# jacobkaufmann/kateth

Hardware: AMD Instinct MI355X
Metric: blobs/sec for blob_to_kzg_commitment and verify_blob_kzg_proof_batch (n=4096) (higher is better)
Workload: dtype u32 limbs (381-bit Fp / 255-bit Fr Montgomery integer arithmetic; signed 30-bit limbs on v_mad_i64_i32 in the fixed-base MSM, 28/29-bit radix in the other hot loops); 1 GPU; blob_to_kzg_commitment batch=4096 blobs per GPU (BASELINE configs[1]); blobs_per_gpu=4096, calls_in_flight=1, window_bits=22, parallelism=blob-sharded x1, RCCL all-gather of 48-B results, plane_groups=8

## Files before the change

include/kateth_amd.h:

```cpp
#ifndef KATETH_AMD_H
#define KATETH_AMD_H

#include <stddef.h>
#include <stdint.h>

#ifdef __cplusplus
extern "C" {
#endif

#define KZG_FIELD_ELEMENTS_PER_BLOB 4096
#define KZG_BYTES_PER_FIELD_ELEMENT 32
#define KZG_BYTES_PER_BLOB 131072
#define KZG_BYTES_PER_G1 48
#define KZG_BYTES_PER_G2 96
#define KZG_SETUP_G1_POINTS 4096
#define KZG_SETUP_G2_POINTS 65
#define KZG_CELLS_PER_EXT_BLOB 128
#define KZG_FIELD_ELEMENTS_PER_CELL 64
#define KZG_BYTES_PER_CELL 2048
#define KZG_G1_MONOMIAL_POINTS 64

#define KZG_OK 0
#define KZG_ERR_BLOB_INVALID_LEN 1
#define KZG_ERR_BLOB_INVALID_FIELD_ELEMENT 2
#define KZG_ERR_EC_INVALID_ENCODING 3
#define KZG_ERR_EC_NOT_ON_CURVE 4
#define KZG_ERR_EC_NOT_IN_GROUP 5
#define KZG_ERR_FF_INVALID_ENCODING 6
#define KZG_ERR_FF_NOT_IN_FIELD 7
#define KZG_ERR_CELLS_NOT_ENOUGH 8
#define KZG_ERR_CELLS_INCONSISTENT 9
#define KZG_ERR_CELL_INDEX 10
#define KZG_ERR_COMMITMENT_INDEX 11

#define KZG_FAIL_ARGUMENT (-1)
#define KZG_FAIL_HIP (-2)
#define KZG_FAIL_NO_DEVICE (-3)
#define KZG_FAIL_SETUP_G1 (-4)
#define KZG_FAIL_SETUP_G2 (-5)
#define KZG_FAIL_SETUP_UNSUPPORTED (-6)
#define KZG_FAIL_HOST (-7)

typedef struct kzg_ctx kzg_ctx;

#define KZG_CFG_TABLE_MAX 0x1
#define KZG_CFG_BUILD_ASYNC 0x2
#define KZG_ALL_DEVICES 0xffffffffu
typedef struct kzg_config {
  uint32_t struct_size;
  int32_t device;
  int32_t window_bits;
  int32_t flags;
  int32_t plane_groups;
  uint64_t table_budget_bytes;
  const int32_t* devices;
  uint32_t ndev;
  uint32_t reserved;
} kzg_config;
#define KZG_CONFIG_INIT {(uint32_t)sizeof(kzg_config), 0, 0, 0, 0, 0, NULL, 0, 0}

const char* kzg_recommended_env(void);

const char* kzg_last_error(void);
int32_t kzg_last_error_code(void);

int32_t kzg_ctx_create(const uint8_t* g1_lagrange, const uint8_t* g2_monomial, const kzg_config* cfg, kzg_ctx** out);
int32_t kzg_ctx_create_multi(const uint8_t* g1_lagrange, const uint8_t* g2_monomial, const int32_t* devices, uint32_t ndev, const kzg_config* cfg,
                             kzg_ctx** out);
void kzg_ctx_destroy(kzg_ctx* ctx);
int32_t kzg_device_count(void);
uint32_t kzg_ctx_members(const kzg_ctx* ctx);
int32_t kzg_ctx_member_device(const kzg_ctx* ctx, uint32_t k);
const kzg_ctx* kzg_ctx_member(const kzg_ctx* ctx, uint32_t k);
int32_t kzg_ctx_ready(const kzg_ctx* ctx);
int32_t kzg_ctx_wait_ready(const kzg_ctx* ctx);

int32_t kzg_ctx_window_bits(const kzg_ctx* ctx);
const char* kzg_ctx_msm_kernel_name(const kzg_ctx* ctx);
int32_t kzg_ctx_plane_groups(const kzg_ctx* ctx);
uint64_t kzg_ctx_table_bytes(const kzg_ctx* ctx);
uint64_t kzg_ctx_workspace_bytes(const kzg_ctx* ctx, uint32_t slot);

int32_t kzg_blob_to_commitment_batch(const kzg_ctx* ctx, const uint8_t* blobs, uint64_t n, uint8_t* out48, int32_t* status);
int32_t kzg_blob_to_commitment_batch_dev(const kzg_ctx* ctx, const void* d_blobs, uint64_t n, void* d_out48, void* d_status, void* hip_stream);

int32_t kzg_blob_to_commitment_batch_affine(const kzg_ctx* ctx, const uint8_t* blobs, uint64_t n, uint8_t* out_affine96, int32_t* status);
int32_t kzg_compute_blob_proof_batch_affine(const kzg_ctx* ctx, const uint8_t* blobs, const uint8_t* commitments48, uint64_t n, uint8_t* out_affine96, int32_t* status);
int32_t kzg_compute_proof_batch_affine(const kzg_ctx* ctx, const uint8_t* blobs, const uint8_t* z32, uint64_t n, uint8_t* out_proof_affine96, uint8_t* out_y32, int32_t* status);

int32_t kzg_g1_decompress_batch(const kzg_ctx* ctx, const uint8_t* in48, uint64_t n, uint8_t* out_affine96, int32_t* status);

int32_t kzg_evaluate_blobs(const kzg_ctx* ctx, const uint8_t* blobs, const uint8_t* z32, uint64_t n, uint8_t* out_y32, int32_t* status);

int32_t kzg_compute_blob_proof_batch(const kzg_ctx* ctx, const uint8_t* blobs, const uint8_t* commitments48, uint64_t n, uint8_t* out48, int32_t* status);
int32_t kzg_compute_blob_proof_batch_dev(const kzg_ctx* ctx, const void* d_blobs, const void* d_commitments48, uint64_t n, void* d_out48, void* d_status, void* hip_stream);

int32_t kzg_blob_sidecar_batch(const kzg_ctx* ctx, const uint8_t* blobs, uint64_t n, uint8_t* out_commitments48, uint8_t* out_proofs48,
                               uint8_t* out_versioned_hashes32 , int32_t* status);
int32_t kzg_blob_sidecar_batch_dev(const kzg_ctx* ctx, const void* d_blobs, uint64_t n, void* d_out_commitments48, void* d_out_proofs48,
                                   void* d_out_versioned_hashes32 , void* d_status, void* hip_stream);

int32_t kzg_compute_cells_batch(const kzg_ctx* ctx, const uint8_t* blobs, uint64_t n, uint8_t* out_cells , int32_t* status);
int32_t kzg_compute_cells_batch_dev(const kzg_ctx* ctx, const void* d_blobs, uint64_t n, void* d_out_cells, void* d_status, void* hip_stream);

int32_t kzg_recover_cells_batch(const kzg_ctx* ctx, const uint8_t* cells , const uint8_t* present , uint64_t n,
                                uint8_t* out_cells , int32_t* status);
int32_t kzg_recover_cells_batch_dev(const kzg_ctx* ctx, const void* d_cells, const void* d_present, uint64_t n, void* d_out_cells, void* d_status,
                                    void* hip_stream);

int32_t kzg_compute_cells_and_proofs_batch(const kzg_ctx* ctx, const uint8_t* blobs, uint64_t n, uint8_t* out_cells ,
                                           uint8_t* out_proofs48 , int32_t* status);
int32_t kzg_compute_cells_and_proofs_batch_dev(const kzg_ctx* ctx, const void* d_blobs, uint64_t n, void* d_out_cells , void* d_out_proofs48,
                                               void* d_status, void* hip_stream);
int32_t kzg_recover_cells_and_proofs_batch(const kzg_ctx* ctx, const uint8_t* cells, const uint8_t* present, uint64_t n, uint8_t* out_cells,
                                           uint8_t* out_proofs48, int32_t* status);
int32_t kzg_recover_cells_and_proofs_batch_dev(const kzg_ctx* ctx, const void* d_cells, const void* d_present, uint64_t n, void* d_out_cells,
                                               void* d_out_proofs48, void* d_status, void* hip_stream);

int32_t kzg_compute_cells_and_proofs_select_batch(const kzg_ctx* ctx, const uint8_t* blobs, const uint8_t* want , uint64_t n,
                                                  uint8_t* out_cells , uint8_t* inout_proofs48 ,
                                                  int32_t* status);
int32_t kzg_compute_cells_and_proofs_select_batch_dev(const kzg_ctx* ctx, const void* d_blobs, const uint8_t* want , uint64_t n,
                                                      void* d_out_cells , void* d_inout_proofs48, void* d_status, void* hip_stream);
int32_t kzg_recover_cells_and_proofs_select_batch(const kzg_ctx* ctx, const uint8_t* cells, const uint8_t* present, const uint8_t* want ,
                                                  uint64_t n, uint8_t* out_cells, uint8_t* inout_proofs48, int32_t* status);
int32_t kzg_recover_cells_and_proofs_select_batch_dev(const kzg_ctx* ctx, const void* d_cells, const void* d_present, const uint8_t* want ,
                                                      uint64_t n, void* d_out_cells, void* d_inout_proofs48, void* d_status, void* hip_stream);
uint64_t kzg_ctx_cellproof_vectors(const kzg_ctx* ctx);

int32_t kzg_compute_proof_batch(const kzg_ctx* ctx, const uint8_t* blobs, const uint8_t* z32, uint64_t n, uint8_t* out_proof48, uint8_t* out_y32, int32_t* status);

int32_t kzg_verify_blob_proof_batch(const kzg_ctx* ctx, const uint8_t* blobs, const uint8_t* commitments48, const uint8_t* proofs48, uint64_t n, int32_t* ok);
int32_t kzg_verify_blob_proof_batch_dev(const kzg_ctx* ctx, const void* d_blobs, const void* d_commitments48, const void* d_proofs48, uint64_t n, int32_t* ok, void* hip_stream);

int32_t kzg_verify_blob_proof(const kzg_ctx* ctx, const uint8_t* blob, const uint8_t* commitment48, const uint8_t* proof48, int32_t* ok);

int32_t kzg_verify_proof(const kzg_ctx* ctx, const uint8_t* proof48, const uint8_t* commitment48, const uint8_t* z32, const uint8_t* y32, int32_t* ok);

int32_t kzg_verify_proof_batch(const kzg_ctx* ctx, const uint8_t* proofs48, const uint8_t* commitments48, const uint8_t* z32, const uint8_t* y32, uint64_t n,
                               int32_t* ok);
int32_t kzg_verify_proof_batch_dev(const kzg_ctx* ctx, const void* d_proofs48, const void* d_commitments48, const void* d_z32, const void* d_y32, uint64_t n,
                                   int32_t* ok, void* hip_stream);
int32_t kzg_verify_proof_batch_group_dev(const kzg_ctx* ctx, const void* const* d_proofs48, const void* const* d_commitments48, const void* const* d_z32,
                                         const void* const* d_y32, const uint64_t* n_local, int32_t* ok, void* const* hip_streams);

int32_t kzg_ctx_g1_monomial(const kzg_ctx* ctx, uint32_t first, uint32_t count, uint8_t* out48);

int32_t kzg_verify_cell_proof_batch(const kzg_ctx* ctx, const uint8_t* commitments48, const uint64_t* cell_indices, const uint8_t* cells ,
                                    const uint8_t* proofs48, uint64_t n, int32_t* ok);
int32_t kzg_verify_cell_proof_batch_dev(const kzg_ctx* ctx, const void* d_commitments48, const void* d_cell_indices, const void* d_cells,
                                        const void* d_proofs48, uint64_t n, int32_t* ok, void* hip_stream);

int32_t kzg_verify_cell_proof_batch_rows(const kzg_ctx* ctx, const uint8_t* commitments48 , uint64_t u, const uint64_t* commitment_indices ,
                                         const uint64_t* cell_indices , const uint8_t* cells , const uint8_t* proofs48 ,
                                         uint64_t n, int32_t* ok);
int32_t kzg_verify_cell_proof_batch_rows_dev(const kzg_ctx* ctx, const void* d_commitments48, uint64_t u, const void* d_commitment_indices,
                                             const void* d_cell_indices, const void* d_cells, const void* d_proofs48, uint64_t n, int32_t* ok,
                                             void* hip_stream);
int32_t kzg_cell_row_weights(const kzg_ctx* ctx, const uint8_t* r32, uint64_t first_index, const uint64_t* commitment_indices , uint64_t n,
                             uint64_t u, uint8_t* out_w32 );

int32_t kzg_verify_blob_proof_batch_each(const kzg_ctx* ctx, const uint8_t* blobs, const uint8_t* commitments48, const uint8_t* proofs48, uint64_t n,
                                         uint8_t* ok_each, int32_t* status, int32_t* ok);
int32_t kzg_verify_blob_proof_batch_each_dev(const kzg_ctx* ctx, const void* d_blobs, const void* d_commitments48, const void* d_proofs48, uint64_t n,
                                             uint8_t* ok_each, int32_t* status, int32_t* ok, void* hip_stream);
int32_t kzg_verify_proof_batch_each(const kzg_ctx* ctx, const uint8_t* proofs48, const uint8_t* commitments48, const uint8_t* z32, const uint8_t* y32, uint64_t n,
                                    uint8_t* ok_each, int32_t* status, int32_t* ok);
int32_t kzg_verify_proof_batch_each_dev(const kzg_ctx* ctx, const void* d_proofs48, const void* d_commitments48, const void* d_z32, const void* d_y32, uint64_t n,
                                        uint8_t* ok_each, int32_t* status, int32_t* ok, void* hip_stream);
uint64_t kzg_verify_each_checks(const kzg_ctx* ctx);
uint64_t kzg_ctx_sessions_created(const kzg_ctx* ctx);

int32_t kzg_verify_cell_proof_batch_each(const kzg_ctx* ctx, const uint8_t* commitments48, const uint64_t* cell_indices, const uint8_t* cells ,
                                         const uint8_t* proofs48, uint64_t n, uint8_t* ok_each, int32_t* status, int32_t* ok);
int32_t kzg_verify_cell_proof_batch_each_dev(const kzg_ctx* ctx, const void* d_commitments48, const void* d_cell_indices, const void* d_cells,
                                             const void* d_proofs48, uint64_t n, uint8_t* ok_each, int32_t* status, int32_t* ok, void* hip_stream);

int32_t kzg_g1_monomial_lincomb(const kzg_ctx* ctx, const uint8_t* scalars32, uint64_t m, uint8_t* out96);

int32_t kzg_blob_to_commitment_batch_group_dev(const kzg_ctx* ctx, const void* const* d_blobs, const uint64_t* n_local, void* const* d_out48,
                                               void* const* d_status, void* const* hip_streams);
int32_t kzg_compute_blob_proof_batch_group_dev(const kzg_ctx* ctx, const void* const* d_blobs, const void* const* d_commitments48, const uint64_t* n_local,
                                               void* const* d_out48, void* const* d_status, void* const* hip_streams);
int32_t kzg_verify_blob_proof_batch_group_dev(const kzg_ctx* ctx, const void* const* d_blobs, const void* const* d_commitments48,
                                              const void* const* d_proofs48, const uint64_t* n_local, int32_t* ok, void* const* hip_streams);

typedef struct kzg_verify_session kzg_verify_session;
int32_t kzg_verify_phase1_dev(const kzg_ctx* ctx, const void* d_blobs, const void* d_commitments48, const void* d_proofs48, uint64_t n_local,
                              uint8_t* out_root32, int32_t* err6, kzg_verify_session** session, void* hip_stream);
int32_t kzg_verify_phase2_dev(kzg_verify_session* session, const uint8_t* roots32, uint64_t world, uint64_t first_index, uint64_t n_total,
                              uint8_t* out192);
void kzg_verify_session_destroy(kzg_verify_session* session);
int32_t kzg_verify_session_zy(kzg_verify_session* session, uint64_t first, uint64_t count, uint8_t* out_z32, uint8_t* out_y32);
int32_t kzg_verify_batch_finish(const kzg_ctx* ctx, const uint8_t* partials192, uint64_t world, int32_t* ok);
int32_t kzg_verify_session_tree(kzg_verify_session* session, const uint8_t* roots32, uint64_t world, uint64_t first_index, uint64_t n_total);
int32_t kzg_verify_session_tree_range(kzg_verify_session* session, uint64_t lo, uint64_t hi, uint8_t* out192);
int32_t kzg_verify_proof_phase1_dev(const kzg_ctx* ctx, const void* d_proofs48, const void* d_commitments48, const void* d_z32, const void* d_y32,
                                    uint64_t n_local, uint8_t* out_root32, int32_t* err8, kzg_verify_session** session, void* hip_stream);

int32_t kzg_synth_blobs_dev(const kzg_ctx* ctx, uint64_t seed, uint64_t first_index, uint64_t n, void* d_blobs, void* hip_stream);

int32_t kzg_microbench_fp_mul(const kzg_ctx* ctx, uint64_t lanes, uint64_t iters, float* ms);
int32_t kzg_microbench_valu_issue(const kzg_ctx* ctx, uint32_t waves_per_simd, uint32_t iters, double* cycles_per_inst, double* clock_ghz);
int32_t kzg_clock_probe_launch(const kzg_ctx* ctx, uint32_t duration_us);
int32_t kzg_clock_probe_read(const kzg_ctx* ctx, double* ghz_mean, double* ghz_min, double* ghz_max);

int32_t kzg_selftest_field_mul(const kzg_ctx* ctx, uint64_t lanes, uint64_t iters, uint64_t* mismatches);
int32_t kzg_selftest_exception_guard(int32_t kind);

int32_t kzg_profile_begin(const kzg_ctx* ctx);
int32_t kzg_profile_end(const kzg_ctx* ctx, double* msm_ms_total, uint64_t* msm_launches);
#define KZG_PROF_KINDS 8
int32_t kzg_profile_end_kinds(const kzg_ctx* ctx, double* ms, uint64_t* launches);
const char* kzg_profile_kind_name(int32_t kind);
uint64_t kzg_ctx_adds_per_blob(const kzg_ctx* ctx);

#ifdef __cplusplus
}
#endif
#endif
```

kateth_amd/csrc/comb_geom.hpp:

```cpp
#pragma once
#include <stdint.h>

#include "field.cuh"

namespace kzg {

struct CombGeom {
  uint32_t nb;
  uint32_t G;
  uint32_t H;
  uint32_t lpg;
  uint32_t ep64;
  uint32_t epg;
  uint32_t fair;
};

KZG_HD uint32_t comb_tbits(uint32_t nb, uint32_t r) { return nb == 3u ? (r == 0u ? 22u : 21u) : 64u / nb; }
KZG_HD uint32_t comb_point_off(uint32_t nb, uint32_t r) { return nb == 3u ? (r == 0u ? 0u : (r == 1u ? 22u : 43u)) : r * (64u / nb); }
KZG_HD uint32_t comb_entry_off(uint32_t nb, uint32_t r) {
  return nb == 3u ? (r == 0u ? 0u : (r == 1u ? (1u << 21) : (1u << 21) + (1u << 20))) : r << (64u / nb - 1u);
}
KZG_HD CombGeom comb_make_geom(uint32_t nb, uint32_t G) {
  CombGeom g;
  g.nb = nb;
  g.G = G;
  g.H = 256u / G;
  g.lpg = 64u / G;
  g.ep64 = nb == 3u ? (1u << 22) : nb << (64u / nb - 1u);
  g.epg = 64u * g.ep64;
  g.fair = 20u;
  return g;
}
KZG_HD uint64_t comb_table_entries(const CombGeom& g) { return (uint64_t)g.G * g.epg; }

struct CombWalk {
  uint32_t h, s, r, dq;
};
KZG_HD uint32_t comb_blocks_per_lane(const CombGeom& g, uint32_t splits, uint32_t lpb) { return (64u * g.nb) / (splits * (lpb / g.G)); }
KZG_HD bool comb_shape_is_wide(const CombGeom& g, uint32_t splits, uint32_t lpb) { return comb_blocks_per_lane(g, splits, lpb) % (4u * g.nb) == 0u; }
enum : int { COMB_SHAPE_ANY = 0, COMB_SHAPE_WIDE = 1, COMB_SHAPE_NARROW = 2 };
struct CombLanePos {
  uint32_t q, r;
};
KZG_HD void comb_walk_start(CombWalk& w, uint32_t H) {
  w.h = H - 1u;
  w.s = 0;
  w.r = 0;
  w.dq = 0;
}
KZG_HD bool comb_walk_advance(CombWalk& w, uint32_t nb, uint32_t bpo) {
  w.s++;
  w.r++;
  if (w.r == nb) {
    w.r = 0;
    w.dq++;
  }
  if (w.s != bpo) return false;
  w.s = 0;
  w.r = 0;
  w.dq = 0;
  w.h--;
  return true;
}
KZG_HD void comb_lane_advance(CombLanePos& p, uint32_t nb, bool wrapped, uint32_t b0) {
  p.r++;
  if (p.r == nb) {
    p.r = 0;
    p.q++;
  }
  if (wrapped) {
    p.q = b0 / nb;
    p.r = b0 % nb;
  }
}
KZG_HD bool comb_walk_loads_masks(const CombWalk& w) { return w.r == 0u && (w.dq & 3u) == 0u; }
KZG_HD uint32_t comb_walk_mask_slot(const CombWalk& w) { return w.dq & 3u; }
KZG_HD bool comb_walk_doubles(const CombWalk& w, uint32_t H) { return w.s == 0u && w.h != H - 1u; }
KZG_HD uint32_t comb_max_splits(const CombGeom& g) { return (64u * g.nb) / g.lpg; }

}
```

kateth_amd/csrc/engine.hip:

```cpp
#include <new>
#include <stdexcept>

#include "engine_internal.hpp"
#include "msm_comb.cuh"
#include "msm_reduce_kernels.cuh"
#include "setup_kernels.cuh"

#include <algorithm>
extern "C" const char* kzg_recommended_env(void) { return "GPU_MAX_HW_QUEUES=16"; }
static void hw_queues_note(bool trace) {
  static std::atomic<bool> said{false};
  if (!trace || said.exchange(true)) return;
  const char* e = getenv("GPU_MAX_HW_QUEUES");
  if (!e || atoi(e) < 8)
    fprintf(stderr, "[kateth_amd trace] GPU_MAX_HW_QUEUES is %s: calls kept in flight on several streams may share a hardware queue and run one after "
                    "the other; export %s before the process first touches HIP (the library does not change the environment)\n",
            e ? e : "unset (the runtime's default is 4)", kzg_recommended_env());
}

namespace {
class HelperPool {
  std::mutex mu;
  std::condition_variable cv;
  std::deque<std::function<void()>> q;
// ... 167 lines not shown
  WsSlot& w = ctx->wss[ctx->ws_cur];
  if (!w.ev) HIP_TRY(hipEventCreateWithFlags(&w.ev, hipEventDisableTiming));
  HIP_TRY(hipEventRecord(w.ev, st));
  w.last_st = st;
  w.used = true;
  return 0;
}

int32_t stage_init(const kzg_ctx* ctx) {
  if (ctx->stage_ready) return 0;
  bool ok = hipStreamCreateWithFlags(&ctx->verify_stream, hipStreamNonBlocking) == hipSuccess &&
            hipStreamCreateWithFlags(&ctx->stage_copy_stream, hipStreamNonBlocking) == hipSuccess;
  for (int r = 0; r < KZG_STAGE_STREAMS && ok; r++)
    ok = hipStreamCreateWithFlags(&ctx->stage_streams[r], hipStreamNonBlocking) == hipSuccess &&
         hipEventCreateWithFlags(&ctx->stage_join[r], hipEventDisableTiming) == hipSuccess;
  for (int k = 0; k < KZG_STAGE_SLOTS && ok; k++)
    ok = hipEventCreateWithFlags(&ctx->stage_copied[k], hipEventDisableTiming) == hipSuccess &&
         hipEventCreateWithFlags(&ctx->stage_done[k], hipEventDisableTiming) == hipSuccess;
  if (!ok) {
    stage_destroy(ctx);
    return fail(KZG_FAIL_HIP, "staging pipeline: stream/event creation failed");
  }
  ctx->stage_ready = true;
  return 0;
}
int32_t stage_reserve(const kzg_ctx* ctx, size_t arena_bytes, size_t io_bytes) {
  if (ctx->stage_bytes < arena_bytes) {
    if (ctx->stage) {
      HIP_TRY(hipDeviceSynchronize());
      (void)hipFree(ctx->stage);
    }
    ctx->stage = nullptr;
    ctx->stage_bytes = 0;
    if (hipMalloc(&ctx->stage, arena_bytes) != hipSuccess) return fail(KZG_FAIL_HIP, "hipMalloc(staging arena) failed");
    ctx->stage_bytes = arena_bytes;
  }
  if (ctx->hostio_bytes < io_bytes) {
    if (ctx->hostio) {
      HIP_TRY(hipDeviceSynchronize());
      (void)hipFree(ctx->hostio);
    }
    ctx->hostio = nullptr;
    ctx->hostio_bytes = 0;
    const size_t want = io_bytes + io_bytes / 4;
    if (hipMalloc(&ctx->hostio, want) != hipSuccess) return fail(KZG_FAIL_HIP, "hipMalloc(host i/o pool) failed");
    ctx->hostio_bytes = want;
  }
  return 0;
}
void stage_destroy(const kzg_ctx* ctx) {
  if (ctx->stage) (void)hipFree(ctx->stage);
  ctx->stage = nullptr;
  ctx->stage_bytes = 0;
  if (ctx->hostio) (void)hipFree(ctx->hostio);
  ctx->hostio = nullptr;
  ctx->hostio_bytes = 0;
  if (ctx->verify_stream) (void)hipStreamDestroy(ctx->verify_stream);
  if (ctx->stage_copy_stream) (void)hipStreamDestroy(ctx->stage_copy_stream);
  ctx->verify_stream = ctx->stage_copy_stream = nullptr;
  for (int r = 0; r < KZG_STAGE_STREAMS; r++) {
    if (ctx->stage_streams[r]) (void)hipStreamDestroy(ctx->stage_streams[r]);
    if (ctx->stage_join[r]) (void)hipEventDestroy(ctx->stage_join[r]);
    ctx->stage_streams[r] = nullptr;
    ctx->stage_join[r] = nullptr;
  }
  for (int k = 0; k < KZG_STAGE_SLOTS; k++) {
    if (ctx->stage_copied[k]) (void)hipEventDestroy(ctx->stage_copied[k]);
    if (ctx->stage_done[k]) (void)hipEventDestroy(ctx->stage_done[k]);
    ctx->stage_copied[k] = ctx->stage_done[k] = nullptr;
  }
  ctx->stage_ready = false;
}
void stage_drain(const kzg_ctx* ctx) {
  (void)hipStreamSynchronize(ctx->stage_copy_stream);
  for (int r = 0; r < KZG_STAGE_STREAMS; r++) (void)hipStreamSynchronize(ctx->stage_streams[r]);
}
int32_t stream_after(hipStream_t waiter, hipStream_t signaller, hipEvent_t ev) {
  HIP_TRY(hipEventRecord(ev, signaller));
  HIP_TRY(hipStreamWaitEvent(waiter, ev, 0));
  return 0;
}
int32_t StageRing::open(const kzg_ctx* c, uint64_t nslots, size_t bytes_per_slot, size_t io_bytes, bool overlap_copies) {
  ctx = c, slots = nslots, slot_bytes = bytes_per_slot, overlap = overlap_copies;
  if (slots < 1 || slots > (uint64_t)KZG_STAGE_SLOTS) return fail(KZG_FAIL_ARGUMENT, "staging ring: slot count out of range");
  const int32_t rc = stage_init(ctx);
  return rc ? rc : stage_reserve(ctx, slots * slot_bytes, io_bytes);
}
int32_t StageRing::feed(uint64_t k, const uint8_t* host_src, size_t bytes, hipStream_t comp, uint8_t** d_chunk) {
  const uint64_t slot = k % slots;
  hipStream_t copy_st = overlap ? ctx->stage_copy_stream : comp;
  if (bytes > slot_bytes) return fail(KZG_FAIL_ARGUMENT, "staging ring: chunk larger than its slot");
  *d_chunk = ctx->stage + slot * slot_bytes;
  if (copy_st != comp && k >= slots) HIP_TRY(hipStreamWaitEvent(copy_st, ctx->stage_done[slot], 0));
  HIP_TRY(hipMemcpyAsync(*d_chunk, host_src, bytes, hipMemcpyHostToDevice, copy_st));
  return copy_st != comp ? stream_after(comp, copy_st, ctx->stage_copied[slot]) : 0;
}
hipEvent_t StageRing::done_event(uint64_t k) const { return ctx->stage_done[k % slots]; }
int32_t StageRing::consumed(uint64_t k, hipStream_t comp) {
  HIP_TRY(hipEventRecord(done_event(k), comp));
  return 0;
}

int32_t HostCall::open(std::vector<uint64_t> passes_plan, size_t item_slot_bytes, bool overlap) {
  plan = std::move(passes_plan);
  for (uint64_t m : plan) max_pass = m > max_pass ? m : max_pass;
  int32_t rc = too_many ? fail(KZG_FAIL_ARGUMENT, "host call: too many arrays") : 0;
  if (rc == 0 && hipSetDevice(ctx->device) != hipSuccess) rc = fail(KZG_FAIL_HIP, "hipSetDevice failed");
  if (rc) return close(rc);
  stage_guard = std::unique_lock<std::mutex>(ctx->stage_lock);
  rc = ring.open(ctx, plan.size() > 1 ? 2 : 1, (size_t)max_pass * item_slot_bytes, io.off, overlap);
  if (rc) return close(rc);
  opened = true;
  st = ctx->stage_streams[0];
  for (int a = 0; a < count && rc == 0; a++)
    if (arrays[a].kind == UP && hipMemcpyAsync(dev(a), arrays[a].host, arrays[a].bytes, hipMemcpyHostToDevice, st) != hipSuccess)
      rc = fail(KZG_FAIL_HIP, "host-to-device copy failed");
  return rc ? close(rc) : 0;
}
int32_t HostCall::close(int32_t rc) {
  for (int a = 0; a < count && rc == 0; a++)
    if (arrays[a].kind == DOWN && hipMemcpyAsync(arrays[a].host, dev(a), arrays[a].bytes, hipMemcpyDeviceToHost, st) != hipSuccess)
      rc = fail(KZG_FAIL_HIP, "device-to-host copy failed");
  if (rc == 0 && hipStreamSynchronize(st) != hipSuccess) rc = fail(KZG_FAIL_HIP, "device-to-host copy failed");
  if (rc) (void)hipDeviceSynchronize();
  return rc;
}

static void tables_free(CombTables& t);
const MsmOverride* (*g_msm_override_hook)(kzg_ctx* ctx, uint32_t window_bits) = nullptr;

struct MsmShapeCost {
  uint32_t splits;
  uint32_t lpb;
  double cost;
};
static MsmShapeCost msm_shape(const kzg_ctx* ctx, uint64_t n) {
  const double S = (double)ctx->num_cus * 8.0;
  const uint32_t per_lane = (64u * ctx->comb.nb) / ctx->comb.lpg;
  const double A = (double)ctx->comb.H * per_lane, D = 0.75 * (ctx->comb.H - 1u);
  auto rounds = [&](double waves) { return waves <= S ? 1.0 : (double)(uint64_t)((waves + S - 1) / S); };
  MsmShapeCost best{1, 64, 0};
  bool have = false;
  for (uint32_t v = 1; v <= 64 && v <= per_lane; v++) {
    if (per_lane % v != 0) continue;
    const double c = rounds((double)n * v) * (A / v + D + 10.0);
    if (!have || c < best.cost) {
      best = MsmShapeCost{v, 64, c};
      have = true;
    }
  }
  const bool half_ok = !ctx->knobs.comb_full_wave && ctx->comb.G <= 32 && (64u * ctx->comb.nb) % (32u / ctx->comb.G) == 0;
  if (half_ok && n >= 2) {
    const double c = rounds((double)((n + 1) / 2)) * (2.0 * A + D + 10.0);
    if (c < best.cost) best = MsmShapeCost{1, 32, c};
  }
  return best;
}

uint32_t choose_splits(const kzg_ctx* ctx, uint64_t n) {
  if (ctx->use_comb) {
    if (ctx->d_table_lat && n <= KZG_LAT_MAX_BLOBS && !ctx->knobs.msm_splits) return lat_splits(n);
    const uint32_t per_lane = (64u * ctx->comb.nb) / ctx->comb.lpg;
    if (ctx->knobs.msm_splits && ctx->knobs.msm_splits <= 64 && per_lane % ctx->knobs.msm_splits == 0) return ctx->knobs.msm_splits;
    return msm_shape(ctx, n).splits;
  }
  if (ctx->knobs.msm_splits) return ctx->knobs.msm_splits;
  const uint64_t target = (uint64_t)ctx->num_cus * 8;
  uint32_t s = 1;
  while (s < 64 && n * s < target) s <<= 1;
  return s;
}
uint32_t msm_lanes_per_blob(const kzg_ctx* ctx, uint64_t n, uint32_t splits) {
  if (!ctx->use_comb || splits != 1 || ctx->knobs.msm_splits) return 64;
  if (msm_uses_lat(ctx, splits)) return 64;
  return msm_shape(ctx, n).lpb;
}

extern "C" uint64_t kzg_ctx_adds_per_blob(const kzg_ctx* ctx) {
  if (!ctx) return 0;
  std::lock_guard<std::mutex> guard(ctx->lock);
  return ctx->use_comb ? (uint64_t)256u * 64u * ctx->comb.nb : ctx->msm_override->adds_per_blob;
}

extern "C" int32_t kzg_profile_begin(const kzg_ctx* ctx) try {
  if (!ctx) return fail(KZG_FAIL_ARGUMENT, "null argument");
  std::lock_guard<std::mutex> guard(ctx->prof_lock);
  ctx->prof_used = 0;
  ctx->profiling.store(true);
  return 0;
} catch (...) {
  return abi_exception();
}

static const char* const PROF_NAMES[PROF_KINDS] = {"k_msm_comb30", "k_challenge*", "k_eval_frac", "k_g1_decompress", "k_poly",
                                                    "k_var_* (two lincombs)", "k_msm_reduce* + k_g1_compress", "k_comb_transpose"};

extern "C" const char* kzg_ctx_msm_kernel_name(const kzg_ctx* ctx) { return (ctx && ctx->msm_override) ? ctx->msm_override->kernel_name : "k_msm_comb30"; }
extern "C" int32_t kzg_ctx_plane_groups(const kzg_ctx* ctx) try {
  if (!ctx || !ctx->use_comb) return 0;
  std::lock_guard<std::mutex> guard(ctx->lock);
  return (int32_t)ctx->comb.G;
} catch (...) {
  return abi_exception();
}
extern "C" const char* kzg_profile_kind_name(int32_t kind) { return (kind >= 0 && kind < PROF_KINDS) ? PROF_NAMES[kind] : ""; }

extern "C" int32_t kzg_profile_end_kinds(const kzg_ctx* ctx, double* ms_out, uint64_t* launches) try {
  if (!ctx || !ms_out || !launches) return fail(KZG_FAIL_ARGUMENT, "null argument");
  std::lock_guard<std::mutex> guard(ctx->prof_lock);
  HIP_TRY(hipSetDevice(ctx->device));
  for (int k = 0; k < PROF_KINDS; k++) {
    ms_out[k] = 0;
    launches[k] = 0;
  }
  ctx->profiling.store(false);
  for (size_t i = 0; i < ctx->prof_used; i++) {
    float ms = 0;
    const ProfEvent& pe = ctx->prof_events[i];
    if (hipEventSynchronize(pe.e1) != hipSuccess || hipEventElapsedTime(&ms, pe.e0, pe.e1) != hipSuccess) {
      (void)hipGetLastError();
      continue;
    }
    ms_out[pe.kind] += ms;
    launches[pe.kind]++;
  }
  ctx->prof_used = 0;
  return 0;
} catch (...) {
  return abi_exception();
}

extern "C" int32_t kzg_profile_end(const kzg_ctx* ctx, double* msm_ms_total, uint64_t* msm_launches) try {
  if (!ctx || !msm_ms_total || !msm_launches) return fail(KZG_FAIL_ARGUMENT, "null argument");
  double ms[PROF_KINDS];
  uint64_t cnt[PROF_KINDS];
  int32_t rc = kzg_profile_end_kinds(ctx, ms, cnt);
  if (rc) return rc;
  *msm_ms_total = ms[PROF_MSM_FIXED];
  *msm_launches = cnt[PROF_MSM_FIXED];
  return 0;
} catch (...) {
  return abi_exception();
}

int32_t prof_next(const kzg_ctx* ctx, int kind, hipEvent_t* e0, hipEvent_t* e1) {
  *e0 = *e1 = nullptr;
  std::lock_guard<std::mutex> guard(ctx->prof_lock);
  if (!ctx->profiling.load()) return 0;
  if (ctx->prof_used == ctx->prof_events.size()) {
    hipEvent_t a, b;
    HIP_TRY(hipEventCreate(&a));
    HIP_TRY(hipEventCreate(&b));
    ctx->prof_events.push_back(ProfEvent{kind, a, b});
  }
  ProfEvent& pe = ctx->prof_events[ctx->prof_used++];
  pe.kind = kind;
  *e0 = pe.e0;
  *e1 = pe.e1;
  return 0;
}

EnvKnobs read_env_knobs() {
  {
    EnvKnobs k;
    k.trace = getenv("KATETH_AMD_TRACE") != nullptr;
    if (const char* e = getenv("KATETH_AMD_HOST_FP")) host_fp_force_portable() = std::string(e) == "portable";
    if (const char* e = getenv("KATETH_AMD_PROOF_CHUNK")) k.proof_chunk = (uint64_t)atoll(e) > 0 ? (uint64_t)atoll(e) : 0;
    if (const char* e = getenv("KATETH_AMD_SIDECAR_PASS")) k.sidecar_pass = (uint64_t)atoll(e) > 0 ? (uint64_t)atoll(e) : 0;
    if (const char* e = getenv("KATETH_AMD_CELLS_PASS")) k.cells_pass = (uint64_t)atoll(e) > 0 ? (uint64_t)atoll(e) : 0;
    if (const char* e = getenv("KATETH_AMD_CELLPROOF_PASS")) k.cellproof_pass = (uint64_t)atoll(e) > 0 ? (uint64_t)atoll(e) : 0;
    if (const char* e = getenv("KATETH_AMD_PROOF_OVERLAP")) k.proof_overlap = atoi(e) != 0;
    if (const char* e = getenv("KATETH_AMD_EVAL_GROUP")) k.eval_group = atoi(e);
    k.verify_serial = getenv("KATETH_AMD_VERIFY_SERIAL") != nullptr;
    k.single_via_batch = getenv("KATETH_AMD_SINGLE_VIA_BATCH") != nullptr;
    if (const char* e = getenv("KATETH_AMD_VAR_MSM")) k.var_msm_classic = std::string(e) == "classic";
    if (const char* e = getenv("KATETH_AMD_VAR_GLV")) k.var_glv = atoi(e) != 0;
    if (const char* e = getenv("KATETH_AMD_VAR_SEG")) k.var_seg = (uint32_t)std::max(0, atoi(e));
    if (const char* e = getenv("KATETH_AMD_VERIFY_STREAMS")) k.verify_streams = (uint32_t)atoi(e) <= (uint32_t)KZG_STAGE_STREAMS ? (uint32_t)atoi(e) : 0u;
    if (const char* e = getenv("KATETH_AMD_VERIFY_CHUNK")) k.verify_chunk = (uint64_t)atoll(e) > 0 ? (uint64_t)atoll(e) : 0;
    k.comb_full_wave = getenv("KATETH_AMD_COMB_FULL_WAVE") != nullptr;
    if (const char* e = getenv("KATETH_AMD_LAT_TABLE")) k.lat_table = atoi(e) != 0;
    if (const char* e = getenv("KATETH_AMD_COMB_FAIR")) k.comb_fair = (uint32_t)atoi(e) < 40u ? (uint32_t)atoi(e) : 0u;
    if (const char* e = getenv("KATETH_AMD_MSM_SPLITS")) {
      const int v = atoi(e);
      if (v >= 1 && v <= 64 && (v & (v - 1)) == 0) k.msm_splits = (uint32_t)v;
    }
    if (const char* e = getenv("KATETH_AMD_CHALLENGE_SPLIT_MAX")) k.challenge_split_max = (uint64_t)atoll(e) > 0 ? (uint64_t)atoll(e) : 0;
    return k;
  }
}

extern "C" int32_t kzg_ctx_window_bits(const kzg_ctx* ctx) try {
  if (!ctx) return 0;
  std::lock_guard<std::mutex> guard(ctx->lock);
  return (int32_t)ctx->window_class;
} catch (...) {
  return abi_exception();
}
extern "C" uint64_t kzg_ctx_table_bytes(const kzg_ctx* ctx) {
  if (!ctx) return 0;
  std::lock_guard<std::mutex> guard(ctx->lock);
  return ctx->table_bytes;
}
extern "C" uint64_t kzg_ctx_workspace_bytes(const kzg_ctx* ctx, uint32_t slot) {
  if (!ctx || slot >= (uint32_t)KZG_WS_SLOTS) return 0;
  std::lock_guard<std::mutex> guard(ctx->lock);
  return ctx->wss[slot].bytes;
}
extern "C" uint32_t kzg_ctx_members(const kzg_ctx* ctx) { return ctx ? 1u + (uint32_t)ctx->peers.size() : 0u; }
extern "C" const kzg_ctx* kzg_ctx_member(const kzg_ctx* ctx, uint32_t k) {
  if (!ctx || k > ctx->peers.size()) return nullptr;
  return k == 0 ? ctx : ctx->peers[k - 1];
}
extern "C" int32_t kzg_ctx_member_device(const kzg_ctx* ctx, uint32_t k) try {
  const kzg_ctx* m = kzg_ctx_member(ctx, k);
  return m ? m->device : -1;
} catch (...) {
  return abi_exception();
}

extern "C" void kzg_ctx_destroy(kzg_ctx* ctx) {
  if (!ctx) return;
  for (kzg_ctx* p : ctx->peers) kzg_ctx_destroy(p);
  ctx->peers.clear();
  ctx->build_cancel.store(true);
  if (ctx->build_thread.joinable()) ctx->build_thread.join();
  (void)hipSetDevice(ctx->device);
  (void)hipDeviceSynchronize();
  for (CombTables& t : ctx->retired) tables_free(t);
  if (ctx->d_table) (void)hipFree(ctx->d_table);
  if (ctx->d_table_lat) (void)hipFree(ctx->d_table_lat);
  if (ctx->d_bases_brp) (void)hipFree(ctx->d_bases_brp);
  if (ctx->d_roots_brp) (void)hipFree(ctx->d_roots_brp);
  if (ctx->d_eval_tab) (void)hipFree(ctx->d_eval_tab);
  if (ctx->d_cells_tab) (void)hipFree(ctx->d_cells_tab);
  if (ctx->d_recover_tab) (void)hipFree(ctx->d_recover_tab);
  if (ctx->d_cellv_tab) (void)hipFree(ctx->d_cellv_tab);
  if (ctx->d_cellv_h64) (void)hipFree(ctx->d_cellv_h64);
  if (ctx->d_g1_monomial) (void)hipFree(ctx->d_g1_monomial);
  if (ctx->d_cellproof_tab) (void)hipFree(ctx->d_cellproof_tab);
  if (ctx->d_gen_affine) (void)hipFree(ctx->d_gen_affine);
  if (ctx->d_comb_k) (void)hipFree(ctx->d_comb_k);
  if (ctx->d_comb_k_lat) (void)hipFree(ctx->d_comb_k_lat);
  if (ctx->msm_override && ctx->msm_override->destroy) ctx->msm_override->destroy(ctx);
  delete ctx->pairing;
  for (WsSlot& w : ctx->wss) {
    if (w.p) (void)hipFree(w.p);
    if (w.ev) (void)hipEventDestroy(w.ev);
  }
  if (ctx->d_clock_probe) (void)hipFree(ctx->d_clock_probe);
  if (ctx->probe_stream) (void)hipStreamDestroy(ctx->probe_stream);
  if (ctx->side_stream) (void)hipStreamDestroy(ctx->side_stream);
  if (ctx->copy_stream) (void)hipStreamDestroy(ctx->copy_stream);
  for (auto e : ctx->proof_events) (void)hipEventDestroy(e);
  for (auto& pin : ctx->pair_pins) {
    if (pin.p) (void)hipHostFree(pin.p);
    if (pin.ev) (void)hipEventDestroy(pin.ev);
  }
  for (auto& pe : ctx->prof_events) {
    (void)hipEventDestroy(pe.e0);
    (void)hipEventDestroy(pe.e1);
  }
  session_pool_clear(ctx);
  stage_destroy(ctx);
  delete ctx;
}


struct ScratchAllocs {
  std::vector<void*> ptrs;
  template <class T>
  hipError_t alloc(T** p, size_t bytes) {
    hipError_t e = hipMalloc(p, bytes);
    if (e == hipSuccess) ptrs.push_back(*p);
    return e;
  }
  ~ScratchAllocs() {
    for (void* p : ptrs) (void)hipFree(p);
  }
};

static void tables_free(CombTables& t) {
  if (t.d_table) (void)hipFree(t.d_table);
  if (t.d_table_lat) (void)hipFree(t.d_table_lat);
  if (t.d_comb_k) (void)hipFree(t.d_comb_k);
  if (t.d_comb_k_lat) (void)hipFree(t.d_comb_k_lat);
  t = CombTables{};
}
static void tables_install(kzg_ctx* ctx, const CombTables& t) {
  std::lock_guard<std::mutex> guard(ctx->lock);
  if (ctx->d_table || ctx->d_table_lat || ctx->d_comb_k || ctx->d_comb_k_lat) {
    CombTables old;
    old.d_table = ctx->d_table;
    old.d_table_lat = ctx->d_table_lat;
    old.d_comb_k = ctx->d_comb_k;
    old.d_comb_k_lat = ctx->d_comb_k_lat;
    ctx->retired.push_back(old);
  }
  ctx->comb = t.comb;
  ctx->comb_lat = t.comb_lat;
  ctx->d_table = t.d_table;
  ctx->d_table_lat = t.d_table_lat;
  ctx->d_comb_k = t.d_comb_k;
  ctx->d_comb_k_lat = t.d_comb_k_lat;
  ctx->table_bytes = t.table_bytes;
  ctx->window_class = t.window_class;
}

static int32_t comb_build_table(const kzg_ctx* ctx, const CombGeom& cg, uint4** out_table, ScratchAllocs& scratch, TraceTimer& tt, hipStream_t st,
                                const std::atomic<bool>* cancel) {
  uint4* d_table = nullptr;
  HIP_TRY(hipMalloc(&d_table, comb_table_entries(cg) * 96));
  *out_table = d_table;
  tt.mark("table allocation");
  uint4 *d_B = nullptr, *d_D = nullptr;
  HIP_TRY(scratch.alloc(&d_B, (size_t)cg.G * 4096 * 96));
  HIP_TRY(scratch.alloc(&d_D, (size_t)cg.G * 4096 * 96));
  hipLaunchKernelGGL(k_comb_bases, dim3(64), dim3(64), 0, st, ctx->d_bases_brp, cg, d_B, d_D);
  HIP_TRY(hipGetLastError());
  uint32_t min_t = 64;
  for (uint32_t r = 0; r < cg.nb; r++) min_t = comb_tbits(cg.nb, r) < min_t ? comb_tbits(cg.nb, r) : min_t;
  const uint32_t sl = (min_t - 1 < 9) ? min_t - 1 : 9;
  uint32_t nq = 64;
  while (nq > 1 && (uint64_t)nq * cg.ep64 * sizeof(g1_xyzz) > (13ull << 30)) nq >>= 1;
  g1_xyzz* d_tmp = nullptr;
  HIP_TRY(scratch.alloc(&d_tmp, (size_t)nq * cg.ep64 * sizeof(g1_xyzz)));
  uint32_t* d_inf_seen = nullptr;
  HIP_TRY(scratch.alloc(&d_inf_seen, sizeof(uint32_t)));
  HIP_TRY(hipMemsetAsync(d_inf_seen, 0, sizeof(uint32_t), st));
  for (uint32_t grp = 0; grp < cg.G; grp++) {
    for (uint32_t q0 = 0; q0 < 64; q0 += nq) {
      if (cancel && cancel->load()) {
        (void)hipStreamSynchronize(st);
        return fail(KZG_FAIL_ARGUMENT, "table build cancelled (context destroyed)");
      }
      const uint64_t threads = (uint64_t)nq * (cg.ep64 >> sl);
      hipLaunchKernelGGL(k_comb_chain, dim3((unsigned)((threads + 63) / 64)), dim3(64), 0, st, d_B, d_D, grp, q0, nq, cg, sl, d_tmp);
      constexpr int KN = 8;
      const uint64_t count = (uint64_t)nq * cg.ep64;
      const uint64_t nthreads = (count + KN - 1) / KN;
      hipLaunchKernelGGL(k_table_normalize<KN>, dim3((unsigned)((nthreads + 63) / 64)), dim3(64), 0, st, d_tmp, count, d_table,
                         (uint64_t)grp * cg.epg + (uint64_t)q0 * cg.ep64, TABLE_FMT_PACKED30, d_inf_seen);
      HIP_TRY(hipGetLastError());
      if (cancel) HIP_TRY(hipStreamSynchronize(st));
    }
  }
  uint32_t inf_seen = 0;
  HIP_TRY(hipMemcpyAsync(&inf_seen, d_inf_seen, sizeof(uint32_t), hipMemcpyDeviceToHost, st));
  HIP_TRY(hipStreamSynchronize(st));
  tt.mark("comb table build kernels");
  if (inf_seen)
    return fail(KZG_FAIL_SETUP_UNSUPPORTED, "degenerate setup: a +-1 combination of consecutive g1_lagrange points is the point at infinity "
                                   "(repeated / opposite points); the fixed-base comb table cannot represent it");
  return 0;
}

static inline uint32_t class_blocks(uint32_t c) { return c >= 22 ? 3u : (c >= 16 ? 4u : (c >= 8 ? 8u : 16u)); }

static int32_t comb_build_tables(const kzg_ctx* ctx, uint32_t c, uint32_t G, CombTables& t, hipStream_t st, const std::atomic<bool>* cancel) {
  TraceTimer tt(ctx->knobs.trace, cancel ? "comb_build (background)" : "comb_build");
  ScratchAllocs scratch;
  t = CombTables{};
  const uint32_t nb = class_blocks(c);
  t.comb = comb_make_geom(nb, G);
  t.comb.fair = ctx->knobs.comb_fair;
  t.window_class = nb == 3 ? 22u : 64u / nb;
  t.table_bytes = comb_table_entries(t.comb) * 96;
  int32_t rc = comb_build_table(ctx, t.comb, &t.d_table, scratch, tt, st, cancel);
  if (rc == 0 && nb == 3 && ctx->knobs.lat_table) {
    t.comb_lat = comb_make_geom(8, 64);
    t.comb_lat.fair = t.comb.fair;
    rc = comb_build_table(ctx, t.comb_lat, &t.d_table_lat, scratch, tt, st, cancel);
  }
  auto constant_terms = [&]() -> int32_t {
    uint4* d_sum = nullptr;
    uint32_t* d_sum_inf = nullptr;
    HIP_TRY(scratch.alloc(&d_sum, 96));
    HIP_TRY(scratch.alloc(&d_sum_inf, sizeof(uint32_t)));
    hipLaunchKernelGGL(k_setup_sum_bases, dim3(1), dim3(64), 0, st, ctx->d_bases_brp, d_sum, d_sum_inf);
    HIP_TRY(hipGetLastError());
    uint32_t h[24], sum_inf = 0;
    HIP_TRY(hipMemcpyAsync(h, d_sum, 96, hipMemcpyDeviceToHost, st));
    HIP_TRY(hipMemcpyAsync(&sum_inf, d_sum_inf, sizeof(uint32_t), hipMemcpyDeviceToHost, st));
    HIP_TRY(hipStreamSynchronize(st));
    if (sum_inf) return 0;
    fp_t x, y;
    for (int q = 0; q < 12; q++) {
      x.v[q] = h[q];
      y.v[q] = h[12 + q];
    }
    auto constant_for = [&](uint32_t H, uint4** d_out) -> int32_t {
      const uint32_t c0p[8] = KZG_FR_COMB_C0_PLAIN;
      fr_t c0, two, pw, inv, k;
      for (int q = 0; q < 8; q++) c0.v[q] = c0p[q];
      to_mont<FrParams>(c0, c0);
      two = fr_one();
      add_mod<FrParams>(two, two, two);
      pw = fr_one();
      for (uint32_t i = 0; i + 1 < H; i++) fr_mul(pw, pw, two);
      fr_inv(inv, pw);
      fr_mul(k, c0, inv);
      from_mont<FrParams>(k, k);
      g1_xyzz acc;
      xyzz_set_inf(acc);
      for (int bit = 255; bit >= 0; bit--) {
        xyzz_dbl(acc);
        if ((k.v[bit >> 5] >> (bit & 31)) & 1u) xyzz_madd(acc, x, y);
      }
      fp_t kx, ky;
      if (!xyzz_to_affine(kx, ky, acc)) return 0;
      uint32_t hk[24];
      fp_to_packed30(hk, kx);
      fp_to_packed30(hk + 12, ky);
      HIP_TRY(hipMalloc(d_out, 96));
      HIP_TRY(hipMemcpyAsync(*d_out, hk, 96, hipMemcpyHostToDevice, st));
      HIP_TRY(hipStreamSynchronize(st));
      return 0;
    };
    int32_t rck = constant_for(t.comb.H, &t.d_comb_k);
    if (rck == 0 && t.d_table_lat) rck = constant_for(t.comb_lat.H, &t.d_comb_k_lat);
    return rck;
  };
  if (rc == 0) rc = constant_terms();
  if (rc == 0 && hipStreamSynchronize(st) != hipSuccess) rc = fail(KZG_FAIL_HIP, "table build: synchronize failed");
  tt.mark("comb constant term");
  if (rc) {
    const ErrorSnapshot keep = error_snapshot();
    (void)hipStreamSynchronize(st);
    tables_free(t);
    error_publish(keep);
  }
  return rc;
}

static int32_t ctx_build(kzg_ctx* ctx, const uint8_t* g1_lagrange, const uint8_t* g2_monomial, uint32_t c, uint32_t G) {
  TraceTimer tt(ctx->knobs.trace, "ctx_build");
  ScratchAllocs scratch;
  hipStream_t st = nullptr;
  {
    host::g2_affine tau{}, tau64{};
    for (int i = 0; i < KZG_SETUP_G2_POINTS; i++) {
      host::g2_affine q;
      int32_t stq = host::g2_decompress(q, g2_monomial + 96 * i);
      if (stq != 0) return fail_detail(KZG_FAIL_SETUP_G2, stq, "g2_monomial[" + std::to_string(i) + "] rejected, code " + std::to_string(stq));
      if (i == 1) tau = q;
      if (i == KZG_G1_MONOMIAL_POINTS) tau64 = q;
    }
    ctx->pairing = new host::pairing_ctx();
    ctx->pairing->fc = host::make_frob_consts();
    host::g2_affine gen;
    {
      const uint32_t x0[12] = KZG_FP_G2X0_MONT, x1[12] = KZG_FP_G2X1_MONT, y0[12] = KZG_FP_G2Y0_MONT, y1[12] = KZG_FP_G2Y1_MONT;
      for (int q = 0; q < 12; q++) {
        gen.x.c0.v[q] = x0[q];
        gen.x.c1.v[q] = x1[q];
        gen.y.c0.v[q] = y0[q];
        gen.y.c1.v[q] = y1[q];
      }
      gen.inf = false;
    }
    ctx->pairing->lines_g2 = host::precompute_lines(gen);
    ctx->pairing->lines_tau = host::precompute_lines(tau);
    ctx->pairing->lines_tau64 = host::precompute_lines(tau64);
  }
  tt.mark("G2 decode + Miller lines (host)");
  {
    const uint32_t gx[12] = KZG_FP_G1X_R392, gy[12] = KZG_FP_G1Y_R392;
    uint32_t h[24];
    for (int q = 0; q < 12; q++) {
      h[q] = gx[q];
      h[12 + q] = gy[q];
    }
    const uint32_t px[12] = KZG_FP_G1PHIX_R392, py[12] = KZG_FP_G1PHIY_R392;
    uint32_t h2[48];
    for (int q = 0; q < 24; q++) h2[q] = h[q];
    for (int q = 0; q < 12; q++) {
      h2[24 + q] = px[q];
      h2[36 + q] = py[q];
    }
    HIP_TRY(hipMalloc(&ctx->d_gen_affine, 192));
    HIP_TRY(hipMemcpy(ctx->d_gen_affine, h2, 192, hipMemcpyHostToDevice));
  }
  uint8_t* d_in = nullptr;
  int32_t* d_status = nullptr;
  HIP_TRY(scratch.alloc(&d_in, 4096 * 48));
  HIP_TRY(scratch.alloc(&d_status, 4096 * sizeof(int32_t)));
  HIP_TRY(hipMemcpy(d_in, g1_lagrange, 4096 * 48, hipMemcpyHostToDevice));
  HIP_TRY(hipMalloc(&ctx->d_bases_brp, 4096 * 96));
  hipLaunchKernelGGL(k_setup_g1, dim3(64), dim3(64), 0, st, d_in, ctx->d_bases_brp, d_status);
  HIP_TRY(hipGetLastError());
  std::vector<int32_t> h_status(4096);
  HIP_TRY(hipMemcpy(h_status.data(), d_status, 4096 * sizeof(int32_t), hipMemcpyDeviceToHost));
  for (int i = 0; i < 4096; i++)
    if (h_status[i] != 0)
      return fail_detail(KZG_FAIL_SETUP_G1, h_status[i] == 100 ? 0 : h_status[i], "g1_lagrange[" + std::to_string(i) + "] rejected, code " + std::to_string(h_status[i]) +
                                         (h_status[i] == 100 ? " (point at infinity is not supported as a setup base)" : ""));
  tt.mark("G1 decode");
  HIP_TRY(hipMalloc(&ctx->d_roots_brp, 4096 * sizeof(fr_t)));
  hipLaunchKernelGGL(k_setup_roots, dim3(64), dim3(64), 0, st, ctx->d_roots_brp);
  HIP_TRY(hipMalloc(&ctx->d_eval_tab, (size_t)EVAL_TAB_HEXES * EVAL_TAB_DWORDS * sizeof(uint32_t)));
  hipLaunchKernelGGL(k_setup_eval_tab, dim3(EVAL_TAB_HEXES / 64), dim3(64), 0, st, ctx->d_roots_brp, ctx->d_eval_tab);
  HIP_TRY(hipMalloc(&ctx->d_cells_tab, (size_t)CELLS_TAB_ENTRIES * CELLS_TAB_ENTRY * sizeof(uint32_t)));
  hipLaunchKernelGGL(k_setup_cells_tab, dim3(CELLS_TAB_ENTRIES / 64), dim3(64), 0, st, ctx->d_cells_tab);
  HIP_TRY(hipMalloc(&ctx->d_recover_tab, (size_t)RECOVER_TAB_ENTRIES * CELLS_TAB_ENTRY * sizeof(uint32_t)));
  hipLaunchKernelGGL(k_setup_recover_tab, dim3(RECOVER_TAB_ENTRIES / 64), dim3(64), 0, st, ctx->d_recover_tab);
  HIP_TRY(hipMalloc(&ctx->d_cellv_tab, (size_t)CELLV_TAB_ENTRIES * CELLS_TAB_ENTRY * sizeof(uint32_t)));
  HIP_TRY(hipMalloc(&ctx->d_cellv_h64, 128 * sizeof(fr_t)));
  hipLaunchKernelGGL(k_setup_cellv_tab, dim3(CELLV_TAB_ENTRIES / 64), dim3(64), 0, st, ctx->d_cellv_tab, ctx->d_cellv_h64);
  HIP_TRY(hipGetLastError());
  HIP_TRY(hipDeviceSynchronize());
  tt.mark("roots + evaluation table");
  if (ctx->msm_override && ctx->msm_override->build) {
    int32_t rco = ctx->msm_override->build(ctx);
    if (rco) return rco;
  }
  if (ctx->use_comb) {
    CombTables t;
    int32_t rcc = comb_build_tables(ctx, c, G, t, st, nullptr);
    if (rcc) return rcc;
    tables_install(ctx, t);
  }
  HIP_TRY(hipDeviceSynchronize());
  return 0;
}

static int32_t ctx_create_with(const uint8_t* g1_lagrange, const uint8_t* g2_monomial, int device, uint32_t c, uint32_t G, kzg_ctx** out) {
  kzg_ctx* ctx = new (std::nothrow) kzg_ctx();
  if (!ctx) return fail(KZG_FAIL_ARGUMENT, "out of host memory");
  ctx->device = device;
  const uint32_t nb = class_blocks(c);
  ctx->knobs = read_env_knobs();
  ctx->comb = comb_make_geom(nb, G);
  ctx->comb.fair = ctx->knobs.comb_fair;
  ctx->window_class = nb == 3 ? 22u : 64u / nb;
  if (hipStreamCreateWithFlags(&ctx->side_stream, hipStreamNonBlocking) != hipSuccess ||
      hipStreamCreateWithFlags(&ctx->copy_stream, hipStreamNonBlocking) != hipSuccess) {
    delete ctx;
    return fail(KZG_FAIL_HIP, "hipStreamCreate failed");
  }
  hipDeviceProp_t prop;
  if (hipGetDeviceProperties(&prop, device) == hipSuccess) ctx->num_cus = (uint32_t)prop.multiProcessorCount;
  if (g_msm_override_hook) ctx->msm_override = g_msm_override_hook(ctx, c);
  int32_t rc = ctx_build(ctx, g1_lagrange, g2_monomial, c, G);
  if (rc != 0) {
    const ErrorSnapshot keep = error_snapshot();
    kzg_ctx_destroy(ctx);
    (void)hipGetLastError();
    error_publish(keep);
    return rc;
  }
  warm_code_object_blob();
  warm_code_object_proof();
  warm_code_object_verify();
  *out = ctx;
  return 0;
}

static void build_thread_main(kzg_ctx* ctx, std::vector<TableChoice> ladder, bool automatic) {
  int32_t rc = 0;
  hipStream_t st = nullptr;
  if (hipSetDevice(ctx->device) != hipSuccess || hipStreamCreateWithFlags(&st, hipStreamNonBlocking) != hipSuccess)
    rc = fail(KZG_FAIL_HIP, "background table build: stream creation failed");
  if (rc == 0) {
    for (const TableChoice& ch : ladder) {
      if (class_blocks(ch.c) == ctx->comb.nb && ch.G == ctx->comb.G) {
        break;
      }
      CombTables t;
      rc = comb_build_tables(ctx, ch.c, ch.G, t, st, &ctx->build_cancel);
      if (rc == 0) {
        tables_install(ctx, t);
        break;
      }
      if (!automatic || rc != KZG_FAIL_HIP || ctx->build_cancel.load()) break;
      (void)hipGetLastError();
    }
  }
  if (st) (void)hipStreamDestroy(st);
  if (rc) (void)hipGetLastError();
  {
    std::lock_guard<std::mutex> guard(ctx->build_mu);
    ctx->build_rc = rc;
    if (rc) ctx->build_err = error_snapshot();
    ctx->build_running = false;
  }
  ctx->build_cv.notify_all();
}

extern "C" int32_t kzg_ctx_ready(const kzg_ctx* ctx) try {
  if (!ctx) return 0;
  {
    std::lock_guard<std::mutex> guard(ctx->build_mu);
    if (ctx->build_running) return 0;
  }
  for (const kzg_ctx* p : ctx->peers)
    if (!kzg_ctx_ready(p)) return 0;
  return 1;
} catch (...) {
  return abi_exception();
}
extern "C" int32_t kzg_ctx_wait_ready(const kzg_ctx* ctx) try {
  if (!ctx) return fail(KZG_FAIL_ARGUMENT, "null argument");
  int32_t rc = 0;
  {
    std::unique_lock<std::mutex> guard(ctx->build_mu);
    ctx->build_cv.wait(guard, [&] { return !ctx->build_running; });
    rc = ctx->build_rc;
    if (rc) error_publish(ctx->build_err);
  }
  for (const kzg_ctx* p : ctx->peers) {
    const int32_t rp = kzg_ctx_wait_ready(p);
    if (rc == 0) rc = rp;
  }
  return rc;
} catch (...) {
  return abi_exception();
}

extern "C" int32_t kzg_device_count(void) try {
  int ndev = 0;
  if (hipGetDeviceCount(&ndev) != hipSuccess || ndev <= 0)
    return fail(KZG_FAIL_NO_DEVICE, "no HIP device visible: the kateth_amd engine has no CPU fallback");
  return ndev;
} catch (...) {
  return abi_exception();
}

int32_t ctx_create_single(const uint8_t* g1_lagrange, const uint8_t* g2_monomial, const kzg_config* cfg, int device, kzg_ctx** out) {
  *out = nullptr;
  HIP_TRY(hipSetDevice(device));
  constexpr size_t GiB = (size_t)1 << 30;
  constexpr size_t GROUP22_BYTES = (size_t)64 * ((size_t)1 << 22) * 96;
  constexpr size_t CLASS16_BYTES = (size_t)16 * 64 * ((size_t)4 << 15) * 96;
  size_t free_b = 0, total_b = 0;
  if (hipMemGetInfo(&free_b, &total_b) != hipSuccess) free_b = 0;
  const int32_t flags = cfg ? cfg->flags : 0;
  if (flags & ~(KZG_CFG_TABLE_MAX | KZG_CFG_BUILD_ASYNC)) return fail(KZG_FAIL_ARGUMENT, "unknown kzg_config.flags bit");
  if (cfg && cfg->reserved) return fail(KZG_FAIL_ARGUMENT, "kzg_config.reserved must be 0");
  uint32_t want = cfg ? (uint32_t)cfg->window_bits : 0u;
  if (want == 0)
    if (const char* e = getenv("KATETH_AMD_WINDOW_BITS")) want = (uint32_t)atoi(e);
  if (want != 0 && (want < 4 || want > 22)) return fail(KZG_FAIL_ARGUMENT, "window_bits must be 0 (automatic) or in [4,22]");
  uint32_t G_fixed = (cfg && cfg->plane_groups) ? (uint32_t)cfg->plane_groups : 0u;
  if (G_fixed == 0)
    if (const char* e = getenv("KATETH_AMD_COMB_GROUPS")) G_fixed = (uint32_t)atoi(e);
  if (G_fixed && !(G_fixed == 1 || G_fixed == 2 || G_fixed == 4 || G_fixed == 8 || G_fixed == 16))
    return fail(KZG_FAIL_ARGUMENT, "plane groups must be 1, 2, 4, 8 or 16");
  size_t budget = cfg ? (size_t)cfg->table_budget_bytes : 0;
  if (budget == 0 && !(flags & KZG_CFG_TABLE_MAX))
    if (const char* e = getenv("KATETH_AMD_TABLE_BUDGET_GIB"))
      if (atof(e) > 0) budget = (size_t)(atof(e) * (double)GiB);
  if (budget == 0) budget = (flags & KZG_CFG_TABLE_MAX) ? ~(size_t)0 : 100 * GiB;
  const TableChoice full[4] = {{22, 8, 8 * GROUP22_BYTES + 40 * GiB}, {22, 4, 4 * GROUP22_BYTES + 40 * GiB}, {16, 16, 21 * GiB}, {8, 16, 0}};
  const size_t table_of[4] = {8 * GROUP22_BYTES, 4 * GROUP22_BYTES, CLASS16_BYTES, 0};
  std::vector<TableChoice> ladder;
  const bool automatic = want == 0;
  if (!automatic) {
    uint32_t G = want >= 22 ? (free_b >= full[0].need ? 8u : 4u) : 16u;
    if (G_fixed) G = G_fixed;
    ladder.push_back(TableChoice{want, G, 0});
  } else {
    for (int k = 0; k < 4; k++)
      if (free_b >= full[k].need && budget >= table_of[k]) ladder.push_back(TableChoice{full[k].c, G_fixed ? G_fixed : full[k].G, full[k].need});
  }
  if (ladder.empty()) ladder.push_back(TableChoice{8, G_fixed ? G_fixed : 16u, 0});
  if ((flags & KZG_CFG_BUILD_ASYNC) && !g_msm_override_hook && class_blocks(ladder[0].c) < 8u) {
    kzg_ctx* ctx = nullptr;
    hw_queues_note(getenv("KATETH_AMD_TRACE") != nullptr);
    if (getenv("KATETH_AMD_TRACE"))
      fprintf(stderr, "[kateth_amd trace] kzg_ctx_create device %d: first-use table class 8; class %u, %u plane groups follows in the background\n", device,
              ladder[0].c, ladder[0].G);
    int32_t rc = ctx_create_with(g1_lagrange, g2_monomial, device, 8, 16, &ctx);
    if (rc) return rc;
    {
      std::lock_guard<std::mutex> guard(ctx->build_mu);
      ctx->build_running = true;
    }
    try {
      ctx->build_thread = std::thread(build_thread_main, ctx, ladder, automatic);
    } catch (...) {
      build_thread_main(ctx, ladder, automatic);
    }
    *out = ctx;
    return 0;
  }
  const bool trace = getenv("KATETH_AMD_TRACE") != nullptr;
  hw_queues_note(trace);
  auto say = [&](const char* how, const TableChoice& ch) {
    if (trace)
      fprintf(stderr, "[kateth_amd trace] kzg_ctx_create device %d: table class %u, %u plane groups (%s; %.1f GiB free, budget %s)\n", device, ch.c, ch.G, how,
              (double)free_b / (double)GiB, budget == ~(size_t)0 ? "none" : (std::to_string((double)budget / (double)GiB) + " GiB").c_str());
  };
  int32_t rc = fail(KZG_FAIL_HIP, "no table class fits");
  for (const TableChoice& ch : ladder) {
    say(automatic ? "automatic" : "as configured", ch);
    rc = ctx_create_with(g1_lagrange, g2_monomial, device, ch.c, ch.G, out);
    if (!automatic || rc != KZG_FAIL_HIP) return rc;
    (void)hipGetLastError();
  }
  return rc;
}

static int32_t cfg_check(const kzg_config* cfg) {
  if (cfg && cfg->struct_size != (uint32_t)sizeof(kzg_config))
    return fail(KZG_FAIL_ARGUMENT, "kzg_config.struct_size is " + std::to_string(cfg->struct_size) + ", this library's kzg_config has " +
                                       std::to_string(sizeof(kzg_config)) + " bytes: initialise with KZG_CONFIG_INIT from the matching include/kateth_amd.h");
  return 0;
}

extern "C" int32_t kzg_ctx_create(const uint8_t* g1_lagrange, const uint8_t* g2_monomial, const kzg_config* cfg, kzg_ctx** out) try {
  if (!g1_lagrange || !g2_monomial || !out) return fail(KZG_FAIL_ARGUMENT, "null argument");
  *out = nullptr;
  if (int32_t rcc = cfg_check(cfg)) return rcc;
  const int32_t ndev = kzg_device_count();
  if (ndev < 0) return ndev;
  if (cfg && cfg->ndev != 0) return group_create(g1_lagrange, g2_monomial, cfg, out);
  const int device = cfg ? cfg->device : 0;
  if (device < 0 || device >= ndev) return fail(KZG_FAIL_ARGUMENT, "device ordinal out of range");
  return ctx_create_single(g1_lagrange, g2_monomial, cfg, device, out);
} catch (...) {
  return abi_exception();
}

extern "C" int32_t kzg_ctx_create_multi(const uint8_t* g1_lagrange, const uint8_t* g2_monomial, const int32_t* devices, uint32_t ndev,
                                        const kzg_config* cfg, kzg_ctx** out) try {
  kzg_config c = KZG_CONFIG_INIT;
  if (int32_t rcc = cfg_check(cfg)) return rcc;
  if (cfg) c = *cfg;
  c.devices = devices;
  c.ndev = ndev;
  if (ndev == 0) return fail(KZG_FAIL_ARGUMENT, "kzg_ctx_create_multi: ndev must not be 0 (KZG_ALL_DEVICES = every visible device)");
  return kzg_ctx_create(g1_lagrange, g2_monomial, &c, out);
} catch (...) {
  return abi_exception();
}

int32_t msm_launch(const kzg_ctx* ctx, bool be_bytes, const uint8_t* d_scalars, uint64_t n, int32_t* d_status, g1_xyzz* partials, uint32_t splits, uint32_t lpb,
                   void* scratch, hipStream_t st, hipEvent_t scalars_consumed) {
  if (ctx->msm_override) {
    int32_t rco = ctx->msm_override->launch(ctx, be_bytes, d_scalars, n, d_status, partials, splits, lpb, scratch, st);
    if (rco == 0 && scalars_consumed) HIP_TRY(hipEventRecord(scalars_consumed, st));
    return rco;
  }
  uint64_t* masks = reinterpret_cast<uint64_t*>(scratch);
  {
    ProfScope ps(ctx, PROF_TRANSPOSE, st);
    if (be_bytes)
      hipLaunchKernelGGL((k_comb_transpose<true>), dim3((unsigned)(n * 8)), dim3(512), 0, st, d_scalars, n, masks, d_status);
    else
      hipLaunchKernelGGL((k_comb_transpose<false>), dim3((unsigned)(n * 8)), dim3(512), 0, st, d_scalars, n, masks, d_status);
  }
  if (scalars_consumed) HIP_TRY(hipEventRecord(scalars_consumed, st));
  ProfScope ps(ctx, PROF_MSM_FIXED, st);
  const bool lat = msm_uses_lat(ctx, splits);
  const uint4* table = lat ? ctx->d_table_lat : ctx->d_table;
  const CombGeom geom = lat ? ctx->comb_lat : ctx->comb;
  const uint4* comb_k = (const uint4*)(lat ? ctx->d_comb_k_lat : ctx->d_comb_k);
  if (comb_shape_is_wide(geom, splits, lpb))
    hipLaunchKernelGGL((k_msm_comb30<false, COMB_SHAPE_WIDE>), dim3((unsigned)msm_units(n, splits, lpb)), dim3(64), 0, st, masks, n, splits, lpb, table, geom,
                       partials, comb_k, (uint64_t*)nullptr);
  else
    hipLaunchKernelGGL((k_msm_comb30<false, COMB_SHAPE_NARROW>), dim3((unsigned)msm_units(n, splits, lpb)), dim3(64), 0, st, masks, n, splits, lpb, table, geom,
                       partials, comb_k, (uint64_t*)nullptr);
  HIP_TRY(hipGetLastError());
  return 0;
}
int32_t msm_finish(const kzg_ctx* ctx, uint64_t n, uint8_t* d_out48, uint8_t* d_out_affine96, const int32_t* d_status, g1_xyzz* partials,
                                 g1_xyzz* sums, uint32_t splits, uint32_t lpb, hipStream_t st) {
  ProfScope ps(ctx, PROF_REDUCE_COMPRESS, st);
  g1_xyzz* unit_sums = (splits == 1) ? sums : partials + (size_t)n * splits * 64;
  const uint64_t units = msm_units(n, splits, lpb);
  if (lpb == 32)
    hipLaunchKernelGGL(k_msm_reduce_half4, dim3((unsigned)((units + 1) / 2)), dim3(64), 0, st, partials, units, unit_sums, n);
  else
    hipLaunchKernelGGL(k_msm_reduce, dim3((unsigned)units), dim3(64), 0, st, partials, units, lpb, unit_sums, units);
  if (splits > 64) {
    hipLaunchKernelGGL((k_msm_reduce_splits<true>), dim3((unsigned)n), dim3(64), 0, st, unit_sums, splits, n, sums, d_status, d_out48, d_out_affine96);
    HIP_TRY(hipGetLastError());
    return 0;
  }
  if (splits > 1)
    hipLaunchKernelGGL((k_msm_reduce_splits<false>), dim3((unsigned)n), dim3(64), 0, st, unit_sums, splits, n, sums, (const int32_t*)nullptr,
                       (uint8_t*)nullptr, (uint8_t*)nullptr);
  hipLaunchKernelGGL(k_g1_compress, dim3(blocks_for(n, 64)), dim3(64), 0, st, sums, n, d_status, d_out48, d_out_affine96);
  HIP_TRY(hipGetLastError());
  return 0;
}
int32_t msm_pipeline(const kzg_ctx* ctx, bool be_bytes, const uint8_t* d_scalars, uint64_t n, uint8_t* d_out48, uint8_t* d_out_affine96, int32_t* d_status,
                     const MsmBufs& bufs, uint8_t* ws, hipStream_t st) {
  g1_xyzz* partials = reinterpret_cast<g1_xyzz*>(ws + bufs.o_part);
  const uint32_t lpb = msm_lanes_per_blob(ctx, n, bufs.splits);
  int32_t rc = msm_launch(ctx, be_bytes, d_scalars, n, d_status, partials, bufs.splits, lpb, ws + bufs.o_scratch, st);
  if (rc) return rc;
  return msm_finish(ctx, n, d_out48, d_out_affine96, d_status, partials, reinterpret_cast<g1_xyzz*>(ws + bufs.o_sum), bufs.splits, lpb, st);
}

static int32_t commit_dev_locked(const kzg_ctx* ctx, const void* d_blobs, uint64_t n, void* d_out48, void* d_out_affine96, int32_t* d_status,
                                 hipStream_t st) {
  if (n == 0) return 0;
  const uint64_t chunk_max = 16384;
  const uint64_t cn = n < chunk_max ? n : chunk_max;
  Carve carve;
  const MsmBufs bufs = msm_carve(ctx, carve, cn);
  int32_t rc = ws_reserve(ctx, carve.off, st);
  if (rc) return rc;
  HIP_TRY(hipMemsetAsync(d_status, 0, n * sizeof(int32_t), st));
  for (uint64_t base = 0; base < n; base += cn) {
    const uint64_t m = (n - base < cn) ? (n - base) : cn;
    rc = msm_pipeline(ctx, true, reinterpret_cast<const uint8_t*>(d_blobs) + base * (uint64_t)KZG_BYTES_PER_BLOB, m,
                            d_out48 ? reinterpret_cast<uint8_t*>(d_out48) + base * 48 : nullptr,
                            d_out_affine96 ? reinterpret_cast<uint8_t*>(d_out_affine96) + base * 96 : nullptr, d_status + base, bufs, ws_ptr(ctx), st);
    if (rc) return rc;
  }
  return 0;
}

extern "C" int32_t kzg_blob_to_commitment_batch_dev(const kzg_ctx* ctx, const void* d_blobs, uint64_t n, void* d_out48, void* d_status,
                                                    void* hip_stream) try {
  if (!ctx || (n && (!d_blobs || !d_out48 || !d_status))) return fail(KZG_FAIL_ARGUMENT, "null argument");
  HIP_TRY(hipSetDevice(ctx->device));
  hipStream_t st = reinterpret_cast<hipStream_t>(hip_stream);
  return with_workspace(ctx, st, [&] { return commit_dev_locked(ctx, d_blobs, n, d_out48, nullptr, reinterpret_cast<int32_t*>(d_status), st); });
} catch (...) {
  return abi_exception();
}

static int32_t derive_g1_monomial(const kzg_ctx* ctx) {
  TraceTimer tt(ctx->knobs.trace, "monomial G1 points");
  constexpr uint32_t M = KZG_G1_MONOMIAL_POINTS;
  ScratchAllocs scratch;
  uint8_t *d_blobs = nullptr, *d_out48 = nullptr, *d_inf = nullptr;
  int32_t* d_status = nullptr;
  HIP_TRY(scratch.alloc(&d_blobs, (size_t)M * KZG_BYTES_PER_BLOB));
  HIP_TRY(scratch.alloc(&d_out48, (size_t)M * 48));
  HIP_TRY(scratch.alloc(&d_status, 2 * (size_t)M * sizeof(int32_t)));
  HIP_TRY(scratch.alloc(&d_inf, 2 * (size_t)M));
  uint4* d_points = nullptr;
  HIP_TRY(scratch.alloc(&d_points, 2 * (size_t)M * 96));
  hipStream_t st = nullptr;
  hipLaunchKernelGGL(k_setup_monomial_blobs, dim3(M * 4096 / 256), dim3(256), 0, st, ctx->d_roots_brp, M, d_blobs);
  HIP_TRY(hipGetLastError());
  int32_t rc = kzg_blob_to_commitment_batch_dev(ctx, d_blobs, M, d_out48, d_status, st);
  if (rc) return rc;
  HIP_TRY(hipMemsetAsync(d_inf, 0, 2 * (size_t)M, st));
  launch_g1_decompress(st, d_out48, M, d_status + M, nullptr, 0, nullptr, d_points, d_inf);
  launch_glv_points(st, d_points, M, M);
  HIP_TRY(hipGetLastError());
  int32_t h_status[2 * M];
  uint8_t h_inf[M];
  HIP_TRY(hipMemcpyAsync(h_status, d_status, sizeof(h_status), hipMemcpyDeviceToHost, st));
  HIP_TRY(hipMemcpyAsync(h_inf, d_inf, sizeof(h_inf), hipMemcpyDeviceToHost, st));
  HIP_TRY(hipMemcpyAsync(ctx->g1_monomial48, d_out48, (size_t)M * 48, hipMemcpyDeviceToHost, st));
  HIP_TRY(hipStreamSynchronize(st));
  for (uint32_t j = 0; j < 2 * M; j++)
    if (h_status[j]) return fail(KZG_FAIL_HIP, "monomial G1 points: commitment " + std::to_string(j % M) + " failed, code " + std::to_string(h_status[j]));
  for (uint32_t j = 0; j < M; j++)
    if (h_inf[j]) return fail(KZG_FAIL_SETUP_UNSUPPORTED, "degenerate setup: the commitment of X^" + std::to_string(j) + " is the point at infinity");
  scratch.ptrs.erase(std::find(scratch.ptrs.begin(), scratch.ptrs.end(), (void*)d_points));
  ctx->d_g1_monomial = d_points;
  tt.mark("64 blobs, commitments, decoding");
  return 0;
}
int32_t ensure_g1_monomial(const kzg_ctx* ctx) {
  if (ctx->g1_monomial_ready.load(std::memory_order_acquire)) return 0;
  std::lock_guard<std::mutex> guard(ctx->g1_monomial_mu);
  if (ctx->g1_monomial_ready.load(std::memory_order_relaxed)) return 0;
  HIP_TRY(hipSetDevice(ctx->device));
  const int32_t rc = derive_g1_monomial(ctx);
  if (rc == 0) ctx->g1_monomial_ready.store(true, std::memory_order_release);
  return rc;
}

extern "C" int32_t kzg_ctx_g1_monomial(const kzg_ctx* ctx, uint32_t first, uint32_t count, uint8_t* out48) try {
  if (!ctx || (count && !out48) || first > KZG_G1_MONOMIAL_POINTS || count > KZG_G1_MONOMIAL_POINTS - first) return fail(KZG_FAIL_ARGUMENT, "bad argument");
  const int32_t rc = ensure_g1_monomial(ctx);
  if (rc) return rc;
  memcpy(out48, ctx->g1_monomial48 + (size_t)first * 48, (size_t)count * 48);
  return 0;
} catch (...) {
  return abi_exception();
}

static std::vector<uint64_t> commit_host_plan(uint64_t n) {
  std::vector<uint64_t> plan;
  if (n <= 768) {
    plan.push_back(n);
    return plan;
  }
  const uint64_t ramp[4] = {512, 512, 1024, 2048};
  uint64_t rest = n;
  for (uint64_t r : ramp) {
    if (rest < r) break;
    plan.push_back(r);
    rest -= r;
  }
  if (plan.size() == 4)
    for (; rest >= 4096; rest -= 4096) plan.push_back(4096);
  if (rest >= 256)
    plan.push_back(rest);
  else
    plan[0] += rest;
  return plan;
}

int32_t commit_host(const kzg_ctx* ctx, const uint8_t* blobs, uint64_t n, uint8_t* out48, uint8_t* out_affine96, int32_t* status) {
  if (n == 0) return 0;
  HostCall hc(ctx);
  const int a_res = hc.download(out48 ? out48 : out_affine96, (size_t)n * (out48 ? 48 : 96)), a_st = hc.download(status, n * sizeof(int32_t));
  int32_t rc = hc.open(commit_host_plan(n), KZG_BYTES_PER_BLOB);
  if (rc) return rc;
  const std::vector<uint64_t>& plan = hc.plan;
  const uint64_t max_chunk = hc.max_pass;
  const bool piped = plan.size() > 1;
  const uint64_t nslots = piped ? 2 : 1;
  uint8_t* d_res = hc.dev(a_res);
  int32_t* d_status = hc.dev<int32_t>(a_st);
  hipStream_t comp[2] = {ctx->stage_streams[0], ctx->stage_streams[1]};
  std::lock_guard<std::mutex> guard(ctx->lock);
  WsCall ws(ctx, comp[0]);
  uint64_t max_units = 1;
  for (uint64_t m : plan) {
    const uint32_t sp = choose_splits(ctx, m);
    const uint64_t units = msm_units(m, sp, msm_lanes_per_blob(ctx, m, sp));
    max_units = units > max_units ? units : max_units;
  }
  Carve per_slot;
  const size_t o_part = per_slot.take((size_t)max_units * 65 * sizeof(g1_xyzz)), o_sums = per_slot.take((size_t)max_chunk * sizeof(g1_xyzz)),
               o_masks = per_slot.take(msm_scratch_bytes(ctx, max_chunk));
  rc = ws.begin();
  if (rc == 0) rc = ws_reserve(ctx, nslots * per_slot.off, comp[0]);
  if (rc == 0 && piped) rc = ws_wait(ctx, comp[1]);
  if (rc == 0 && hipMemsetAsync(d_status, 0, n * sizeof(int32_t), comp[0]) != hipSuccess) rc = fail(KZG_FAIL_HIP, "memset failed");
  if (rc == 0 && piped) rc = stream_after(comp[1], comp[0], ctx->stage_join[0]);
  uint64_t base = 0;
  for (size_t k = 0; k < plan.size() && rc == 0; base += plan[k], k++) {
    const int slot = (int)(k & 1);
    const uint64_t m = plan[k];
    const uint32_t splits = choose_splits(ctx, m);
    const uint32_t lpb = msm_lanes_per_blob(ctx, m, splits);
    uint8_t* wslot = ws_ptr(ctx) + (size_t)slot * per_slot.off;
    g1_xyzz* partials = reinterpret_cast<g1_xyzz*>(wslot + o_part);
    g1_xyzz* sums = reinterpret_cast<g1_xyzz*>(wslot + o_sums);
    uint8_t* d_chunk = nullptr;
    rc = hc.ring.feed(k, blobs + base * (size_t)KZG_BYTES_PER_BLOB, m * (size_t)KZG_BYTES_PER_BLOB, comp[slot], &d_chunk);
    if (rc == 0) rc = msm_launch(ctx, true, d_chunk, m, d_status + base, partials, splits, lpb, wslot + o_masks, comp[slot], hc.ring.done_event(k));
    if (rc == 0)
      rc = msm_finish(ctx, m, out48 ? d_res + base * 48 : nullptr, out_affine96 ? d_res + base * 96 : nullptr, d_status + base, partials, sums, splits, lpb,
                      comp[slot]);
  }
  if (rc == 0 && piped) rc = stream_after(comp[0], comp[1], ctx->stage_join[1]);
  if (rc == 0) rc = ws.end();
  return hc.close(rc);
}

extern "C" int32_t kzg_blob_to_commitment_batch(const kzg_ctx* ctx, const uint8_t* blobs, uint64_t n, uint8_t* out48, int32_t* status) try {
  if (!ctx || (n && (!blobs || !out48 || !status))) return fail(KZG_FAIL_ARGUMENT, "null argument");
  return on_members(ctx, n, [&](const kzg_ctx* m, uint64_t first, uint64_t count) {
    return commit_host(m, blobs + first * (size_t)KZG_BYTES_PER_BLOB, count, out48 + first * 48, nullptr, status + first);
  });
} catch (...) {
  return abi_exception();
}
extern "C" int32_t kzg_blob_to_commitment_batch_affine(const kzg_ctx* ctx, const uint8_t* blobs, uint64_t n, uint8_t* out_affine96, int32_t* status) try {
  if (!ctx || (n && (!blobs || !out_affine96 || !status))) return fail(KZG_FAIL_ARGUMENT, "null argument");
  return on_members(ctx, n, [&](const kzg_ctx* m, uint64_t first, uint64_t count) {
    return commit_host(m, blobs + first * (size_t)KZG_BYTES_PER_BLOB, count, nullptr, out_affine96 + first * 96, status + first);
  });
} catch (...) {
  return abi_exception();
}

extern "C" int32_t kzg_synth_blobs_dev(const kzg_ctx* ctx, uint64_t seed, uint64_t first_index, uint64_t n, void* d_blobs, void* hip_stream) try {
  if (!ctx || (n && !d_blobs)) return fail(KZG_FAIL_ARGUMENT, "null argument");
  if (n == 0) return 0;
  HIP_TRY(hipSetDevice(ctx->device));
  launch_synth_blobs(reinterpret_cast<hipStream_t>(hip_stream), seed, first_index, n, reinterpret_cast<uint8_t*>(d_blobs));
  HIP_TRY(hipGetLastError());
  return 0;
} catch (...) {
  return abi_exception();
}

__global__ __launch_bounds__(256) void k_microbench_fp28_mul(uint32_t* out, uint64_t iters) {
  fp28 a, b;
  const uint32_t t = blockIdx.x * blockDim.x + threadIdx.x;
#pragma unroll
  for (int q = 0; q < F28_N; q++) {
    a.l[q] = f28_one_limb(q) ^ (t & 0xffu);
    b.l[q] = f28_r384_limb(q);
  }
#pragma unroll 1
  for (uint64_t it = 0; it < iters; it++) {
    fp28 r;
    f28_mul(r, a, b);
    a = b;
    b = r;
  }
  uint32_t x = 0;
#pragma unroll
  for (int q = 0; q < F28_N; q++) x ^= b.l[q];
  out[t] = x;
}

extern "C" int32_t kzg_microbench_fp_mul(const kzg_ctx* ctx, uint64_t lanes, uint64_t iters, float* ms) try {
  if (!ctx || !ms || lanes == 0) return fail(KZG_FAIL_ARGUMENT, "null argument");
  HIP_TRY(hipSetDevice(ctx->device));
  lanes = align_up(lanes, 256);
  uint32_t* d_out = nullptr;
  HIP_TRY(hipMalloc(&d_out, lanes * sizeof(uint32_t)));
  hipEvent_t e0, e1;
  HIP_TRY(hipEventCreate(&e0));
  HIP_TRY(hipEventCreate(&e1));
  auto kern = k_microbench_fp28_mul;
  hipLaunchKernelGGL(kern, dim3((unsigned)(lanes / 256)), dim3(256), 0, nullptr, d_out, (uint64_t)16);
  HIP_TRY(hipEventRecord(e0, nullptr));
  hipLaunchKernelGGL(kern, dim3((unsigned)(lanes / 256)), dim3(256), 0, nullptr, d_out, iters);
  HIP_TRY(hipEventRecord(e1, nullptr));
  HIP_TRY(hipEventSynchronize(e1));
  HIP_TRY(hipEventElapsedTime(ms, e0, e1));
  (void)hipEventDestroy(e0);
  (void)hipEventDestroy(e1);
  (void)hipFree(d_out);
  return 0;
} catch (...) {
  return abi_exception();
}

__global__ __launch_bounds__(1024) void k_microbench_valu_issue(uint32_t* out, unsigned long long* ticks, uint32_t iters, uint32_t seed) {
  extern __shared__ uint32_t issue_lds[];
  uint64_t x[8];
  for (int c = 0; c < 8; c++) x[c] = ((uint64_t)(seed + threadIdx.x * 7 + c * 0x9e3779b9u) << 20) | 0x3ff0000000000001ull;
  const uint32_t y = seed ^ 0x5555u ^ threadIdx.x, z = seed + 3u;
  if (threadIdx.x == 0) issue_lds[0] = seed;
  __syncthreads();
  const unsigned long long r0 = __builtin_amdgcn_s_memrealtime();
  const unsigned long long t0 = __builtin_amdgcn_s_memtime();
#pragma unroll 1
  for (uint32_t it = 0; it < iters; it++) {
#pragma unroll
    for (int rep = 0; rep < 32; rep++) {
#pragma unroll
      for (int c = 0; c < 8; c++) asm volatile("v_mad_u64_u32 %0, vcc, %1, %2, %0" : "+v"(x[c]) : "v"(y), "v"(z) : "vcc");
    }
  }
  const unsigned long long t1 = __builtin_amdgcn_s_memtime();
  const unsigned long long r1 = __builtin_amdgcn_s_memrealtime();
  uint64_t r = 0;
  for (int c = 0; c < 8; c++) r ^= x[c];
  out[blockIdx.x * blockDim.x + threadIdx.x] = (uint32_t)r ^ (uint32_t)(r >> 32);
  if ((threadIdx.x & 63) == 0) {
    const uint32_t wave = blockIdx.x * (blockDim.x >> 6) + (threadIdx.x >> 6);
    ticks[2 * wave] = t1 - t0;
    ticks[2 * wave + 1] = r1 - r0;
  }
}

extern "C" int32_t kzg_microbench_valu_issue(const kzg_ctx* ctx, uint32_t waves_per_simd, uint32_t iters, double* cycles_per_inst, double* clock_ghz) try {
  if (!ctx || !cycles_per_inst || !clock_ghz || waves_per_simd < 1 || waves_per_simd > 4 || iters == 0) return fail(KZG_FAIL_ARGUMENT, "bad argument");
  HIP_TRY(hipSetDevice(ctx->device));
  const uint32_t blocks = ctx->num_cus, threads = 256 * waves_per_simd;
  const size_t lds = (size_t)(160 * 1024) - 1024;
  HIP_TRY(hipFuncSetAttribute((const void*)k_microbench_valu_issue, hipFuncAttributeMaxDynamicSharedMemorySize, (int)lds));
  uint32_t* d_out = nullptr;
  unsigned long long* d_ticks = nullptr;
  HIP_TRY(hipMalloc(&d_out, (size_t)blocks * threads * 4));
  HIP_TRY(hipMalloc(&d_ticks, (size_t)blocks * (threads / 64) * 2 * 8));
  hipLaunchKernelGGL(k_microbench_valu_issue, dim3(blocks), dim3(threads), lds, nullptr, d_out, d_ticks, iters > 20000u ? iters : 20000u, 1u);
  hipLaunchKernelGGL(k_microbench_valu_issue, dim3(blocks), dim3(threads), lds, nullptr, d_out, d_ticks, iters, 1u);
  std::vector<unsigned long long> t((size_t)blocks * (threads / 64) * 2);
  hipError_t e = hipGetLastError();
  if (e == hipSuccess) e = hipMemcpy(t.data(), d_ticks, t.size() * 8, hipMemcpyDeviceToHost);
  (void)hipFree(d_out);
  (void)hipFree(d_ticks);
  if (e != hipSuccess) return fail(KZG_FAIL_HIP, std::string("valu issue microbenchmark: ") + hipGetErrorString(e));
  std::vector<double> cyc, ghz;
  for (size_t i = 0; i < t.size(); i += 2) {
    cyc.push_back((double)t[i] / ((double)iters * 256.0 * waves_per_simd));
    if (t[i + 1]) ghz.push_back((double)t[i] / ((double)t[i + 1] * 10.0));
  }
  std::sort(cyc.begin(), cyc.end());
  std::sort(ghz.begin(), ghz.end());
  *cycles_per_inst = cyc[cyc.size() / 2];
  *clock_ghz = ghz.empty() ? 0.0 : ghz[ghz.size() / 2];
  return 0;
} catch (...) {
  return abi_exception();
}

__global__ __launch_bounds__(64) void k_clock_probe(unsigned long long* out, unsigned long long ticks) {
  if (threadIdx.x != 0) return;
  const unsigned long long r0 = __builtin_amdgcn_s_memrealtime();
  const unsigned long long t0 = __builtin_amdgcn_s_memtime();
  unsigned long long r1 = r0;
  while (r1 - r0 < ticks) {
    __builtin_amdgcn_s_sleep(127);
    r1 = __builtin_amdgcn_s_memrealtime();
  }
  out[2 * blockIdx.x] = __builtin_amdgcn_s_memtime() - t0;
  out[2 * blockIdx.x + 1] = r1 - r0;
}
constexpr int KZG_CLOCK_PROBES = 8;
// ... 174 lines not shown
```

kateth_amd/csrc/engine_internal.hpp:

```cpp
#pragma once
#include <hip/hip_runtime.h>

#include <stdio.h>
#include <stdlib.h>
#include <string.h>

#include <atomic>
#include <chrono>
#include <condition_variable>
#include <deque>
#include <functional>
#include <mutex>
#include <new>
#include <string>
#include <thread>
#include <utility>
#include <vector>

#include "../../include/kateth_amd.h"
#include "comb_geom.hpp"
#include "g1.cuh"
#include "sha256.cuh"
#include "pairing.hpp"
#include "verify_kind.hpp"

using namespace kzg;

int32_t fail(int32_t code, const std::string& msg);
int32_t abi_exception() noexcept;
const std::string& last_error_text();
struct ErrorSnapshot {
  std::string text;
  int32_t detail = 0;
};
ErrorSnapshot error_snapshot();
void error_publish(const ErrorSnapshot& e);

bool helper_dispatch(std::function<void()> fn);

template <class Job>
static int32_t run_on_helpers(uint32_t count, Job&& job) {
  if (count == 0) return 0;
  std::vector<int32_t> rc(count, 0);
  std::vector<ErrorSnapshot> err(count);
  std::vector<char> handed(count, 0);
  std::mutex mu;
  std::condition_variable cv;
  uint32_t pending = 0;
  for (uint32_t k = 1; k < count; k++) {
    {
      std::lock_guard<std::mutex> g(mu);
      pending++;
    }
    bool ok = false;
    try {
      ok = helper_dispatch([&, k]() {
        rc[k] = job(k);
        if (rc[k]) err[k] = error_snapshot();
        std::lock_guard<std::mutex> g(mu);
        pending--;
        cv.notify_one();
      });
    } catch (...) {
    }
    if (ok) {
      handed[k] = 1;
    } else {
      std::lock_guard<std::mutex> g(mu);
      pending--;
    }
  }
  rc[0] = job(0);
  if (rc[0]) err[0] = error_snapshot();
  for (uint32_t k = 1; k < count; k++)
    if (!handed[k]) {
      rc[k] = job(k);
      if (rc[k]) err[k] = error_snapshot();
    }
  {
    std::unique_lock<std::mutex> g(mu);
    cv.wait(g, [&] { return pending == 0; });
  }
  for (uint32_t k = 0; k < count; k++)
    if (rc[k]) {
      error_publish(err[k]);
      return rc[k];
    }
  return 0;
}

#define HIP_TRY(expr)                                                                                      \
  do {                                                                                                     \
    hipError_t _e = (expr);                                                                                \
    if (_e != hipSuccess) return fail(KZG_FAIL_HIP, std::string(#expr) + ": " + hipGetErrorString(_e));  \
  } while (0)

struct EnvKnobs {
  bool trace = false;
  uint64_t proof_chunk = 0;
  int proof_overlap = -1;
  int eval_group = 0;
  bool verify_serial = false;
  bool single_via_batch = false;
  bool var_glv = false;
  uint32_t var_seg = 1;
  bool var_msm_classic = false;
  uint64_t verify_chunk = 0;
  uint32_t verify_streams = 0;
  uint32_t comb_fair = 20;
  bool lat_table = true;
  bool comb_full_wave = false;
  uint32_t msm_splits = 0;
  uint64_t challenge_split_max = 0;
  uint64_t sidecar_pass = 0;
  uint64_t cells_pass = 0;
  uint64_t cellproof_pass = 0;
};
EnvKnobs read_env_knobs();

struct TraceTimer {
  bool on;
  std::chrono::steady_clock::time_point t0;
  const char* what;
  TraceTimer(bool enabled, const char* w) : on(enabled), t0(std::chrono::steady_clock::now()), what(w) {}
  void mark(const char* label) {
    if (!on) return;
    auto t1 = std::chrono::steady_clock::now();
    fprintf(stderr, "[kateth_amd trace] %s: %s +%.3f ms\n", what, label, std::chrono::duration<double, std::milli>(t1 - t0).count());
    t0 = t1;
  }
};

constexpr int KZG_STAGE_SLOTS = 4;
constexpr int KZG_STAGE_STREAMS = 4;
#define KZG_SESSION_STREAM (reinterpret_cast<hipStream_t>(static_cast<intptr_t>(-1)))
enum ProfKind { PROF_MSM_FIXED = 0, PROF_CHALLENGE, PROF_EVAL, PROF_DECODE, PROF_POLY, PROF_VAR_MSM, PROF_REDUCE_COMPRESS, PROF_TRANSPOSE, PROF_KINDS };
static_assert(PROF_KINDS == KZG_PROF_KINDS, "include/kateth_amd.h and ProfKind disagree");
struct ProfEvent {
  int kind;
  hipEvent_t e0, e1;
};

struct kzg_verify_session;
struct kzg_ctx;
constexpr int KZG_WS_SLOTS = 3;
struct WsSlot {
  void* p = nullptr;
  size_t bytes = 0;
  hipEvent_t ev = nullptr;
  hipStream_t last_st = nullptr;
  bool used = false;
};
struct MsmOverride {
  const char* kernel_name;
  bool replaces_table;
  uint64_t adds_per_blob;
  int32_t (*build)(kzg_ctx* ctx);
  int32_t (*launch)(const kzg_ctx* ctx, bool be_bytes, const uint8_t* d_scalars, uint64_t n, int32_t* d_status, g1_xyzz* partials, uint32_t splits,
                    uint32_t lpb, void* scratch, hipStream_t st);
  void (*destroy)(kzg_ctx* ctx);
};
extern const MsmOverride* (*g_msm_override_hook)(kzg_ctx* ctx, uint32_t window_bits);

struct CombTables {
  CombGeom comb{}, comb_lat{};
  uint4 *d_table = nullptr, *d_table_lat = nullptr, *d_comb_k = nullptr, *d_comb_k_lat = nullptr;
  uint64_t table_bytes = 0;
  uint32_t window_class = 0;
};
struct TableChoice {
  uint32_t c, G;
  size_t need;
};

struct kzg_ctx {
  int device = 0;
  std::vector<kzg_ctx*> peers;
  mutable std::atomic<uint32_t> rr{0};
  std::thread build_thread;
  std::atomic<bool> build_cancel{false};
  mutable std::mutex build_mu;
  mutable std::condition_variable build_cv;
  bool build_running = false;
  int32_t build_rc = 0;
  ErrorSnapshot build_err;
  std::vector<CombTables> retired;
  uint4* d_table = nullptr;
  bool use_comb = true;
  CombGeom comb{};
  const MsmOverride* msm_override = nullptr;
  void* override_state = nullptr;
  CombGeom comb_lat{};
  uint4* d_table_lat = nullptr;
  uint4* d_comb_k = nullptr;
  uint4* d_comb_k_lat = nullptr;
  uint32_t window_class = 0;
  uint4* d_bases_brp = nullptr;
  fr_t* d_roots_brp = nullptr;
  uint32_t* d_eval_tab = nullptr;
  uint32_t* d_cells_tab = nullptr;
  uint32_t* d_recover_tab = nullptr;
  uint32_t* d_cellv_tab = nullptr;
  fr_t* d_cellv_h64 = nullptr;
  mutable std::mutex g1_monomial_mu;
  mutable std::atomic<bool> g1_monomial_ready{false};
  mutable uint4* d_g1_monomial = nullptr;
  mutable uint8_t g1_monomial48[KZG_G1_MONOMIAL_POINTS * 48] = {};
  mutable std::mutex cellproof_mu;
  mutable std::atomic<bool> cellproof_ready{false};
  mutable uint32_t* d_cellproof_tab = nullptr;
  mutable std::atomic<uint64_t> cellproof_vectors{0};
  struct PairPin {
    void* p = nullptr;
    size_t bytes = 0;
    hipEvent_t ev = nullptr;
  };
  mutable std::vector<PairPin> pair_pins;
  uint4* d_gen_affine = nullptr;
  host::pairing_ctx* pairing = nullptr;
  uint64_t table_bytes = 0;
  uint32_t num_cus = 256;
  hipStream_t side_stream = nullptr;
  hipStream_t copy_stream = nullptr;
  EnvKnobs knobs;
  mutable std::mutex lock;
  mutable WsSlot wss[KZG_WS_SLOTS];
  mutable uint32_t ws_next = 0;
  mutable uint32_t ws_cur = 0;
  mutable std::vector<hipEvent_t> proof_events;
  mutable std::mutex prof_lock;
  mutable std::atomic<bool> profiling{false};
  mutable std::vector<ProfEvent> prof_events;
  mutable size_t prof_used = 0;
  mutable unsigned long long* d_clock_probe = nullptr;
  mutable hipStream_t probe_stream = nullptr;
  mutable std::mutex pool_lock;
  mutable std::vector<kzg_verify_session*> session_pool;
  mutable std::atomic<uint64_t> each_checks{0};
  mutable std::atomic<uint64_t> sessions_created{0};
  mutable std::mutex stage_lock;
  mutable uint8_t* stage = nullptr;
  mutable size_t stage_bytes = 0;
  mutable uint8_t* hostio = nullptr;
  mutable size_t hostio_bytes = 0;
  mutable bool stage_ready = false;
  mutable hipStream_t verify_stream = nullptr, stage_copy_stream = nullptr, stage_streams[KZG_STAGE_STREAMS] = {};
  mutable hipEvent_t stage_copied[KZG_STAGE_SLOTS] = {}, stage_done[KZG_STAGE_SLOTS] = {}, stage_join[KZG_STAGE_STREAMS] = {};
};
void session_pool_clear(const kzg_ctx* ctx);

static inline bool is_group(const kzg_ctx* ctx) { return ctx && !ctx->peers.empty(); }
constexpr size_t KZG_BYTES_PER_CELL_SET = (size_t)KZG_CELLS_PER_EXT_BLOB * KZG_BYTES_PER_CELL;
int32_t ctx_create_single(const uint8_t* g1_lagrange, const uint8_t* g2_monomial, const kzg_config* cfg, int device, kzg_ctx** out);
int32_t commit_host(const kzg_ctx* ctx, const uint8_t* blobs, uint64_t n, uint8_t* out48, uint8_t* out_affine96, int32_t* status);
int32_t proof_host(const kzg_ctx* ctx, const uint8_t* blobs, const uint8_t* side, size_t side_bytes, bool side_is_commitment, uint64_t n, uint8_t* out48,
                   uint8_t* out_affine96, uint8_t* out_y32, int32_t* status);
int32_t sidecar_host(const kzg_ctx* ctx, const uint8_t* blobs, uint64_t n, uint8_t* out_commitments48, uint8_t* out_proofs48, uint8_t* out_versioned_hashes32,
                     int32_t* status);
struct CellCall {
  const uint8_t *in, *present;
  uint8_t *out_cells, *out_proofs48;
  int32_t* status;
  const uint8_t* want = nullptr;
  CellCall advanced(uint64_t first) const {
    return CellCall{in + first * (present ? KZG_BYTES_PER_CELL_SET : (size_t)KZG_BYTES_PER_BLOB), present ? present + first * 16 : nullptr,
                    out_cells ? out_cells + first * KZG_BYTES_PER_CELL_SET : nullptr,
                    out_proofs48 ? out_proofs48 + first * (KZG_CELLS_PER_EXT_BLOB * 48) : nullptr, status + first, want ? want + first * 16 : nullptr};
  }
};
int32_t das_host(const kzg_ctx* ctx, const CellCall& call, uint64_t n);
int32_t das_dev(const kzg_ctx* ctx, const CellCall& call, uint64_t n, hipStream_t st);
int32_t verify_proof_single(const kzg_ctx* ctx, const uint8_t* proof48, const uint8_t* commitment48, const uint8_t* z32, const uint8_t* y32, int32_t* ok);
int32_t g1_decompress_single(const kzg_ctx* ctx, const uint8_t* in48, uint64_t n, uint8_t* out_affine96, int32_t* status);
int32_t evaluate_blobs_single(const kzg_ctx* ctx, const uint8_t* blobs, const uint8_t* z32, uint64_t n, uint8_t* out_y32, int32_t* status);
int32_t group_create(const uint8_t* g1_lagrange, const uint8_t* g2_monomial, const kzg_config* cfg, kzg_ctx** out);
int32_t multi_verify_proof(const kzg_ctx* ctx, const uint8_t* proof48, const uint8_t* commitment48, const uint8_t* z32, const uint8_t* y32, int32_t* ok);
using MemberCall = std::function<int32_t(const kzg_ctx* member, uint64_t first, uint64_t count)>;
int32_t on_group_members(const kzg_ctx* ctx, uint64_t n, const MemberCall& fn);
template <class Fn>
static inline int32_t on_members(const kzg_ctx* ctx, uint64_t n, Fn&& fn) {
  return is_group(ctx) ? on_group_members(ctx, n, std::ref(fn)) : fn(ctx, (uint64_t)0, n);
}
using VerifyKind = kzg::verify::Kind;
using kzg::verify::facts;
static_assert(facts(VerifyKind::CELLS).tail_terms == KZG_G1_MONOMIAL_POINTS, "lincomb B's fixed terms of the cells kind are the context's monomial points");
struct VerifyInputs {
  VerifyKind kind;
  const uint8_t *blobs, *commitments48, *proofs48, *z32, *y32;
  bool on_host;
  const uint64_t* cell_indices = nullptr;
  const uint8_t* cells = nullptr;
  const uint64_t* commitment_indices = nullptr;
  uint64_t ncom = 0;
  bool rows() const { return commitment_indices != nullptr; }
  bool any_null() const {
    return !commitments48 || !proofs48 || (kind == VerifyKind::BLOBS ? !blobs : kind == VerifyKind::POINTS ? (!z32 || !y32) : (!cell_indices || !cells));
  }
  VerifyInputs advanced(uint64_t first) const {
    VerifyInputs a{kind, blobs ? blobs + first * (size_t)KZG_BYTES_PER_BLOB : nullptr, rows() ? commitments48 : commitments48 + first * 48, proofs48 + first * 48,
                   z32 ? z32 + first * 32 : nullptr, y32 ? y32 + first * 32 : nullptr, on_host};
    a.cell_indices = cell_indices ? cell_indices + first : nullptr;
    a.cells = cells ? cells + first * (size_t)KZG_BYTES_PER_CELL : nullptr;
    a.commitment_indices = rows() ? commitment_indices + first : nullptr;
    a.ncom = ncom;
    return a;
  }
};
static inline VerifyInputs blob_inputs(const void* blobs, const void* commitments48, const void* proofs48, bool on_host) {
  return VerifyInputs{VerifyKind::BLOBS, (const uint8_t*)blobs, (const uint8_t*)commitments48, (const uint8_t*)proofs48, nullptr, nullptr, on_host};
}
static inline VerifyInputs point_inputs(const void* proofs48, const void* commitments48, const void* z32, const void* y32, bool on_host) {
  return VerifyInputs{VerifyKind::POINTS, nullptr, (const uint8_t*)commitments48, (const uint8_t*)proofs48, (const uint8_t*)z32, (const uint8_t*)y32, on_host};
}
static inline VerifyInputs cell_inputs(const void* commitments48, const void* cell_indices, const void* cells, const void* proofs48, bool on_host) {
  VerifyInputs in{VerifyKind::CELLS, nullptr, (const uint8_t*)commitments48, (const uint8_t*)proofs48, nullptr, nullptr, on_host};
  in.cell_indices = (const uint64_t*)cell_indices;
  in.cells = (const uint8_t*)cells;
  return in;
}
static inline VerifyInputs cell_rows_inputs(const void* commitments48, uint64_t ncom, const void* commitment_indices, const void* cell_indices, const void* cells,
                                            const void* proofs48, bool on_host) {
  VerifyInputs in = cell_inputs(commitments48, cell_indices, cells, proofs48, on_host);
  in.commitment_indices = (const uint64_t*)commitment_indices;
  in.ncom = ncom;
  return in;
}
struct VerifyEach {
  uint8_t* ok_each;
  int32_t* status;
};
int32_t verify_batch_single(const kzg_ctx* ctx, const VerifyInputs& in, uint64_t n, hipStream_t st, const VerifyEach* each, int32_t* ok);
int32_t verify_phase1(const kzg_ctx* ctx, const VerifyInputs& in, uint64_t n, hipStream_t st, uint8_t* out_root32, int32_t* err, kzg_verify_session** session);
int32_t multi_verify_batch(const kzg_ctx* ctx, const VerifyInputs& in, uint64_t n, int32_t* ok);
int32_t multi_verify_each(const kzg_ctx* ctx, const VerifyInputs& in, uint64_t n, const VerifyEach& each, int32_t* ok);
int32_t ensure_g1_monomial(const kzg_ctx* ctx);
int32_t verify_batch_finish(const kzg_ctx* ctx, const uint8_t* partials192, uint64_t world, VerifyKind kind, int32_t* ok);
struct GroupDevShare {
  const kzg_ctx* member;
  VerifyInputs in;
  uint64_t first, count;
  hipStream_t st;
};
int32_t verify_group_dev(const kzg_ctx* ctx, const std::vector<GroupDevShare>& shares, uint64_t n_total, int32_t* ok);
static inline size_t align_up(size_t v, size_t a) { return (v + a - 1) / a * a; }
struct Carve {
  size_t off = 0;
  size_t take(size_t bytes) { const size_t o = off; off = align_up(off + bytes, 256); return o; }
};
int32_t stage_init(const kzg_ctx* ctx);
int32_t stage_reserve(const kzg_ctx* ctx, size_t arena_bytes, size_t io_bytes);
void stage_drain(const kzg_ctx* ctx);
void stage_destroy(const kzg_ctx* ctx);
int32_t stream_after(hipStream_t waiter, hipStream_t signaller, hipEvent_t ev);
struct StageRing {
  const kzg_ctx* ctx = nullptr;
  uint64_t slots = 1;
  size_t slot_bytes = 0;
  bool overlap = true;
  int32_t open(const kzg_ctx* c, uint64_t nslots, size_t bytes_per_slot, size_t io_bytes, bool overlap_copies);
  int32_t feed(uint64_t k, const uint8_t* host_src, size_t bytes, hipStream_t comp, uint8_t** d_chunk);
  hipEvent_t done_event(uint64_t k) const;
  int32_t consumed(uint64_t k, hipStream_t comp);
};

struct HostCall {
  const kzg_ctx* ctx;
  StageRing ring;
  hipStream_t st = nullptr;
  std::vector<uint64_t> plan;
  uint64_t max_pass = 0;
  explicit HostCall(const kzg_ctx* c) : ctx(c) {}
  int upload(const void* host, size_t bytes) { return add(UP, const_cast<void*>(host), bytes); }
  int download(void* host, size_t bytes) { return add(DOWN, host, bytes); }
  int scratch(size_t bytes) { return add(SCRATCH, nullptr, bytes); }
  template <class T = uint8_t>
  T* dev(int handle) const {
    return opened && handle >= 0 ? reinterpret_cast<T*>(ctx->hostio + arrays[handle].off) : nullptr;
  }
  int32_t open(std::vector<uint64_t> passes_plan, size_t item_slot_bytes, bool overlap);
  int32_t open(std::vector<uint64_t> passes_plan, size_t item_slot_bytes) {
    const bool piped = passes_plan.size() > 1;
    return open(std::move(passes_plan), item_slot_bytes, piped);
  }
  template <class Body>
  int32_t passes(const uint8_t* src, size_t item_bytes, Body&& body) {
    int32_t rc = 0;
    uint64_t base = 0;
    for (size_t k = 0; k < plan.size() && rc == 0; base += plan[k], k++) {
      uint8_t* d_chunk = nullptr;
      rc = ring.feed(k, src + base * item_bytes, plan[k] * item_bytes, st, &d_chunk);
      if (rc == 0) rc = body(k, base, plan[k], d_chunk);
      if (rc == 0) rc = ring.consumed(k, st);
    }
    return rc;
  }
  int32_t close(int32_t rc);

 private:
  enum Kind { UP, DOWN, SCRATCH };
  struct Array {
    Kind kind;
    void* host;
    size_t bytes, off;
  };
  static constexpr int MAX_ARRAYS = 8;
  Array arrays[MAX_ARRAYS];
  int count = 0;
  bool opened = false, too_many = false;
  Carve io;
  std::unique_lock<std::mutex> stage_guard;
  int add(Kind kind, void* host, size_t bytes) {
    if (kind != SCRATCH && !host) return -1;
    if (count == MAX_ARRAYS) {
      too_many = true;
      return -1;
    }
    arrays[count] = Array{kind, host, bytes, io.take(bytes)};
    return count++;
  }
};
static inline std::vector<uint64_t> even_plan(uint64_t n, uint64_t pass) {
  std::vector<uint64_t> plan;
  for (uint64_t rest = n; rest; rest -= plan.back()) plan.push_back(rest < pass ? rest : pass);
  return plan;
}

int32_t ws_begin(const kzg_ctx* ctx, hipStream_t st);
int32_t ws_wait(const kzg_ctx* ctx, hipStream_t st);
int32_t ws_reserve(const kzg_ctx* ctx, size_t bytes, hipStream_t st);
int32_t ws_end(const kzg_ctx* ctx, hipStream_t st);
struct WsCall {
  const kzg_ctx* ctx;
  hipStream_t st;
  bool open = false;
  WsCall(const kzg_ctx* c, hipStream_t s) : ctx(c), st(s) {}
  int32_t begin() {
    const int32_t rc = ws_begin(ctx, st);
    open = rc == 0;
    return rc;
  }
  int32_t end() {
    open = false;
    return ws_end(ctx, st);
  }
  ~WsCall() {
    if (open) (void)ws_end(ctx, st);
  }
};
static inline uint8_t* ws_ptr(const kzg_ctx* ctx) { return reinterpret_cast<uint8_t*>(ctx->wss[ctx->ws_cur].p); }
template <class Body>
static inline int32_t with_workspace(const kzg_ctx* ctx, hipStream_t st, Body&& body) {
  std::lock_guard<std::mutex> guard(ctx->lock);
  WsCall ws(ctx, st);
  int32_t rc = ws.begin();
  if (rc == 0) rc = body();
  if (rc == 0) rc = ws.end();
  return rc;
}
int32_t prof_next(const kzg_ctx* ctx, int kind, hipEvent_t* e0, hipEvent_t* e1);
struct ProfScope {
  hipEvent_t e1 = nullptr;
  hipStream_t st;
  ProfScope(const kzg_ctx* ctx, int kind, hipStream_t s) : st(s) {
    hipEvent_t e0 = nullptr;
    if (ctx->profiling.load(std::memory_order_relaxed) && prof_next(ctx, kind, &e0, &e1) == 0 && e0) (void)hipEventRecord(e0, st);
  }
  ~ProfScope() {
    if (e1) (void)hipEventRecord(e1, st);
  }
};
uint32_t choose_splits(const kzg_ctx* ctx, uint64_t n);
static inline unsigned blocks_for(uint64_t n, unsigned per) { return (unsigned)((n + per - 1) / per); }

void warm_code_object_blob();
void warm_code_object_proof();
void warm_code_object_verify();
void launch_challenge(const kzg_ctx* ctx, hipStream_t st, const uint8_t* blobs, const uint8_t* commitments48, uint64_t n, fr_t* z);
bool fused_prep_fits(const kzg_ctx* ctx, uint64_t n_blobs, uint64_t n_points);
void launch_challenge_and_decode(const kzg_ctx* ctx, hipStream_t st, const uint8_t* blobs, const uint8_t* commitments48, uint64_t n, fr_t* z, const uint8_t* in_a,
                                 uint64_t n_a, int32_t* status_a, const uint8_t* in_b, uint64_t n_b, int32_t* status_b, uint4* affine, uint8_t* inf);
void launch_g1_decompress(hipStream_t st, const uint8_t* in_a, uint64_t n_a, int32_t* status_a, const uint8_t* in_b, uint64_t n_b, int32_t* status_b, uint4* affine,
                          uint8_t* inf);
void launch_g1_decompress_range(hipStream_t st, uint64_t first, uint64_t count, const uint8_t* in_a, uint64_t n_a, int32_t* status_a, const uint8_t* in_b, uint64_t n_b,
                                int32_t* status_b, uint4* affine, uint8_t* inf);
void launch_fr_parse(hipStream_t st, const uint8_t* in32, uint64_t n, fr_t* out_plain, int32_t* status);
void launch_fr_store_be(hipStream_t st, const fr_t* plain, uint64_t n, const int32_t* status, uint8_t* out32);
void launch_versioned_hash(hipStream_t st, const uint8_t* commitments48, uint64_t n, const int32_t* status, uint8_t* out32);
void launch_glv_points(hipStream_t st, uint4* aff, uint64_t npts, uint64_t phi_off);
void launch_synth_blobs(hipStream_t st, uint64_t seed, uint64_t first_index, uint64_t n, uint8_t* d_blobs);
constexpr uint64_t KZG_FUSED_PREP_MAX = 16384;

constexpr uint64_t KZG_LAT_MAX_BLOBS = 16;
static inline uint32_t lat_splits(uint64_t n) { return n <= 4 ? 256u : (n <= 8 ? 128u : 64u); }
static inline bool msm_uses_lat(const kzg_ctx* ctx, uint32_t splits) { return ctx->d_table_lat != nullptr && splits >= 64u; }
uint32_t msm_lanes_per_blob(const kzg_ctx* ctx, uint64_t n, uint32_t splits);
static inline uint64_t msm_units(uint64_t n, uint32_t splits, uint32_t lpb) { return lpb == 64 ? n * splits : (n + 1) / 2; }

static inline size_t msm_scratch_bytes(const kzg_ctx* ctx, uint64_t n) { return ctx->use_comb ? (size_t)n * KZG_BYTES_PER_BLOB : 0; }

int32_t msm_launch(const kzg_ctx* ctx, bool be_bytes, const uint8_t* d_scalars, uint64_t n, int32_t* d_status, g1_xyzz* partials, uint32_t splits, uint32_t lpb,
                   void* scratch, hipStream_t st, hipEvent_t scalars_consumed = nullptr);
int32_t msm_finish(const kzg_ctx* ctx, uint64_t n, uint8_t* d_out48, uint8_t* d_out_affine96, const int32_t* d_status, g1_xyzz* partials, g1_xyzz* sums,
                   uint32_t splits, uint32_t lpb, hipStream_t st);
struct MsmBufs {
  uint32_t splits = 1;
  size_t o_part = 0, o_sum = 0, o_scratch = 0;
};
static inline MsmBufs msm_carve(const kzg_ctx* ctx, Carve& ws, uint64_t n) {
  MsmBufs b;
  b.splits = choose_splits(ctx, n);
  b.o_part = ws.take((size_t)n * b.splits * 65 * sizeof(g1_xyzz));
  b.o_sum = ws.take((size_t)n * sizeof(g1_xyzz));
  b.o_scratch = ws.take(msm_scratch_bytes(ctx, n));
  return b;
}
int32_t msm_pipeline(const kzg_ctx* ctx, bool be_bytes, const uint8_t* d_scalars, uint64_t n, uint8_t* d_out48, uint8_t* d_out_affine96, int32_t* d_status,
                     const MsmBufs& bufs, uint8_t* ws, hipStream_t st);
```

kateth_amd/csrc/msm_comb.cuh:

```cuda
#pragma once
#include "comb_geom.hpp"
#include "fp30.cuh"
#include "issue_fair.cuh"
#include "msm_fixed.cuh"

namespace kzg {

#if defined(__HIPCC__)

__device__ __forceinline__ uint64_t wave_transpose64(uint64_t x, int lane) {
  constexpr uint64_t LO[6] = {0x00000000FFFFFFFFull, 0x0000FFFF0000FFFFull, 0x00FF00FF00FF00FFull,
                              0x0F0F0F0F0F0F0F0Full, 0x3333333333333333ull, 0x5555555555555555ull};
#pragma unroll
  for (int s = 0; s < 6; s++) {
    const int d = 32 >> s;
    const uint64_t lo = LO[s];
    const uint64_t y = __shfl_xor(x, d, 64);
    x = (lane & d) ? ((x & ~lo) | ((y >> d) & lo)) : ((x & lo) | ((y << d) & ~lo));
  }
  return x;
}

template <bool BE_BYTES>
static __global__ __launch_bounds__(512) void k_comb_transpose(const uint8_t* __restrict__ scalars, uint64_t n, uint64_t* __restrict__ masks,
                                                               int32_t* __restrict__ status) {
  __shared__ uint64_t tile[256][8];
  issue_priority_latency();
  const int tid = threadIdx.x;
  const int lane = tid & 63, wv = tid >> 6;
  const uint64_t blob = blockIdx.x >> 3;
  const uint32_t q0 = (uint32_t)(blockIdx.x & 7u) * 8u;
  if (blob >= n) return;
  uint32_t sc[8];
  load_scalar<BE_BYTES>(sc, scalars + blob * (uint64_t)KZG_BYTES_PER_BLOB_ + (uint64_t)((q0 + (uint32_t)wv) * 64u + (uint32_t)lane) * 32u);
  bool bad = false;
  if (BE_BYTES) {
    fr_t v;
#pragma unroll
    for (int w = 0; w < 8; w++) v.v[w] = sc[w];
    if (!fr_is_canonical(v)) {
      bad = true;
#pragma unroll
      for (int w = 0; w < 8; w++) sc[w] = 0;
    }
  }
#pragma unroll
  for (int w = 0; w < 4; w++) {
    const uint64_t row = ((uint64_t)sc[2 * w + 1] << 32) | sc[2 * w];
    tile[64 * w + lane][wv] = wave_transpose64(row, lane);
  }
  __syncthreads();
  {
    const int k = tid >> 1, part = tid & 1;
    uint4* dst = reinterpret_cast<uint4*>(masks + (blob * 256u + (uint64_t)k) * 64u + q0 + 4u * (uint32_t)part);
    const uint4* src = reinterpret_cast<const uint4*>(&tile[k][4 * part]);
    dst[0] = src[0];
    dst[1] = src[1];
  }
  if (BE_BYTES) {
    if (__any(bad) && lane == 0) atomicOr(&status[blob], KZG_ERR_BLOB_INVALID_FIELD_ELEMENT);
  }
}

template <int SLOT>
__device__ __forceinline__ uint32_t comb_mask_bits(uint64_t m, uint32_t off) {
#if defined(__HIP_DEVICE_COMPILE__)
  uint64_t r;
  if constexpr (SLOT == 0) asm volatile("v_lshrrev_b64 %0, %1, %2 ; mask slot 0" : "=v"(r) : "s"(off), "v"(m));
  if constexpr (SLOT == 1) asm volatile("v_lshrrev_b64 %0, %1, %2 ; mask slot 1" : "=v"(r) : "s"(off), "v"(m));
  if constexpr (SLOT == 2) asm volatile("v_lshrrev_b64 %0, %1, %2 ; mask slot 2" : "=v"(r) : "s"(off), "v"(m));
  if constexpr (SLOT == 3) asm volatile("v_lshrrev_b64 %0, %1, %2 ; mask slot 3" : "=v"(r) : "s"(off), "v"(m));
  return (uint32_t)r;
#else
  return (uint32_t)(m >> off);
#endif
}

struct CombLane {
  const uint64_t* mrow;
  const uint64_t* mlane;
  const uint4* tgrp;
  uint32_t nb, bpo, b0, kbase, H, ep64;
  uint32_t q0e;
  bool wide;
  CombWalk w, p1;
  CombLanePos lw, lp1;
  uint64_t mb0, mb1, mb2, mb3;
  fp_t nx, ny;
  bool nneg, ndbl;
  uint32_t nidx;
};
__device__ __forceinline__ void comb_next_mask(CombLane& s) {
  if (s.wide) {
    if (comb_walk_loads_masks(s.w)) {
      const uint4* src = reinterpret_cast<const uint4*>(s.mlane + (s.w.h * 64u + s.w.dq));
      const uint4 lo = src[0], hi = src[1];
      s.mb0 = (uint64_t)lo.x | ((uint64_t)lo.y << 32);
      s.mb1 = (uint64_t)lo.z | ((uint64_t)lo.w << 32);
      s.mb2 = (uint64_t)hi.x | ((uint64_t)hi.y << 32);
      s.mb3 = (uint64_t)hi.z | ((uint64_t)hi.w << 32);
    }
  } else {
    s.mb0 = s.mrow[(s.kbase + s.w.h) * 64u + s.lw.q];
  }
  s.p1 = s.w;
  const bool wrapped = comb_walk_advance(s.w, s.nb, s.bpo);
  if (!s.wide) {
    s.lp1 = s.lw;
    comb_lane_advance(s.lw, s.nb, wrapped, s.b0);
  }
}
__device__ __forceinline__ void comb_cut(CombLane& s, uint32_t bits, uint32_t qe, uint32_t r) {
  const uint32_t tb = comb_tbits(s.nb, r);
  const uint32_t pat = bits & ((1u << tb) - 1u);
  s.nneg = (pat >> (tb - 1u)) != 0u;
  const uint32_t m = s.nneg ? (~pat & ((1u << (tb - 1u)) - 1u)) : pat;
  s.nidx = qe + comb_entry_off(s.nb, r) + m;
  load_affine96(s.nx, s.ny, s.tgrp, s.nidx);
}
__device__ __forceinline__ void comb_gather(CombLane& s) {
  if (s.wide) {
    const uint32_t off = comb_point_off(s.nb, s.p1.r);
    uint32_t bits;
    switch (comb_walk_mask_slot(s.p1)) {
      case 0: bits = comb_mask_bits<0>(s.mb0, off); break;
      case 1: bits = comb_mask_bits<1>(s.mb1, off); break;
      case 2: bits = comb_mask_bits<2>(s.mb2, off); break;
      default: bits = comb_mask_bits<3>(s.mb3, off); break;
    }
    comb_cut(s, bits, s.q0e + s.p1.dq * s.ep64, s.p1.r);
  } else {
    comb_cut(s, (uint32_t)(s.mb0 >> comb_point_off(s.nb, s.lp1.r)), s.lp1.q * s.ep64, s.lp1.r);
  }
  s.ndbl = comb_walk_doubles(s.p1, s.H);
}

template <bool TIMED, int SHAPE = COMB_SHAPE_ANY>
static __global__ __launch_bounds__(64, 2) void k_msm_comb30(const uint64_t* __restrict__ masks, uint64_t n, uint32_t splits, uint32_t lpb,
                                                             const uint4* __restrict__ table, CombGeom g, g1_xyzz* __restrict__ partials,
                                                             const uint4* __restrict__ comb_k, uint64_t* __restrict__ wave_times) {
  const int lane = threadIdx.x;
  const uint64_t unit = blockIdx.x;
  uint64_t wt_wall0 = 0, wt_cyc0 = 0;
  if (TIMED) {
    wt_wall0 = wall_clock64();
    wt_cyc0 = clock64();
  }
  const uint32_t l = (uint32_t)lane % lpb;
  const uint64_t blob = (lpb == 64u) ? unit / splits : unit * (64u / lpb) + (uint32_t)lane / lpb;
  const uint32_t split = (lpb == 64u) ? (uint32_t)(unit % splits) : 0u;
  if (blob >= n) {
    g1_xyzz none;
    xyzz_set_inf(none);
    partials[unit * 64 + lane] = none;
    return;
  }
  const uint32_t lpg = lpb / g.G;
  const uint32_t grp = l / lpg;
  const uint32_t owner = split * lpg + l % lpg;
  const uint32_t bpo = comb_blocks_per_lane(g, splits, lpb);
  const uint32_t b0 = owner * bpo;
  const uint64_t* mrow = masks + blob * (64u * 256u);
  const uint32_t kbase = grp * g.H;
  const uint4* tgrp = table + (uint64_t)grp * g.epg * 6u;
  const uint32_t total = g.H * bpo;
  const uint32_t nb = g.nb;

  g1_xyzz30 acc;
  xyzz30_set_inf(acc);
  if (comb_k != nullptr && l == 0u && split == 0u) {
    fp_t kx, ky;
    load_affine96(kx, ky, comb_k, 0);
    f30_unpack(acc.x, kx.v);
    f30_unpack(acc.y, ky.v);
    acc.zz = f30_one();
    acc.zzz = acc.zz;
    acc.inf = 0;
  }

  CombLane s;
  s.mrow = mrow;
  s.tgrp = tgrp;
  s.nb = nb;
  s.bpo = bpo;
  s.b0 = b0;
  s.kbase = kbase;
  s.H = g.H;
  s.ep64 = g.ep64;
  s.wide = SHAPE == COMB_SHAPE_WIDE ? true : (SHAPE == COMB_SHAPE_NARROW ? false : comb_shape_is_wide(g, splits, lpb));
  const uint32_t q0 = b0 / nb;
  s.q0e = q0 * g.ep64;
  s.mlane = mrow + kbase * 64u + q0;
  comb_walk_start(s.w, g.H);
  s.lw.q = q0;
  s.lw.r = b0 % nb;
  s.lp1 = s.lw;
  s.mb0 = s.mb1 = s.mb2 = s.mb3 = 0;
  s.nneg = s.ndbl = false;
  s.nidx = 0;
  comb_next_mask(s);
  comb_gather(s);
  if (total > 1u) comb_next_mask(s);

#pragma unroll 1
  for (uint32_t t = 0; t < total; t++) {
    if (g.fair) issue_fair_tick_low(g.fair);
    fp30 cx, cy;
    f30_load_entry(cx, cy, s.nx.v, s.ny.v, xyzz30_entry_neg(acc, s.nneg));
    f30_pin(cx);
    f30_pin(cy);
    const bool cneg = s.nneg, cdbl = s.ndbl;
    const uint32_t cidx = s.nidx;
    if (t + 1u < total) {
      comb_gather(s);
      if (t + 2u < total) comb_next_mask(s);
    }
    if (cdbl && !acc.inf) {
      g1_xyzz30 tmp = acc;
      xyzz30_dbl(tmp);
      acc = tmp;
    }
    bool done = false;
    if (!acc.inf) done = xyzz30_madd_fast(acc, cx, cy);
    if (!done) {
      g1_xyzz30 tmp = acc;
      fp_t rx, ry;
      load_affine96(rx, ry, tgrp, cidx);
      fp30 sx, sy;
      f30_load_entry(sx, sy, rx.v, ry.v, xyzz30_entry_neg(tmp, cneg));
      xyzz30_madd_complete(tmp, sx, sy);
      acc = tmp;
    }
  }
  g1_xyzz out;
  xyzz30_to_xyzz(out, acc);
  partials[unit * 64 + lane] = out;
  if (TIMED) {
    if (wave_times && lane == 0) {
      uint32_t hwid, xcc;
      asm volatile("s_getreg_b32 %0, hwreg(HW_REG_HW_ID)" : "=s"(hwid));
      asm volatile("s_getreg_b32 %0, hwreg(HW_REG_XCC_ID)" : "=s"(xcc));
      wave_times[unit * 4 + 0] = wt_wall0;
      wave_times[unit * 4 + 1] = wall_clock64();
      wave_times[unit * 4 + 2] = clock64() - wt_cyc0;
      wave_times[unit * 4 + 3] = ((uint64_t)xcc << 32) | hwid;
    }
  }
}

static __global__ __launch_bounds__(64) void k_comb_bases(const uint4* __restrict__ bases_brp, CombGeom g, uint4* __restrict__ B, uint4* __restrict__ D) {
  const uint32_t i = blockIdx.x * blockDim.x + threadIdx.x;
  if (i >= 4096) return;
  fp_t x, y;
  load_affine96(x, y, bases_brp, i);
  const uint32_t half[8] = KZG_FR_HALF_PLAIN;
  g1_xyzz acc;
  xyzz_set_inf(acc);
  for (int bit = 254; bit >= 0; bit--) {
    xyzz_dbl(acc);
    if ((half[bit >> 5] >> (bit & 31)) & 1u) {
      g1_xyzz mine = acc;
      xyzz_madd(mine, x, y);
      acc = mine;
    }
  }
  for (uint32_t grp = 0; grp < g.G; grp++) {
    fp_t ax, ay;
    xyzz_to_affine(ax, ay, acc);
    store_affine96(B, (uint64_t)grp * 4096u + i, ax, ay);
    xyzz_from_affine(acc, ax, ay);
    g1_xyzz d2 = acc;
    xyzz_dbl(d2);
    fp_t dx, dy;
    xyzz_to_affine(dx, dy, d2);
    store_affine96(D, (uint64_t)grp * 4096u + i, dx, dy);
    if (grp + 1 < g.G)
      for (uint32_t k = 0; k < g.H; k++) xyzz_dbl(acc);
  }
}

static __global__ __launch_bounds__(64) void k_comb_chain(const uint4* __restrict__ B, const uint4* __restrict__ D, uint32_t grp, uint32_t q_first,
                                                          uint32_t nq, CombGeom g, uint32_t sl, g1_xyzz* __restrict__ tmp) {
  const uint64_t tid = (uint64_t)blockIdx.x * blockDim.x + threadIdx.x;
  const uint32_t segs_per_chunk = g.ep64 >> sl;
  if (tid >= (uint64_t)nq * segs_per_chunk) return;
  const uint32_t qi = (uint32_t)(tid / segs_per_chunk);
  const uint32_t e_start = (uint32_t)(tid % segs_per_chunk) << sl;
  uint32_t r = 0;
  while (r + 1 < g.nb && comb_entry_off(g.nb, r + 1) <= e_start) r++;
  const uint32_t tb = comb_tbits(g.nb, r);
  const uint32_t m_start = e_start - comb_entry_off(g.nb, r);
  const uint32_t i0 = (q_first + qi) * 64u + comb_point_off(g.nb, r);
  const uint4* Bg = B + (uint64_t)grp * 4096u * 6u;
  const uint4* Dg = D + (uint64_t)grp * 4096u * 6u;
  g1_xyzz acc;
  xyzz_set_inf(acc);
  for (uint32_t p = 0; p < tb; p++) {
    fp_t x, y;
    load_affine96(x, y, Bg, i0 + p);
    if (!((m_start >> p) & 1u)) fp_neg(y, y);
    g1_xyzz mine = acc;
    xyzz_madd(mine, x, y);
    acc = mine;
  }
  g1_xyzz* o = tmp + (uint64_t)qi * g.ep64 + comb_entry_off(g.nb, r);
  o[m_start] = acc;
  uint32_t gray = 0;
#pragma unroll 1
  for (uint32_t j = 1; j < (1u << sl); j++) {
    const uint32_t p = (uint32_t)__builtin_ctz(j);
    gray ^= 1u << p;
    fp_t x, y;
    load_affine96(x, y, Dg, i0 + p);
    if (!((gray >> p) & 1u)) fp_neg(y, y);
    g1_xyzz mine = acc;
    xyzz_madd(mine, x, y);
    acc = mine;
    o[m_start | gray] = acc;
  }
}

#endif
}
```

kateth_amd/csrc/msm_reduce_kernels.cuh:

```cuda
#pragma once
#include "msm_fixed.cuh"

namespace kzg {
#if defined(__HIPCC__)

static __global__ __launch_bounds__(64) void k_msm_reduce(const g1_xyzz* __restrict__ partials, uint64_t units, uint32_t lpb, g1_xyzz* __restrict__ unit_sums,
                                                          uint64_t n_out) {
  __shared__ g1_xyzz28 lds[32];
  issue_priority_latency();
  const int lane = threadIdx.x;
  const uint64_t u = blockIdx.x;
  if (u >= units) return;
  g1_xyzz28 acc;
  {
    const g1_xyzz in = partials[u * 64 + lane];
    xyzz28_from_xyzz(acc, in);
  }
#pragma unroll 1
  for (int step = 1; step < (int)lpb; step <<= 1) {
    const int m = 2 * step - 1;
    if ((lane & m) == step) lds[lane >> 1] = acc;
    __syncthreads();
    if ((lane & m) == 0) {
      const g1_xyzz28 other = lds[(lane + step) >> 1];
      xyzz28_add_complete_inl<true>(acc, other);
    }
    __syncthreads();
  }
  const uint64_t slot = u * (64u / lpb) + (uint32_t)lane / lpb;
  if ((lane & (int)(lpb - 1)) == 0 && slot < n_out) {
    g1_xyzz out;
    xyzz28_to_xyzz(out, acc);
    unit_sums[slot] = out;
  }
}

static __global__ __launch_bounds__(64) void k_msm_reduce_half4(const g1_xyzz* __restrict__ partials, uint64_t units, g1_xyzz* __restrict__ unit_sums,
                                                                uint64_t n_out) {
  __shared__ g1_xyzz28 lds[32];
  issue_priority_latency();
  const int lane = threadIdx.x;
  const int q = lane >> 4, j = lane & 15;
  const uint64_t u = (uint64_t)blockIdx.x * 2 + (uint32_t)(q >> 1);
  const uint64_t slot = u * 2 + (uint32_t)(q & 1);
  const bool live = u < units && slot < n_out;
  g1_xyzz28 acc;
  xyzz28_set_inf(acc);
  if (live) {
    const g1_xyzz* row = partials + u * 64 + (uint32_t)(q & 1) * 32u;
    const g1_xyzz a = row[j], b = row[j + 16];
    g1_xyzz28 other;
    xyzz28_from_xyzz(acc, a);
    xyzz28_from_xyzz(other, b);
    xyzz28_add_complete_inl<true>(acc, other);
  }
#pragma unroll 1
  for (int step = 1; step < 16; step <<= 1) {
    const int m = 2 * step - 1;
    if ((lane & m) == step) lds[lane >> 1] = acc;
    __syncthreads();
    if ((lane & m) == 0) {
      const g1_xyzz28 other = lds[(lane + step) >> 1];
      xyzz28_add_complete_inl<true>(acc, other);
    }
    __syncthreads();
  }
  if (j == 0 && live) {
    g1_xyzz out;
    xyzz28_to_xyzz(out, acc);
    unit_sums[slot] = out;
  }
}

__device__ __forceinline__ void g1_finish_item(const g1_xyzz& sum, uint64_t b, const int32_t* __restrict__ status, uint8_t* __restrict__ out48,
                                               uint8_t* __restrict__ out_affine96) {
  uint32_t w[12], aff[24];
  if (status != nullptr && status[b] != 0) {
#pragma unroll
    for (int q = 0; q < 12; q++) w[q] = 0;
#pragma unroll
    for (int q = 0; q < 24; q++) aff[q] = 0;
  } else if (out_affine96) {
    g1_encode_xyzz28_words<true>(w, aff, sum);
  } else {
    g1_encode_xyzz28_words<false>(w, aff, sum);
  }
  if (out48) {
    uint32_t* o = reinterpret_cast<uint32_t*>(out48 + b * 48);
#pragma unroll
    for (int q = 0; q < 12; q++) o[q] = w[q];
  }
  if (out_affine96) {
    uint32_t* o = reinterpret_cast<uint32_t*>(out_affine96 + b * 96);
#pragma unroll
    for (int q = 0; q < 24; q++) o[q] = aff[q];
  }
}

template <bool FINISH>
static __global__ __launch_bounds__(64) void k_msm_reduce_splits(const g1_xyzz* __restrict__ unit_sums, uint32_t splits, uint64_t n, g1_xyzz* __restrict__ sums,
                                                                 const int32_t* __restrict__ status, uint8_t* __restrict__ out48,
                                                                 uint8_t* __restrict__ out_affine96) {
  __shared__ g1_xyzz28 lds[32];
  issue_priority_latency();
  const int t = threadIdx.x;
  const uint64_t b = blockIdx.x;
  if (b >= n) return;
  g1_xyzz28 acc;
  xyzz28_set_inf(acc);
  if ((uint32_t)t < splits) {
    const g1_xyzz in = unit_sums[b * splits + t];
    xyzz28_from_xyzz(acc, in);
  }
#pragma unroll 1
  for (uint32_t u = 64u + (uint32_t)t; u < splits; u += 64u) {
    const g1_xyzz in = unit_sums[b * splits + u];
    g1_xyzz28 other;
    xyzz28_from_xyzz(other, in);
    xyzz28_add_complete_inl<true>(acc, other);
  }
#pragma unroll 1
  for (int step = 1; step < 64 && (uint32_t)step < splits; step <<= 1) {
    const int m = 2 * step - 1;
    if ((t & m) == step) lds[t >> 1] = acc;
    __syncthreads();
    if ((t & m) == 0) {
      const g1_xyzz28 other = lds[(t + step) >> 1];
      xyzz28_add_complete_inl<true>(acc, other);
    }
    __syncthreads();
  }
  if (t == 0) {
    g1_xyzz out;
    xyzz28_to_xyzz(out, acc);
    if (FINISH)
      g1_finish_item(out, b, status, out48, out_affine96);
    else
      sums[b] = out;
  }
}

static __global__ __launch_bounds__(64) void k_g1_compress(const g1_xyzz* __restrict__ sums, uint64_t n, const int32_t* __restrict__ status,
                                                    uint8_t* __restrict__ out48, uint8_t* __restrict__ out_affine96) {
  issue_priority_latency();
  const uint64_t b = (uint64_t)blockIdx.x * blockDim.x + threadIdx.x;
  if (b >= n) return;
  const g1_xyzz acc = sums[b];
  g1_finish_item(acc, b, status, out48, out_affine96);
}

#endif
}
```

kateth_amd/kzg.py:

```python
from __future__ import annotations

import ctypes
import json
import os
from typing import List, Optional, Sequence, Tuple, Union

BYTES_PER_BLOB = 131072
CELLS_PER_EXT_BLOB = 128
FIELD_ELEMENTS_PER_CELL = 64
BYTES_PER_CELL = 2048
_HERE = os.path.dirname(os.path.abspath(__file__))


class BlobError(Exception):
    def __init__(self, kind: str):
        super().__init__("blob::Error::" + kind)
        self.kind = kind


class FiniteFieldError(Exception):
    def __init__(self, kind: str):
        super().__init__("bls::FiniteFieldError::" + kind)
        self.kind = kind


class ECGroupError(Exception):
    def __init__(self, kind: str):
        super().__init__("bls::ECGroupError::" + kind)
        self.kind = kind


class BlsError(Exception):

    def __init__(self, inner: Exception):
        super().__init__(str(inner))
        self.inner = inner


class KzgError(Exception):

    def __init__(self, inner: Exception):
        super().__init__(str(inner))
        self.inner = inner


class LoadSetupError(Exception):
    pass


class CellsError(Exception):

    def __init__(self, kind: str):
        super().__init__("cells::Error::" + kind)
        self.kind = kind


class EngineError(RuntimeError):
    """negative return from the C ABI: HIP / argument / device failure."""


_STATUS = {
    1: lambda: BlobError("InvalidLen"),
    2: lambda: BlobError("InvalidFieldElement"),
    3: lambda: ECGroupError("InvalidEncoding"),
    4: lambda: ECGroupError("NotOnCurve"),
    5: lambda: ECGroupError("NotInGroup"),
    6: lambda: FiniteFieldError("InvalidEncoding"),
    7: lambda: FiniteFieldError("NotInFiniteField"),
    8: lambda: CellsError("NotEnoughCells"),
    9: lambda: CellsError("Inconsistent"),
    10: lambda: CellsError("CellIndex"),
    11: lambda: CellsError("CommitmentIndex"),
}


def error_from_status(code: int) -> Exception:
    return _STATUS[code]()


def _kzg_error(code: int) -> KzgError:
    inner = error_from_status(code)
    return KzgError(inner if isinstance(inner, BlobError) else BlsError(inner))


def _cell_verify_error(code: int) -> Exception:
    inner = error_from_status(code)
    return inner if isinstance(inner, CellsError) else _kzg_error(code)


class _Config(ctypes.Structure):
    _fields_ = [("struct_size", ctypes.c_uint32), ("device", ctypes.c_int32), ("window_bits", ctypes.c_int32), ("flags", ctypes.c_int32), ("plane_groups", ctypes.c_int32),
                ("table_budget_bytes", ctypes.c_uint64), ("devices", ctypes.POINTER(ctypes.c_int32)), ("ndev", ctypes.c_uint32), ("reserved", ctypes.c_uint32)]

    @classmethod
    def new(cls, device=0, window_bits=0, flags=0, plane_groups=0, table_budget_bytes=0, devices=None, ndev=0, reserved=0):
        return cls(ctypes.sizeof(cls), device, window_bits, flags, plane_groups, table_budget_bytes, devices, ndev, reserved)


CFG_TABLE_MAX = 0x1
CFG_BUILD_ASYNC = 0x2
ALL_DEVICES = 0xFFFFFFFF


def library_path() -> str:
    return os.environ.get("KATETH_AMD_LIB", os.path.join(_HERE, "libkateth_amd.so"))


_LIB = None
_ALT_LIBS = {}

_u8p = ctypes.c_void_p
_i32p = ctypes.POINTER(ctypes.c_int32)
_vpp = ctypes.POINTER(ctypes.c_void_p)
_u64p = ctypes.POINTER(ctypes.c_uint64)

_SIGNATURES = {
    "kzg_last_error": (ctypes.c_char_p, []),
    "kzg_last_error_code": (ctypes.c_int32, []),
    "kzg_ctx_create": (ctypes.c_int32, [_u8p, _u8p, ctypes.POINTER(_Config), ctypes.POINTER(ctypes.c_void_p)]),
    "kzg_ctx_create_multi": (ctypes.c_int32, [_u8p, _u8p, ctypes.POINTER(ctypes.c_int32), ctypes.c_uint32, ctypes.POINTER(_Config), ctypes.POINTER(ctypes.c_void_p)]),
    "kzg_ctx_destroy": (None, [ctypes.c_void_p]),
    "kzg_device_count": (ctypes.c_int32, []),
    "kzg_ctx_members": (ctypes.c_uint32, [ctypes.c_void_p]),
    "kzg_ctx_member_device": (ctypes.c_int32, [ctypes.c_void_p, ctypes.c_uint32]),
    "kzg_ctx_member": (ctypes.c_void_p, [ctypes.c_void_p, ctypes.c_uint32]),
    "kzg_ctx_ready": (ctypes.c_int32, [ctypes.c_void_p]),
    "kzg_ctx_wait_ready": (ctypes.c_int32, [ctypes.c_void_p]),
    "kzg_ctx_window_bits": (ctypes.c_int32, [ctypes.c_void_p]),
    "kzg_ctx_msm_kernel_name": (ctypes.c_char_p, [ctypes.c_void_p]),
    "kzg_ctx_plane_groups": (ctypes.c_int32, [ctypes.c_void_p]),
    "kzg_ctx_table_bytes": (ctypes.c_uint64, [ctypes.c_void_p]),
    "kzg_blob_to_commitment_batch": (ctypes.c_int32, [ctypes.c_void_p, _u8p, ctypes.c_uint64, _u8p, _i32p]),
    "kzg_blob_to_commitment_batch_dev": (ctypes.c_int32, [ctypes.c_void_p, ctypes.c_void_p, ctypes.c_uint64, ctypes.c_void_p, ctypes.c_void_p, ctypes.c_void_p]),
    "kzg_blob_to_commitment_batch_affine": (ctypes.c_int32, [ctypes.c_void_p, _u8p, ctypes.c_uint64, _u8p, _i32p]),
    "kzg_compute_blob_proof_batch_affine": (ctypes.c_int32, [ctypes.c_void_p, _u8p, _u8p, ctypes.c_uint64, _u8p, _i32p]),
    "kzg_compute_proof_batch_affine": (ctypes.c_int32, [ctypes.c_void_p, _u8p, _u8p, ctypes.c_uint64, _u8p, _u8p, _i32p]),
    "kzg_compute_blob_proof_batch": (ctypes.c_int32, [ctypes.c_void_p, _u8p, _u8p, ctypes.c_uint64, _u8p, _i32p]),
    "kzg_compute_blob_proof_batch_dev": (ctypes.c_int32, [ctypes.c_void_p, ctypes.c_void_p, ctypes.c_void_p, ctypes.c_uint64, ctypes.c_void_p, ctypes.c_void_p, ctypes.c_void_p]),
    "kzg_blob_sidecar_batch": (ctypes.c_int32, [ctypes.c_void_p, _u8p, ctypes.c_uint64, _u8p, _u8p, _u8p, _i32p]),
    "kzg_blob_sidecar_batch_dev": (
        ctypes.c_int32,
        [ctypes.c_void_p, ctypes.c_void_p, ctypes.c_uint64, ctypes.c_void_p, ctypes.c_void_p, ctypes.c_void_p, ctypes.c_void_p, ctypes.c_void_p],
    ),
    "kzg_compute_cells_batch": (ctypes.c_int32, [ctypes.c_void_p, _u8p, ctypes.c_uint64, _u8p, _i32p]),
    "kzg_compute_cells_batch_dev": (ctypes.c_int32, [ctypes.c_void_p, ctypes.c_void_p, ctypes.c_uint64, ctypes.c_void_p, ctypes.c_void_p, ctypes.c_void_p]),
    "kzg_recover_cells_batch": (ctypes.c_int32, [ctypes.c_void_p, _u8p, _u8p, ctypes.c_uint64, _u8p, _i32p]),
    "kzg_recover_cells_batch_dev": (
        ctypes.c_int32,
        [ctypes.c_void_p, ctypes.c_void_p, ctypes.c_void_p, ctypes.c_uint64, ctypes.c_void_p, ctypes.c_void_p, ctypes.c_void_p],
    ),
    "kzg_compute_cells_and_proofs_batch": (ctypes.c_int32, [ctypes.c_void_p, _u8p, ctypes.c_uint64, _u8p, _u8p, _i32p]),
    "kzg_compute_cells_and_proofs_batch_dev": (
        ctypes.c_int32,
        [ctypes.c_void_p, ctypes.c_void_p, ctypes.c_uint64, ctypes.c_void_p, ctypes.c_void_p, ctypes.c_void_p, ctypes.c_void_p],
    ),
    "kzg_recover_cells_and_proofs_batch": (ctypes.c_int32, [ctypes.c_void_p, _u8p, _u8p, ctypes.c_uint64, _u8p, _u8p, _i32p]),
    "kzg_recover_cells_and_proofs_batch_dev": (
        ctypes.c_int32,
        [ctypes.c_void_p, ctypes.c_void_p, ctypes.c_void_p, ctypes.c_uint64, ctypes.c_void_p, ctypes.c_void_p, ctypes.c_void_p, ctypes.c_void_p],
    ),
    "kzg_compute_cells_and_proofs_select_batch": (ctypes.c_int32, [ctypes.c_void_p, _u8p, _u8p, ctypes.c_uint64, _u8p, _u8p, _i32p]),
    "kzg_compute_cells_and_proofs_select_batch_dev": (
        ctypes.c_int32,
        [ctypes.c_void_p, ctypes.c_void_p, _u8p, ctypes.c_uint64, ctypes.c_void_p, ctypes.c_void_p, ctypes.c_void_p, ctypes.c_void_p],
    ),
    "kzg_recover_cells_and_proofs_select_batch": (ctypes.c_int32, [ctypes.c_void_p, _u8p, _u8p, _u8p, ctypes.c_uint64, _u8p, _u8p, _i32p]),
    "kzg_recover_cells_and_proofs_select_batch_dev": (
        ctypes.c_int32,
        [ctypes.c_void_p, ctypes.c_void_p, ctypes.c_void_p, _u8p, ctypes.c_uint64, ctypes.c_void_p, ctypes.c_void_p, ctypes.c_void_p, ctypes.c_void_p],
    ),
    "kzg_ctx_cellproof_vectors": (ctypes.c_uint64, [ctypes.c_void_p]),
    "kzg_compute_proof_batch": (ctypes.c_int32, [ctypes.c_void_p, _u8p, _u8p, ctypes.c_uint64, _u8p, _u8p, _i32p]),
    "kzg_verify_blob_proof_batch": (ctypes.c_int32, [ctypes.c_void_p, _u8p, _u8p, _u8p, ctypes.c_uint64, _i32p]),
    "kzg_verify_blob_proof_batch_dev": (ctypes.c_int32, [ctypes.c_void_p, ctypes.c_void_p, ctypes.c_void_p, ctypes.c_void_p, ctypes.c_uint64, _i32p, ctypes.c_void_p]),
    "kzg_verify_blob_proof": (ctypes.c_int32, [ctypes.c_void_p, _u8p, _u8p, _u8p, _i32p]),
    "kzg_verify_proof": (ctypes.c_int32, [ctypes.c_void_p, _u8p, _u8p, _u8p, _u8p, _i32p]),
    "kzg_verify_proof_batch": (ctypes.c_int32, [ctypes.c_void_p, _u8p, _u8p, _u8p, _u8p, ctypes.c_uint64, _i32p]),
    "kzg_verify_proof_batch_dev": (ctypes.c_int32, [ctypes.c_void_p, ctypes.c_void_p, ctypes.c_void_p, ctypes.c_void_p, ctypes.c_void_p, ctypes.c_uint64, _i32p, ctypes.c_void_p]),
    "kzg_verify_cell_proof_batch": (ctypes.c_int32, [ctypes.c_void_p, _u8p, _u64p, _u8p, _u8p, ctypes.c_uint64, _i32p]),
    "kzg_verify_cell_proof_batch_dev": (ctypes.c_int32, [ctypes.c_void_p, ctypes.c_void_p, ctypes.c_void_p, ctypes.c_void_p, ctypes.c_void_p, ctypes.c_uint64, _i32p, ctypes.c_void_p]),
    "kzg_ctx_g1_monomial": (ctypes.c_int32, [ctypes.c_void_p, ctypes.c_uint32, ctypes.c_uint32, _u8p]),
    "kzg_verify_proof_batch_group_dev": (ctypes.c_int32, [ctypes.c_void_p, _vpp, _vpp, _vpp, _vpp, _u64p, _i32p, _vpp]),
    "kzg_verify_proof_phase1_dev": (
        ctypes.c_int32,
        [ctypes.c_void_p, ctypes.c_void_p, ctypes.c_void_p, ctypes.c_void_p, ctypes.c_void_p, ctypes.c_uint64, _u8p, _i32p, ctypes.POINTER(ctypes.c_void_p), ctypes.c_void_p],
    ),
    "kzg_verify_blob_proof_batch_each": (ctypes.c_int32, [ctypes.c_void_p, _u8p, _u8p, _u8p, ctypes.c_uint64, _u8p, _i32p, _i32p]),
    "kzg_verify_blob_proof_batch_each_dev": (
        ctypes.c_int32,
        [ctypes.c_void_p, ctypes.c_void_p, ctypes.c_void_p, ctypes.c_void_p, ctypes.c_uint64, _u8p, _i32p, _i32p, ctypes.c_void_p],
    ),
    "kzg_verify_proof_batch_each": (ctypes.c_int32, [ctypes.c_void_p, _u8p, _u8p, _u8p, _u8p, ctypes.c_uint64, _u8p, _i32p, _i32p]),
    "kzg_verify_proof_batch_each_dev": (
        ctypes.c_int32,
        [ctypes.c_void_p, ctypes.c_void_p, ctypes.c_void_p, ctypes.c_void_p, ctypes.c_void_p, ctypes.c_uint64, _u8p, _i32p, _i32p, ctypes.c_void_p],
    ),
    "kzg_verify_cell_proof_batch_rows": (ctypes.c_int32, [ctypes.c_void_p, _u8p, ctypes.c_uint64, _u64p, _u64p, _u8p, _u8p, ctypes.c_uint64, _i32p]),
    "kzg_verify_cell_proof_batch_rows_dev": (
        ctypes.c_int32,
        [ctypes.c_void_p, ctypes.c_void_p, ctypes.c_uint64, ctypes.c_void_p, ctypes.c_void_p, ctypes.c_void_p, ctypes.c_void_p, ctypes.c_uint64, _i32p, ctypes.c_void_p]),
    "kzg_cell_row_weights": (ctypes.c_int32, [ctypes.c_void_p, _u8p, ctypes.c_uint64, _u64p, ctypes.c_uint64, ctypes.c_uint64, _u8p]),
    "kzg_verify_cell_proof_batch_each": (ctypes.c_int32, [ctypes.c_void_p, _u8p, _u64p, _u8p, _u8p, ctypes.c_uint64, _u8p, _i32p, _i32p]),
    "kzg_verify_cell_proof_batch_each_dev": (
        ctypes.c_int32,
        [ctypes.c_void_p, ctypes.c_void_p, ctypes.c_void_p, ctypes.c_void_p, ctypes.c_void_p, ctypes.c_uint64, _u8p, _i32p, _i32p, ctypes.c_void_p],
    ),
    "kzg_g1_monomial_lincomb": (ctypes.c_int32, [ctypes.c_void_p, _u8p, ctypes.c_uint64, _u8p]),
    "kzg_verify_each_checks": (ctypes.c_uint64, [ctypes.c_void_p]),
    "kzg_ctx_sessions_created": (ctypes.c_uint64, [ctypes.c_void_p]),
    "kzg_verify_session_tree": (ctypes.c_int32, [ctypes.c_void_p, _u8p, ctypes.c_uint64, ctypes.c_uint64, ctypes.c_uint64]),
    "kzg_verify_session_tree_range": (ctypes.c_int32, [ctypes.c_void_p, ctypes.c_uint64, ctypes.c_uint64, _u8p]),
    "kzg_g1_decompress_batch": (ctypes.c_int32, [ctypes.c_void_p, _u8p, ctypes.c_uint64, _u8p, _i32p]),
    "kzg_evaluate_blobs": (ctypes.c_int32, [ctypes.c_void_p, _u8p, _u8p, ctypes.c_uint64, _u8p, _i32p]),
    "kzg_verify_phase1_dev": (
        ctypes.c_int32,
        [ctypes.c_void_p, ctypes.c_void_p, ctypes.c_void_p, ctypes.c_void_p, ctypes.c_uint64, _u8p, _i32p, ctypes.POINTER(ctypes.c_void_p), ctypes.c_void_p],
    ),
    "kzg_blob_to_commitment_batch_group_dev": (ctypes.c_int32, [ctypes.c_void_p, _vpp, _u64p, _vpp, _vpp, _vpp]),
    "kzg_compute_blob_proof_batch_group_dev": (ctypes.c_int32, [ctypes.c_void_p, _vpp, _vpp, _u64p, _vpp, _vpp, _vpp]),
    "kzg_verify_blob_proof_batch_group_dev": (ctypes.c_int32, [ctypes.c_void_p, _vpp, _vpp, _vpp, _u64p, _i32p, _vpp]),
    "kzg_recommended_env": (ctypes.c_char_p, []),
    "kzg_ctx_workspace_bytes": (ctypes.c_uint64, [ctypes.c_void_p, ctypes.c_uint32]),
    "kzg_verify_phase2_dev": (ctypes.c_int32, [ctypes.c_void_p, _u8p, ctypes.c_uint64, ctypes.c_uint64, ctypes.c_uint64, _u8p]),
    "kzg_verify_session_destroy": (None, [ctypes.c_void_p]),
    "kzg_verify_session_zy": (ctypes.c_int32, [ctypes.c_void_p, ctypes.c_uint64, ctypes.c_uint64, _u8p, _u8p]),
    "kzg_verify_batch_finish": (ctypes.c_int32, [ctypes.c_void_p, _u8p, ctypes.c_uint64, _i32p]),
    "kzg_synth_blobs_dev": (ctypes.c_int32, [ctypes.c_void_p, ctypes.c_uint64, ctypes.c_uint64, ctypes.c_uint64, ctypes.c_void_p, ctypes.c_void_p]),
    "kzg_profile_begin": (ctypes.c_int32, [ctypes.c_void_p]),
    "kzg_profile_end": (ctypes.c_int32, [ctypes.c_void_p, ctypes.POINTER(ctypes.c_double), ctypes.POINTER(ctypes.c_uint64)]),
    "kzg_profile_end_kinds": (ctypes.c_int32, [ctypes.c_void_p, ctypes.POINTER(ctypes.c_double), ctypes.POINTER(ctypes.c_uint64)]),
    "kzg_profile_kind_name": (ctypes.c_char_p, [ctypes.c_int32]),
    "kzg_ctx_adds_per_blob": (ctypes.c_uint64, [ctypes.c_void_p]),
    "kzg_selftest_field_mul": (ctypes.c_int32, [ctypes.c_void_p, ctypes.c_uint64, ctypes.c_uint64, ctypes.POINTER(ctypes.c_uint64)]),
    "kzg_selftest_exception_guard": (ctypes.c_int32, [ctypes.c_int32]),
    "kzg_microbench_fp_mul": (ctypes.c_int32, [ctypes.c_void_p, ctypes.c_uint64, ctypes.c_uint64, ctypes.POINTER(ctypes.c_float)]),
    "kzg_clock_probe_launch": (ctypes.c_int32, [ctypes.c_void_p, ctypes.c_uint32]),
    "kzg_clock_probe_read": (ctypes.c_int32, [ctypes.c_void_p, ctypes.POINTER(ctypes.c_double), ctypes.POINTER(ctypes.c_double), ctypes.POINTER(ctypes.c_double)]),
    "kzg_microbench_valu_issue": (ctypes.c_int32, [ctypes.c_void_p, ctypes.c_uint32, ctypes.c_uint32, ctypes.POINTER(ctypes.c_double), ctypes.POINTER(ctypes.c_double)]),
}

EXPORTED_SYMBOLS = tuple(_SIGNATURES)


def _ensure_hip_runtime():
    mode = getattr(ctypes, "RTLD_GLOBAL", 0)
    try:
        import torch

        cand = os.path.join(os.path.dirname(torch.__file__), "lib", "libamdhip64.so")
        if os.path.exists(cand):
            ctypes.CDLL(cand, mode=mode)
            return
    except ImportError:
        pass
    for cand in (os.environ.get("KATETH_AMD_HIP_RUNTIME", ""), "/opt/rocm/lib/libamdhip64.so", "libamdhip64.so"):
        if cand:
            try:
                ctypes.CDLL(cand, mode=mode)
                return
            except OSError:
                continue
    raise ImportError("kateth_amd: no HIP runtime (libamdhip64.so) could be loaded")


def load_library(path: Optional[str] = None):
    global _LIB
    if path is None and _LIB is not None:
        return _LIB
    if path is not None and path in _ALT_LIBS:
        return _ALT_LIBS[path]
    alt = path is not None
    path = path or library_path()
    if not os.path.exists(path):
        raise ImportError(
            "kateth_amd: HIP engine %s not found -- build it with `python -c 'import __graft_entry__ as g; g.build()'` "
            "(hipcc --offload-arch=gfx950).  There is no CPU fallback." % path
        )
    _ensure_hip_runtime()
    lib = ctypes.CDLL(path)
    for name, (restype, argtypes) in _SIGNATURES.items():
        fn = getattr(lib, name)
        fn.restype = restype
        fn.argtypes = argtypes
    if alt:
# ... 68 lines not shown
        return self._data

    def __len__(self):
        return len(self._data)


class P1:

    COMPRESSED = 48

    def __init__(self, affine96: bytes):
        assert len(affine96) == 96
        self.affine = bytes(affine96)

    def is_inf(self) -> bool:
        return not any(self.affine)

    def compress(self) -> bytes:
        if self.is_inf():
            return bytes([0xC0]) + bytes(47)
        rinv = pow(1 << 384, -1, _P)
        x = int.from_bytes(self.affine[:48], "little") * rinv % _P
        y = int.from_bytes(self.affine[48:], "little") * rinv % _P
        out = bytearray(x.to_bytes(48, "big"))
        out[0] |= 0x80 | (0x20 if y > (_P - 1) // 2 else 0)
        return bytes(out)

    def __eq__(self, other):
        return isinstance(other, P1) and self.affine == other.affine

    def __hash__(self):
        return hash(self.affine)


class Setup:

    G1 = 4096
    G2 = 65

    def __init__(self, handle: int, lib):
        self._h = ctypes.c_void_p(handle)
        self._lib = lib

    @classmethod
    def load_json(cls, path, device: int = 0, window_bits: int = 0, lib_path: Optional[str] = None, plane_groups: int = 0, devices=None,
                  table_max: bool = False, build_async: bool = False, table_budget_bytes: int = 0) -> "Setup":
        try:
            with open(path) as fh:
                raw = json.load(fh)
        except OSError as err:
            raise LoadSetupError("Io(%s)" % err)
        except ValueError as err:
            raise LoadSetupError("Serde(%s)" % err)
        try:
            g1 = [_unhex(s) for s in raw["g1_lagrange"]]
            g2 = [_unhex(s) for s in raw["g2_monomial"]]
        except (KeyError, ValueError, AttributeError) as err:
            raise LoadSetupError("Serde(%s)" % err)
        return cls.from_bytes(g1, g2, device=device, window_bits=window_bits, lib_path=lib_path, plane_groups=plane_groups, devices=devices,
                              table_max=table_max, build_async=build_async, table_budget_bytes=table_budget_bytes)

    @classmethod
    def from_bytes(cls, g1_lagrange: Sequence[bytes], g2_monomial: Sequence[bytes], device: int = 0, window_bits: int = 0,
                   lib_path: Optional[str] = None, plane_groups: int = 0, devices=None, table_max: bool = False, build_async: bool = False,
                   table_budget_bytes: int = 0) -> "Setup":
        if len(g1_lagrange) != cls.G1:
            raise LoadSetupError("InvalidLenG1Lagrange")
        if len(g2_monomial) != cls.G2:
            raise LoadSetupError("InvalidLenG2Monomial")
        if any(len(p) != 48 for p in g1_lagrange) or any(len(p) != 96 for p in g2_monomial):
            raise LoadSetupError("Bls(ECGroup(InvalidEncoding))")
        lib = load_library(lib_path)
        flags = (CFG_TABLE_MAX if table_max else 0) | (CFG_BUILD_ASYNC if build_async else 0)
        cfg = _Config.new(device, window_bits, flags, plane_groups, table_budget_bytes, None, 0, 0)
        keep = None
        if devices is not None:
            if isinstance(devices, str):
                assert devices == "all", devices
                cfg.ndev = ALL_DEVICES
            else:
                keep = (ctypes.c_int32 * len(devices))(*devices)
                cfg.devices = ctypes.cast(keep, ctypes.POINTER(ctypes.c_int32))
                cfg.ndev = len(devices)
        out = ctypes.c_void_p()
        rc = lib.kzg_ctx_create(b"".join(g1_lagrange), b"".join(g2_monomial), ctypes.byref(cfg), ctypes.byref(out))
        if rc in (-4, -5):
            code = lib.kzg_last_error_code()
            kind = str(error_from_status(code)) if code in _STATUS else "ECGroup"
            raise LoadSetupError("Bls(%s): %s" % (kind, lib.kzg_last_error().decode()))
        if rc == -6:
            raise LoadSetupError("Unsupported: %s" % lib.kzg_last_error().decode())
        if rc != 0:
            raise EngineError("kzg_ctx_create failed (%d): %s" % (rc, lib.kzg_last_error().decode()))
        return cls(out.value, lib)

    @property
    def members(self) -> int:
        return self._lib.kzg_ctx_members(self._h)

    def member_device(self, k: int) -> int:
        return self._lib.kzg_ctx_member_device(self._h, k)

    def member(self, k: int) -> "Setup":
        h = self._lib.kzg_ctx_member(self._h, k)
        if not h:
            raise IndexError(k)
        m = Setup(h, self._lib)
        m._borrowed = True
        m._owner = self
        return m

    @property
    def ready(self) -> bool:
        return bool(self._lib.kzg_ctx_ready(self._h))

    def wait_ready(self):
        self._check(self._lib.kzg_ctx_wait_ready(self._h), "kzg_ctx_wait_ready")

    def close(self):
        if self._h:
            if not getattr(self, "_borrowed", False):
                self._lib.kzg_ctx_destroy(self._h)
            self._h = None

    def __del__(self):
        try:
            self.close()
        except Exception:
            pass

    @property
    def handle(self) -> int:
        return self._h.value

    @property
    def window_bits(self) -> int:
        return self._lib.kzg_ctx_window_bits(self._h)

    @property
    def plane_groups(self) -> int:
        return self._lib.kzg_ctx_plane_groups(self._h)

    @property
    def msm_kernel_name(self) -> str:
        return self._lib.kzg_ctx_msm_kernel_name(self._h).decode()

    @property
    def table_bytes(self) -> int:
        return self._lib.kzg_ctx_table_bytes(self._h)

    def workspace_bytes(self):
        return [int(self._lib.kzg_ctx_workspace_bytes(self._h, k)) for k in range(3)]

    def _check(self, rc: int, what: str):
        if rc < 0:
            raise EngineError("%s failed (%d): %s" % (what, rc, self._lib.kzg_last_error().decode()))

    def _verdict(self, what: str, args, tail=(), to_error=_kzg_error) -> bool:
        ok = ctypes.c_int32(0)
        rc = getattr(self._lib, what)(self._h, *args, ctypes.byref(ok), *tail)
        self._check(rc, what)
        if rc > 0:
            raise to_error(rc)
        return bool(ok.value)

    def _verdicts(self, what: str, args, n: int, tail=()) -> Tuple[List[bool], List[int], bool]:
        ok_each, status, ok = ctypes.create_string_buffer(max(n, 1)), (ctypes.c_int32 * max(n, 1))(), ctypes.c_int32(0)
        rc = getattr(self._lib, what)(self._h, *args, n, ctypes.cast(ok_each, _u8p), status, ctypes.byref(ok), *tail)
        self._check(rc, what)
        if rc > 0:
            raise EngineError("%s returned %d" % (what, rc))
        return [bool(b) for b in ok_each.raw[:n]], list(status[:n]), bool(ok.value)

    def _produce(self, what: str, inputs, n: int, out_bytes):
        outs = [None if b is None else ctypes.create_string_buffer(b * n) for b in out_bytes]
        status = (ctypes.c_int32 * n)()
        rc = getattr(self._lib, what)(self._h, *inputs, n, *[None if o is None else ctypes.cast(o, ctypes.c_void_p) for o in outs], status)
        self._check(rc, what)
        return tuple(None if o is None else o.raw for o in outs) + (list(status),)

    @staticmethod
    def _host_args(*buffers):
        return [a if isinstance(a, int) else _buf(a) for a in buffers]

    @staticmethod
    def _cell_index_array(cell_indices, n: int):
        if isinstance(cell_indices, int):
            return ctypes.cast(cell_indices, _u64p)
        if isinstance(cell_indices, (bytes, bytearray, memoryview)):
            return (ctypes.c_uint64 * n).from_buffer_copy(cell_indices)
        return (ctypes.c_uint64 * n)(*cell_indices)

    def blob_to_commitment_batch(self, blobs: bytes, n: Optional[int] = None):
        blobs = _buf(blobs)
        n = len(blobs) // BYTES_PER_BLOB if n is None else n
        if len(blobs) != n * BYTES_PER_BLOB:
            raise BlobError("InvalidLen")
        return self._produce("kzg_blob_to_commitment_batch", [blobs], n, [48])

    def compute_blob_proof_batch(self, blobs: bytes, commitments: bytes):
        blobs, commitments = _buf(blobs), _buf(commitments)
        n = len(commitments) // 48
        if len(blobs) != n * BYTES_PER_BLOB or len(commitments) != 48 * n:
            raise BlobError("InvalidLen")
        return self._produce("kzg_compute_blob_proof_batch", [blobs, commitments], n, [48])

    def blob_sidecar_batch(self, blobs: bytes, n: Optional[int] = None):
        blobs = _buf(blobs)
        n = len(blobs) // BYTES_PER_BLOB if n is None else n
        if len(blobs) != n * BYTES_PER_BLOB:
            raise BlobError("InvalidLen")
        return self._produce("kzg_blob_sidecar_batch", [blobs], n, [48, 48, 32])

    def compute_cells_batch(self, blobs: bytes, n: Optional[int] = None):
        blobs = _buf(blobs)
        n = len(blobs) // BYTES_PER_BLOB if n is None else n
        if len(blobs) != n * BYTES_PER_BLOB:
            raise BlobError("InvalidLen")
        return self._produce("kzg_compute_cells_batch", [blobs], n, [CELLS_PER_EXT_BLOB * BYTES_PER_CELL])

    def recover_cells_batch(self, cells: bytes, present: bytes, n: Optional[int] = None):
        cells, present = _buf(cells), _buf(present)
        n = len(present) // 16 if n is None else n
        if len(cells) != n * CELLS_PER_EXT_BLOB * BYTES_PER_CELL or len(present) != n * 16:
            raise ValueError("recover_cells_batch: n * 262144 bytes of cells and n * 16 bytes of mask")
        return self._produce("kzg_recover_cells_batch", [cells, present], n, [CELLS_PER_EXT_BLOB * BYTES_PER_CELL])

    def compute_cells_and_proofs_batch(self, blobs: bytes, n: Optional[int] = None, want_cells: bool = True):
        blobs = _buf(blobs)
        n = len(blobs) // BYTES_PER_BLOB if n is None else n
        if len(blobs) != n * BYTES_PER_BLOB:
            raise BlobError("InvalidLen")
        return self._produce("kzg_compute_cells_and_proofs_batch", [blobs], n,
                             [CELLS_PER_EXT_BLOB * BYTES_PER_CELL if want_cells else None, CELLS_PER_EXT_BLOB * 48])

    def recover_cells_and_proofs_batch(self, cells: bytes, present: bytes, n: Optional[int] = None):
        cells, present = _buf(cells), _buf(present)
        n = len(present) // 16 if n is None else n
        if len(cells) != n * CELLS_PER_EXT_BLOB * BYTES_PER_CELL or len(present) != n * 16:
            raise ValueError("recover_cells_and_proofs_batch: n * 262144 bytes of cells and n * 16 bytes of mask")
        return self._produce("kzg_recover_cells_and_proofs_batch", [cells, present], n, [CELLS_PER_EXT_BLOB * BYTES_PER_CELL, CELLS_PER_EXT_BLOB * 48])

    def _select_call(self, what: str, inputs, n: int, proofs, want_cells: bool):
        size = n * CELLS_PER_EXT_BLOB * 48
        if proofs is not None and len(_buf(proofs)) != size:
            raise ValueError("%s: the proof buffer is n * 6144 bytes" % what)
        io = ctypes.create_string_buffer(bytes(_buf(proofs)) if proofs is not None else bytes(size), size)
        cells = ctypes.create_string_buffer(n * CELLS_PER_EXT_BLOB * BYTES_PER_CELL) if want_cells else None
        status = (ctypes.c_int32 * n)()
        rc = getattr(self._lib, what)(self._h, *inputs, n, None if cells is None else ctypes.cast(cells, ctypes.c_void_p), ctypes.cast(io, ctypes.c_void_p), status)
        self._check(rc, what)
        return (None if cells is None else cells.raw), io.raw, list(status)

    def compute_cells_and_proofs_select_batch(self, blobs: bytes, want: bytes, proofs: Optional[bytes] = None, want_cells: bool = True):
        blobs, want = _buf(blobs), _buf(want)
        n = len(want) // 16
        if len(blobs) != n * BYTES_PER_BLOB or len(want) != n * 16:
            raise ValueError("compute_cells_and_proofs_select_batch: n * 131072 bytes of blobs and n * 16 bytes of mask")
        return self._select_call("kzg_compute_cells_and_proofs_select_batch", [blobs, want], n, proofs, want_cells)

    def recover_cells_and_proofs_select_batch(self, cells: bytes, present: bytes, want: bytes, proofs: Optional[bytes] = None):
        cells, present, want = _buf(cells), _buf(present), _buf(want)
        n = len(present) // 16
        if len(cells) != n * CELLS_PER_EXT_BLOB * BYTES_PER_CELL or len(present) != n * 16 or len(want) != n * 16:
            raise ValueError("recover_cells_and_proofs_select_batch: n * 262144 bytes of cells and two n * 16 bytes of masks")
        return self._select_call("kzg_recover_cells_and_proofs_select_batch", [cells, present, want], n, proofs, True)

    def compute_proof_batch(self, blobs: bytes, zs: bytes):
        blobs, zs = _buf(blobs), _buf(zs)
        n = len(zs) // 32
        if len(blobs) != n * BYTES_PER_BLOB:
            raise BlobError("InvalidLen")
        return self._produce("kzg_compute_proof_batch", [blobs, zs], n, [48, 32])

    def blob_to_commitment_batch_affine(self, blobs: bytes, n: Optional[int] = None):
        blobs = _buf(blobs)
        n = len(blobs) // BYTES_PER_BLOB if n is None else n
        if len(blobs) != n * BYTES_PER_BLOB:
            raise BlobError("InvalidLen")
        return self._produce("kzg_blob_to_commitment_batch_affine", [blobs], n, [96])

    def compute_blob_proof_batch_affine(self, blobs: bytes, commitments: bytes):
        blobs, commitments = _buf(blobs), _buf(commitments)
        n = len(commitments) // 48
        if len(blobs) != n * BYTES_PER_BLOB or len(commitments) != 48 * n:
            raise BlobError("InvalidLen")
        return self._produce("kzg_compute_blob_proof_batch_affine", [blobs, commitments], n, [96])

    def compute_proof_batch_affine(self, blobs: bytes, zs: bytes):
        blobs, zs = _buf(blobs), _buf(zs)
        n = len(zs) // 32
        if len(blobs) != n * BYTES_PER_BLOB:
            raise BlobError("InvalidLen")
        return self._produce("kzg_compute_proof_batch_affine", [blobs, zs], n, [96, 32])

    def blob_to_commitment_point(self, blob) -> P1:
        blob = _buf(blob)
        if len(blob) != BYTES_PER_BLOB:
            raise BlobError("InvalidLen")
        out, status = self.blob_to_commitment_batch_affine(blob, 1)
        if status[0]:
            raise error_from_status(status[0])
        return P1(out)

    def blob_proof_point(self, blob, commitment: bytes) -> P1:
        blob, commitment = _buf(blob), _buf(commitment)
# ... 585 lines not shown
```

Before: 152,800 blobs/s.

## Add feedback-driven load balancing across comb MSM unit classes

Adds a runtime balancer for the fixed-base comb MSM. The kernel now records per-class (unit index mod 8) finish times on the device and hands them to the host through pinned memory. The next call pairs slow classes with fast ones and moves a number of trailing comb blocks from each slow unit to its partner, which writes a second partial set that the half-wave reducer then folds in. This targets tail imbalance when a single round of waves does not fill the GPU evenly, at the cost of extra timing atomics, a reset step in the reducer, and extra adds for units that give work away. A knob to force half-wave shape is also added.

```diff
diff --git a/include/kateth_amd.h b/include/kateth_amd.h
--- a/include/kateth_amd.h
+++ b/include/kateth_amd.h
@@ -80,6 +80,7 @@
 int32_t kzg_ctx_plane_groups(const kzg_ctx* ctx);
 uint64_t kzg_ctx_table_bytes(const kzg_ctx* ctx);
 uint64_t kzg_ctx_workspace_bytes(const kzg_ctx* ctx, uint32_t slot);
+int32_t kzg_ctx_comb_balance(const kzg_ctx* ctx, uint64_t* out44);
 
 int32_t kzg_blob_to_commitment_batch(const kzg_ctx* ctx, const uint8_t* blobs, uint64_t n, uint8_t* out48, int32_t* status);
 int32_t kzg_blob_to_commitment_batch_dev(const kzg_ctx* ctx, const void* d_blobs, uint64_t n, void* d_out48, void* d_status, void* hip_stream);
diff --git a/kateth_amd/csrc/comb_balance.hpp b/kateth_amd/csrc/comb_balance.hpp
--- /dev/null
+++ b/kateth_amd/csrc/comb_balance.hpp
@@ -0,0 +1,103 @@
+#pragma once
+#include <math.h>
+#include <stdint.h>
+#include <stdlib.h>
+#include <string.h>
+
+#include "comb_geom.hpp"
+
+namespace kzg {
+
+constexpr double COMB_BALANCE_DAMP = 0.5;
+constexpr double COMB_BALANCE_HYSTERESIS = 4.0;
+
+inline CombBalance comb_balance_pack(const uint32_t partner[8], const uint32_t shed[8]) {
+  CombBalance b{0, 0};
+  for (uint32_t r = 0; r < 8u; r++) {
+    b.partner |= (uint64_t)(partner[r] & 0xffu) << (8u * r);
+    b.shed |= (uint64_t)(shed[r] & 0xffu) << (8u * r);
+  }
+  return b;
+}
+
+inline CombBalance comb_balance_next(const CombBalance& ran, const double t[8], uint32_t total, uint32_t bpo) {
+  double mean = 0;
+  for (uint32_t r = 0; r < 8u; r++) {
+    if (!(t[r] > 0)) return comb_balance_none();
+    mean += t[r] / 8.0;
+  }
+  if (total == 0u || bpo < 2u || !comb_balance_valid(ran, bpo)) return comb_balance_none();
+  const double tau = mean / total;
+  double nat[8];
+  uint32_t old_partner[8];
+  bool old_pairs = false;
+  for (uint32_t r = 0; r < 8u; r++) {
+    old_partner[r] = comb_balance_partner(ran, r);
+    old_pairs = old_pairs || old_partner[r] != r;
+    nat[r] = t[r] + tau * ((double)comb_balance_shed(ran, r) - (double)comb_balance_shed(ran, old_partner[r]));
+  }
+  uint32_t order[8];
+  for (uint32_t r = 0; r < 8u; r++) order[r] = r;
+  for (uint32_t i = 1; i < 8u; i++)
+    for (uint32_t j = i; j > 0u && nat[order[j]] < nat[order[j - 1u]]; j--) {
+      const uint32_t x = order[j];
+      order[j] = order[j - 1u];
+      order[j - 1u] = x;
+    }
+  uint32_t cand[8];
+  for (uint32_t i = 0; i < 4u; i++) {
+    cand[order[i]] = order[7u - i];
+    cand[order[7u - i]] = order[i];
+  }
+  auto predicted_end = [&](const uint32_t* partner) {
+    double worst = 0;
+    for (uint32_t r = 0; r < 8u; r++) {
+      const double e = 0.5 * (nat[r] + nat[partner[r]]);
+      worst = e > worst ? e : worst;
+    }
+    return worst;
+  };
+  const bool keep = old_pairs && predicted_end(old_partner) <= predicted_end(cand) + COMB_BALANCE_HYSTERESIS * tau;
+  const uint32_t* pairing = keep ? old_partner : cand;
+  uint32_t partner[8], shed[8];
+  for (uint32_t r = 0; r < 8u; r++) {
+    partner[r] = r;
+    shed[r] = 0;
+  }
+  for (uint32_t a = 0; a < 8u; a++) {
+    const uint32_t b = pairing[a];
+    if (b <= a) continue;
+    const double before = old_partner[a] == b ? (double)comb_balance_shed(ran, a) - (double)comb_balance_shed(ran, b) : 0.0;
+    const double target = (nat[a] - nat[b]) / (2.0 * tau);
+    const double x = before + COMB_BALANCE_DAMP * (target - before);
+    long d = (long)(target >= before ? floor(x + 0.5) : ceil(x - 0.5));
+    const long cap = bpo - 1u < 255u ? (long)bpo - 1 : 255;
+    d = d > cap ? cap : (d < -cap ? -cap : d);
+    if (d == 0) continue;
+    partner[a] = b;
+    partner[b] = a;
+    shed[d > 0 ? a : b] = (uint32_t)labs(d);
+  }
+  return comb_balance_pack(partner, shed);
+}
+
+inline bool comb_balance_parse(const char* text, CombBalance& out) {
+  if (text == nullptr || strlen(text) < 10u || text[8] != ':') return false;
+  uint32_t partner[8], shed[8];
+  for (uint32_t r = 0; r < 8u; r++) {
+    if (text[r] < '0' || text[r] > '7') return false;
+    partner[r] = (uint32_t)(text[r] - '0');
+  }
+  const char* p = text + 9;
+  for (uint32_t r = 0; r < 8u; r++) {
+    char* end = nullptr;
+    const unsigned long v = strtoul(p, &end, 10);
+    if (end == p || v > 255ul || *end != (r == 7u ? '\0' : ',')) return false;
+    shed[r] = (uint32_t)v;
+    p = end + 1;
+  }
+  out = comb_balance_pack(partner, shed);
+  return true;
+}
+
+}
diff --git a/kateth_amd/csrc/comb_geom.hpp b/kateth_amd/csrc/comb_geom.hpp
--- a/kateth_amd/csrc/comb_geom.hpp
+++ b/kateth_amd/csrc/comb_geom.hpp
@@ -78,4 +78,36 @@
 KZG_HD bool comb_walk_doubles(const CombWalk& w, uint32_t H) { return w.s == 0u && w.h != H - 1u; }
 KZG_HD uint32_t comb_max_splits(const CombGeom& g) { return (64u * g.nb) / g.lpg; }
 
+KZG_HD void comb_walk_at(CombWalk& w, uint32_t H, uint32_t nb, uint32_t bpo, uint32_t t) {
+  w.h = H - 1u - t / bpo;
+  w.s = t % bpo;
+  w.r = w.s % nb;
+  w.dq = w.s / nb;
 }
+KZG_HD void comb_lane_at(CombLanePos& p, uint32_t nb, uint32_t b0, const CombWalk& w) {
+  p.q = (b0 + w.s) / nb;
+  p.r = (b0 + w.s) % nb;
+}
+KZG_HD uint32_t comb_walk_mask_base(const CombWalk& w) { return w.dq & ~3u; }
+
+struct CombBalance {
+  uint64_t partner;
+  uint64_t shed;
+};
+constexpr uint64_t COMB_BALANCE_IDENTITY = 0x0706050403020100ull;
+KZG_HD CombBalance comb_balance_none() { return CombBalance{COMB_BALANCE_IDENTITY, 0}; }
+KZG_HD uint32_t comb_balance_partner(const CombBalance& b, uint32_t r) { return (uint32_t)(b.partner >> (8u * r)) & 0xffu; }
+KZG_HD uint32_t comb_balance_shed(const CombBalance& b, uint32_t r) { return (uint32_t)(b.shed >> (8u * r)) & 0xffu; }
+KZG_HD bool comb_balance_empty(const CombBalance& b) { return b.shed == 0; }
+KZG_HD bool comb_balance_valid(const CombBalance& b, uint32_t bpo) {
+  for (uint32_t r = 0; r < 8u; r++) {
+    const uint32_t p = comb_balance_partner(b, r), d = comb_balance_shed(b, r);
+    if (p >= 8u || comb_balance_partner(b, p) != r) return false;
+    if (d != 0u && (p == r || d + 1u > bpo || comb_balance_shed(b, p) != 0u)) return false;
+  }
+  return true;
+}
+enum : uint32_t { COMB_REC_START = 0, COMB_REC_END = 1, COMB_REC_UNITS = 9, COMB_REC_WORDS = 10 };
+KZG_HD uint64_t comb_balance_units(uint64_t n) { return (n / 16u) * 8u; }
+
+}
diff --git a/kateth_amd/csrc/engine.hip b/kateth_amd/csrc/engine.hip
--- a/kateth_amd/csrc/engine.hip
+++ b/kateth_amd/csrc/engine.hip
@@ -343,7 +343,7 @@
   const bool half_ok = !ctx->knobs.comb_full_wave && ctx->comb.G <= 32 && (64u * ctx->comb.nb) % (32u / ctx->comb.G) == 0;
   if (half_ok && n >= 2) {
     const double c = rounds((double)((n + 1) / 2)) * (2.0 * A + D + 10.0);
-    if (c < best.cost) best = MsmShapeCost{1, 32, c};
+    if (c < best.cost || ctx->knobs.comb_half_wave) best = MsmShapeCost{1, 32, c};
   }
   return best;
 }
@@ -391,6 +391,21 @@
   if (!ctx || !ctx->use_comb) return 0;
   std::lock_guard<std::mutex> guard(ctx->lock);
   return (int32_t)ctx->comb.G;
+} catch (...) {
+  return abi_exception();
+}
+extern "C" int32_t kzg_ctx_comb_balance(const kzg_ctx* ctx, uint64_t* out44) try {
+  if (!ctx || !out44) return fail(KZG_FAIL_ARGUMENT, "null argument");
+  std::lock_guard<std::mutex> guard(ctx->bal_lock);
+  const CombBalance now = ctx->knobs.comb_balance == 2 ? ctx->knobs.comb_balance_forced : (ctx->knobs.comb_balance == 1 ? ctx->bal_plan : comb_balance_none());
+  for (uint32_t r = 0; r < 8u; r++) {
+    out44[r] = comb_balance_partner(now, r);
+    out44[8u + r] = comb_balance_shed(now, r);
+    out44[28u + r] = comb_balance_partner(ctx->bal_last_ran, r);
+    out44[36u + r] = comb_balance_shed(ctx->bal_last_ran, r);
+  }
+  for (uint32_t i = 0; i < COMB_REC_WORDS + 2u; i++) out44[16u + i] = ctx->bal_last[i];
+  return 0;
 } catch (...) {
   return abi_exception();
 }
@@ -470,6 +485,13 @@
     if (const char* e = getenv("KATETH_AMD_VERIFY_STREAMS")) k.verify_streams = (uint32_t)atoi(e) <= (uint32_t)KZG_STAGE_STREAMS ? (uint32_t)atoi(e) : 0u;
     if (const char* e = getenv("KATETH_AMD_VERIFY_CHUNK")) k.verify_chunk = (uint64_t)atoll(e) > 0 ? (uint64_t)atoll(e) : 0;
     k.comb_full_wave = getenv("KATETH_AMD_COMB_FULL_WAVE") != nullptr;
+    if (const char* e = getenv("KATETH_AMD_COMB_HALF_WAVE")) k.comb_half_wave = atoi(e) != 0;
+    if (const char* e = getenv("KATETH_AMD_COMB_BALANCE")) {
+      if (std::string(e) == "off")
+        k.comb_balance = 0;
+      else if (comb_balance_parse(e, k.comb_balance_forced))
+        k.comb_balance = 2;
+    }
     if (const char* e = getenv("KATETH_AMD_LAT_TABLE")) k.lat_table = atoi(e) != 0;
     if (const char* e = getenv("KATETH_AMD_COMB_FAIR")) k.comb_fair = (uint32_t)atoi(e) < 40u ? (uint32_t)atoi(e) : 0u;
     if (const char* e = getenv("KATETH_AMD_MSM_SPLITS")) {
@@ -533,6 +555,8 @@
   if (ctx->d_gen_affine) (void)hipFree(ctx->d_gen_affine);
   if (ctx->d_comb_k) (void)hipFree(ctx->d_comb_k);
   if (ctx->d_comb_k_lat) (void)hipFree(ctx->d_comb_k_lat);
+  if (ctx->d_bal_rec) (void)hipFree(ctx->d_bal_rec);
+  if (ctx->h_bal_msg) (void)hipHostFree(ctx->h_bal_msg);
   if (ctx->msm_override && ctx->msm_override->destroy) ctx->msm_override->destroy(ctx);
   delete ctx->pairing;
   for (WsSlot& w : ctx->wss) {
@@ -810,6 +834,13 @@
     int32_t rcc = comb_build_tables(ctx, c, G, t, st, nullptr);
     if (rcc) return rcc;
     tables_install(ctx, t);
+    unsigned long long init[kzg_ctx::KZG_BAL_RING * COMB_REC_WORDS] = {};
+    for (uint32_t i = 0; i < kzg_ctx::KZG_BAL_RING; i++) init[i * COMB_REC_WORDS + COMB_REC_START] = ~0ull;
+    HIP_TRY(hipMalloc(&ctx->d_bal_rec, sizeof(init)));
+    HIP_TRY(hipMemcpy(ctx->d_bal_rec, init, sizeof(init), hipMemcpyHostToDevice));
+    const size_t msg_bytes = kzg_ctx::KZG_BAL_RING * (COMB_REC_WORDS + 2) * sizeof(unsigned long long);
+    HIP_TRY(hipHostMalloc(&ctx->h_bal_msg, msg_bytes, hipHostMallocDefault));
+    memset(ctx->h_bal_msg, 0, msg_bytes);
   }
   HIP_TRY(hipDeviceSynchronize());
   return 0;
@@ -1026,8 +1057,48 @@
   return abi_exception();
 }
 
+static void balance_begin(const kzg_ctx* ctx, uint64_t n, uint32_t splits, uint32_t lpb, const CombGeom& geom, bool lat, MsmCall& call) {
+  call = MsmCall{};
+  if (lat || lpb != 32u || splits != 1u || !comb_shape_is_wide(geom, splits, lpb) || comb_balance_units(n) == 0u) return;
+  const uint32_t bpo = comb_blocks_per_lane(geom, splits, lpb), total = geom.H * bpo;
+  if (ctx->knobs.comb_balance == 2 && comb_balance_valid(ctx->knobs.comb_balance_forced, bpo)) call.plan = ctx->knobs.comb_balance_forced;
+  const uint64_t units = msm_units(n, splits, lpb), round = (uint64_t)ctx->num_cus * 8u;
+  if (n % 16u != 0u || units > round || 2u * units <= round || ctx->d_bal_rec == nullptr) return;
+  constexpr uint32_t R = kzg_ctx::KZG_BAL_RING, W = COMB_REC_WORDS + 2u;
+  std::lock_guard<std::mutex> guard(ctx->bal_lock);
+  for (uint64_t s = ctx->bal_seq; s > ctx->bal_seen && s + R > ctx->bal_seq; s--) {
+    const kzg_ctx::BalIssued& was = ctx->bal_issued[s % R];
+    volatile const unsigned long long* msg = ctx->h_bal_msg + (s % R) * W;
+    unsigned long long w[W];
+    w[W - 1u] = __atomic_load_n(&msg[W - 1u], __ATOMIC_ACQUIRE);
+    for (uint32_t i = 1; i + 1u < W; i++) w[i] = msg[i];
+    w[0] = __atomic_load_n(&msg[0], __ATOMIC_ACQUIRE);
+    if (was.seq != s || w[0] != s || w[W - 1u] != s || w[1u + COMB_REC_UNITS] != was.units) continue;
+    ctx->bal_seen = s;
+    ctx->bal_last[0] = s;
+    for (uint32_t i = 0; i < COMB_REC_WORDS; i++) ctx->bal_last[1u + i] = w[1u + i];
+    ctx->bal_last[1u + COMB_REC_WORDS] = was.units;
+    ctx->bal_last_ran = was.ran;
+    if (ctx->knobs.comb_balance == 1) {
+      double t[8];
+      for (uint32_t r = 0; r < 8u; r++) t[r] = (double)(int64_t)(w[1u + COMB_REC_END + r] - w[1u + COMB_REC_START]);
+      ctx->bal_plan = comb_balance_next(was.ran, t, was.total, was.bpo);
+    }
+    break;
+  }
+  if (ctx->knobs.comb_balance == 1 && comb_balance_valid(ctx->bal_plan, bpo)) call.plan = ctx->bal_plan;
+  call.seq = ++ctx->bal_seq;
+  kzg_ctx::BalIssued& now = ctx->bal_issued[call.seq % R];
+  now.seq = call.seq;
+  now.units = units;
+  now.total = total;
+  now.bpo = bpo;
+  now.ran = call.plan;
+}
+
 int32_t msm_launch(const kzg_ctx* ctx, bool be_bytes, const uint8_t* d_scalars, uint64_t n, int32_t* d_status, g1_xyzz* partials, uint32_t splits, uint32_t lpb,
-                   void* scratch, hipStream_t st, hipEvent_t scalars_consumed) {
+                   void* scratch, hipStream_t st, MsmCall& call, hipEvent_t scalars_consumed) {
+  call = MsmCall{};
   if (ctx->msm_override) {
     int32_t rco = ctx->msm_override->launch(ctx, be_bytes, d_scalars, n, d_status, partials, splits, lpb, scratch, st);
     if (rco == 0 && scalars_consumed) HIP_TRY(hipEventRecord(scalars_consumed, st));
@@ -1047,23 +1118,29 @@
   const uint4* table = lat ? ctx->d_table_lat : ctx->d_table;
   const CombGeom geom = lat ? ctx->comb_lat : ctx->comb;
   const uint4* comb_k = (const uint4*)(lat ? ctx->d_comb_k_lat : ctx->d_comb_k);
+  balance_begin(ctx, n, splits, lpb, geom, lat, call);
+  call.partials2 = reinterpret_cast<g1_xyzz*>(reinterpret_cast<uint8_t*>(scratch) + (size_t)n * KZG_BYTES_PER_BLOB);
+  unsigned long long* rec = call.seq ? ctx->d_bal_rec + (call.seq % kzg_ctx::KZG_BAL_RING) * COMB_REC_WORDS : nullptr;
   if (comb_shape_is_wide(geom, splits, lpb))
     hipLaunchKernelGGL((k_msm_comb30<false, COMB_SHAPE_WIDE>), dim3((unsigned)msm_units(n, splits, lpb)), dim3(64), 0, st, masks, n, splits, lpb, table, geom,
-                       partials, comb_k, (uint64_t*)nullptr);
+                       partials, comb_k, (uint64_t*)nullptr, call.plan, call.partials2, rec);
   else
     hipLaunchKernelGGL((k_msm_comb30<false, COMB_SHAPE_NARROW>), dim3((unsigned)msm_units(n, splits, lpb)), dim3(64), 0, st, masks, n, splits, lpb, table, geom,
-                       partials, comb_k, (uint64_t*)nullptr);
+                       partials, comb_k, (uint64_t*)nullptr, comb_balance_none(), (g1_xyzz*)nullptr, (unsigned long long*)nullptr);
   HIP_TRY(hipGetLastError());
   return 0;
 }
 int32_t msm_finish(const kzg_ctx* ctx, uint64_t n, uint8_t* d_out48, uint8_t* d_out_affine96, const int32_t* d_status, g1_xyzz* partials,
-                                 g1_xyzz* sums, uint32_t splits, uint32_t lpb, hipStream_t st) {
+                                 g1_xyzz* sums, uint32_t splits, uint32_t lpb, hipStream_t st, const MsmCall& call) {
   ProfScope ps(ctx, PROF_REDUCE_COMPRESS, st);
   g1_xyzz* unit_sums = (splits == 1) ? sums : partials + (size_t)n * splits * 64;
   const uint64_t units = msm_units(n, splits, lpb);
-  if (lpb == 32)
-    hipLaunchKernelGGL(k_msm_reduce_half4, dim3((unsigned)((units + 1) / 2)), dim3(64), 0, st, partials, units, unit_sums, n);
-  else
+  if (lpb == 32) {
+    const uint64_t slot = call.seq % kzg_ctx::KZG_BAL_RING;
+    hipLaunchKernelGGL(k_msm_reduce_half4, dim3((unsigned)((units + 1) / 2)), dim3(64), 0, st, partials, units, unit_sums, n, (const g1_xyzz*)call.partials2,
+                       call.plan, call.seq ? ctx->d_bal_rec + slot * COMB_REC_WORDS : (unsigned long long*)nullptr,
+                       call.seq ? ctx->h_bal_msg + slot * (COMB_REC_WORDS + 2u) : (unsigned long long*)nullptr, (unsigned long long)call.seq);
+  } else
     hipLaunchKernelGGL(k_msm_reduce, dim3((unsigned)units), dim3(64), 0, st, partials, units, lpb, unit_sums, units);
   if (splits > 64) {
     hipLaunchKernelGGL((k_msm_reduce_splits<true>), dim3((unsigned)n), dim3(64), 0, st, unit_sums, splits, n, sums, d_status, d_out48, d_out_affine96);
@@ -1081,9 +1158,10 @@
                      const MsmBufs& bufs, uint8_t* ws, hipStream_t st) {
   g1_xyzz* partials = reinterpret_cast<g1_xyzz*>(ws + bufs.o_part);
   const uint32_t lpb = msm_lanes_per_blob(ctx, n, bufs.splits);
-  int32_t rc = msm_launch(ctx, be_bytes, d_scalars, n, d_status, partials, bufs.splits, lpb, ws + bufs.o_scratch, st);
+  MsmCall call;
+  int32_t rc = msm_launch(ctx, be_bytes, d_scalars, n, d_status, partials, bufs.splits, lpb, ws + bufs.o_scratch, st, call);
   if (rc) return rc;
-  return msm_finish(ctx, n, d_out48, d_out_affine96, d_status, partials, reinterpret_cast<g1_xyzz*>(ws + bufs.o_sum), bufs.splits, lpb, st);
+  return msm_finish(ctx, n, d_out48, d_out_affine96, d_status, partials, reinterpret_cast<g1_xyzz*>(ws + bufs.o_sum), bufs.splits, lpb, st, call);
 }
 
 static int32_t commit_dev_locked(const kzg_ctx* ctx, const void* d_blobs, uint64_t n, void* d_out48, void* d_out_affine96, int32_t* d_status,
@@ -1234,10 +1312,11 @@
     g1_xyzz* sums = reinterpret_cast<g1_xyzz*>(wslot + o_sums);
     uint8_t* d_chunk = nullptr;
     rc = hc.ring.feed(k, blobs + base * (size_t)KZG_BYTES_PER_BLOB, m * (size_t)KZG_BYTES_PER_BLOB, comp[slot], &d_chunk);
-    if (rc == 0) rc = msm_launch(ctx, true, d_chunk, m, d_status + base, partials, splits, lpb, wslot + o_masks, comp[slot], hc.ring.done_event(k));
+    MsmCall call;
+    if (rc == 0) rc = msm_launch(ctx, true, d_chunk, m, d_status + base, partials, splits, lpb, wslot + o_masks, comp[slot], call, hc.ring.done_event(k));
     if (rc == 0)
       rc = msm_finish(ctx, m, out48 ? d_res + base * 48 : nullptr, out_affine96 ? d_res + base * 96 : nullptr, d_status + base, partials, sums, splits, lpb,
-                      comp[slot]);
+                      comp[slot], call);
   }
   if (rc == 0 && piped) rc = stream_after(comp[0], comp[1], ctx->stage_join[1]);
   if (rc == 0) rc = ws.end();
diff --git a/kateth_amd/csrc/engine_internal.hpp b/kateth_amd/csrc/engine_internal.hpp
--- a/kateth_amd/csrc/engine_internal.hpp
+++ b/kateth_amd/csrc/engine_internal.hpp
@@ -19,6 +19,7 @@
 
 #include "../../include/kateth_amd.h"
 #include "comb_geom.hpp"
+#include "comb_balance.hpp"
 #include "g1.cuh"
 #include "sha256.cuh"
 #include "pairing.hpp"
@@ -110,6 +111,9 @@
   uint32_t comb_fair = 20;
   bool lat_table = true;
   bool comb_full_wave = false;
+  bool comb_half_wave = false;
+  int comb_balance = 1;
+  CombBalance comb_balance_forced = comb_balance_none();
   uint32_t msm_splits = 0;
   uint64_t challenge_split_max = 0;
   uint64_t sidecar_pass = 0;
@@ -223,6 +227,21 @@
   hipStream_t side_stream = nullptr;
   hipStream_t copy_stream = nullptr;
   EnvKnobs knobs;
+  static constexpr uint32_t KZG_BAL_RING = 16;
+  struct BalIssued {
+    uint64_t seq = 0, units = 0;
+    uint32_t total = 0, bpo = 0;
+    CombBalance ran = comb_balance_none();
+  };
+  mutable std::mutex bal_lock;
+  mutable CombBalance bal_plan = comb_balance_none();
+  mutable uint64_t bal_seq = 0;
+  mutable uint64_t bal_seen = 0;
+  mutable BalIssued bal_issued[KZG_BAL_RING];
+  mutable unsigned long long bal_last[COMB_REC_WORDS + 2] = {};
+  mutable CombBalance bal_last_ran = comb_balance_none();
+  unsigned long long* d_bal_rec = nullptr;
+  unsigned long long* h_bal_msg = nullptr;
   mutable std::mutex lock;
   mutable WsSlot wss[KZG_WS_SLOTS];
   mutable uint32_t ws_next = 0;
@@ -496,12 +515,19 @@
 uint32_t msm_lanes_per_blob(const kzg_ctx* ctx, uint64_t n, uint32_t splits);
 static inline uint64_t msm_units(uint64_t n, uint32_t splits, uint32_t lpb) { return lpb == 64 ? n * splits : (n + 1) / 2; }
 
-static inline size_t msm_scratch_bytes(const kzg_ctx* ctx, uint64_t n) { return ctx->use_comb ? (size_t)n * KZG_BYTES_PER_BLOB : 0; }
+static inline size_t msm_scratch_bytes(const kzg_ctx* ctx, uint64_t n) {
+  return ctx->use_comb ? (size_t)n * KZG_BYTES_PER_BLOB + (size_t)((n + 1) / 2) * 64 * sizeof(g1_xyzz) : 0;
+}
+struct MsmCall {
+  CombBalance plan = comb_balance_none();
+  g1_xyzz* partials2 = nullptr;
+  uint64_t seq = 0;
+};
 
 int32_t msm_launch(const kzg_ctx* ctx, bool be_bytes, const uint8_t* d_scalars, uint64_t n, int32_t* d_status, g1_xyzz* partials, uint32_t splits, uint32_t lpb,
-                   void* scratch, hipStream_t st, hipEvent_t scalars_consumed = nullptr);
+                   void* scratch, hipStream_t st, MsmCall& call, hipEvent_t scalars_consumed = nullptr);
 int32_t msm_finish(const kzg_ctx* ctx, uint64_t n, uint8_t* d_out48, uint8_t* d_out_affine96, const int32_t* d_status, g1_xyzz* partials, g1_xyzz* sums,
-                   uint32_t splits, uint32_t lpb, hipStream_t st);
+                   uint32_t splits, uint32_t lpb, hipStream_t st, const MsmCall& call);
 struct MsmBufs {
   uint32_t splits = 1;
   size_t o_part = 0, o_sum = 0, o_scratch = 0;
diff --git a/kateth_amd/csrc/msm_comb.cuh b/kateth_amd/csrc/msm_comb.cuh
--- a/kateth_amd/csrc/msm_comb.cuh
+++ b/kateth_amd/csrc/msm_comb.cuh
@@ -90,10 +90,11 @@
   bool nneg, ndbl;
   uint32_t nidx;
 };
+template <bool FIRST = false>
 __device__ __forceinline__ void comb_next_mask(CombLane& s) {
   if (s.wide) {
-    if (comb_walk_loads_masks(s.w)) {
-      const uint4* src = reinterpret_cast<const uint4*>(s.mlane + (s.w.h * 64u + s.w.dq));
+    if (FIRST || comb_walk_loads_masks(s.w)) {
+      const uint4* src = reinterpret_cast<const uint4*>(s.mlane + (s.w.h * 64u + (FIRST ? comb_walk_mask_base(s.w) : s.w.dq)));
       const uint4 lo = src[0], hi = src[1];
       s.mb0 = (uint64_t)lo.x | ((uint64_t)lo.y << 32);
       s.mb1 = (uint64_t)lo.z | ((uint64_t)lo.w << 32);
@@ -138,7 +139,9 @@
 template <bool TIMED, int SHAPE = COMB_SHAPE_ANY>
 static __global__ __launch_bounds__(64, 2) void k_msm_comb30(const uint64_t* __restrict__ masks, uint64_t n, uint32_t splits, uint32_t lpb,
                                                              const uint4* __restrict__ table, CombGeom g, g1_xyzz* __restrict__ partials,
-                                                             const uint4* __restrict__ comb_k, uint64_t* __restrict__ wave_times) {
+                                                             const uint4* __restrict__ comb_k, uint64_t* __restrict__ wave_times,
+                                                             CombBalance bal = CombBalance{COMB_BALANCE_IDENTITY, 0}, g1_xyzz* __restrict__ partials2 = nullptr,
+                                                             unsigned long long* __restrict__ rec = nullptr) {
   const int lane = threadIdx.x;
   const uint64_t unit = blockIdx.x;
   uint64_t wt_wall0 = 0, wt_cyc0 = 0;
@@ -146,29 +149,22 @@
     wt_wall0 = wall_clock64();
     wt_cyc0 = clock64();
   }
-  const uint32_t l = (uint32_t)lane % lpb;
-  const uint64_t blob = (lpb == 64u) ? unit / splits : unit * (64u / lpb) + (uint32_t)lane / lpb;
+  if (rec != nullptr && lane == 0) atomicMin(&rec[COMB_REC_START], (unsigned long long)wall_clock64());
   const uint32_t split = (lpb == 64u) ? (uint32_t)(unit % splits) : 0u;
-  if (blob >= n) {
+  if (((lpb == 64u) ? unit / splits : unit * (64u / lpb) + (uint32_t)lane / lpb) >= n) {
     g1_xyzz none;
     xyzz_set_inf(none);
     partials[unit * 64 + lane] = none;
     return;
   }
   const uint32_t lpg = lpb / g.G;
-  const uint32_t grp = l / lpg;
-  const uint32_t owner = split * lpg + l % lpg;
   const uint32_t bpo = comb_blocks_per_lane(g, splits, lpb);
-  const uint32_t b0 = owner * bpo;
-  const uint64_t* mrow = masks + blob * (64u * 256u);
-  const uint32_t kbase = grp * g.H;
-  const uint4* tgrp = table + (uint64_t)grp * g.epg * 6u;
   const uint32_t total = g.H * bpo;
   const uint32_t nb = g.nb;
 
   g1_xyzz30 acc;
   xyzz30_set_inf(acc);
-  if (comb_k != nullptr && l == 0u && split == 0u) {
+  if (comb_k != nullptr && (uint32_t)lane % lpb == 0u && split == 0u) {
     fp_t kx, ky;
     load_affine96(kx, ky, comb_k, 0);
     f30_unpack(acc.x, kx.v);
@@ -178,63 +174,95 @@
     acc.inf = 0;
   }
 
-  CombLane s;
-  s.mrow = mrow;
-  s.tgrp = tgrp;
-  s.nb = nb;
-  s.bpo = bpo;
-  s.b0 = b0;
-  s.kbase = kbase;
-  s.H = g.H;
-  s.ep64 = g.ep64;
-  s.wide = SHAPE == COMB_SHAPE_WIDE ? true : (SHAPE == COMB_SHAPE_NARROW ? false : comb_shape_is_wide(g, splits, lpb));
-  const uint32_t q0 = b0 / nb;
-  s.q0e = q0 * g.ep64;
-  s.mlane = mrow + kbase * 64u + q0;
-  comb_walk_start(s.w, g.H);
-  s.lw.q = q0;
-  s.lw.r = b0 % nb;
-  s.lp1 = s.lw;
-  s.mb0 = s.mb1 = s.mb2 = s.mb3 = 0;
-  s.nneg = s.ndbl = false;
-  s.nidx = 0;
-  comb_next_mask(s);
-  comb_gather(s);
-  if (total > 1u) comb_next_mask(s);
-
+  uint32_t first = 0, cnt = total, d2 = 0;
+  uint64_t unit2 = unit;
+  if (!comb_balance_empty(bal) && unit < comb_balance_units(n)) {
+    const uint32_t cls = (uint32_t)unit & 7u, pr = comb_balance_partner(bal, cls);
+    cnt = total - comb_balance_shed(bal, cls);
+    d2 = comb_balance_shed(bal, pr);
+    unit2 = (unit & ~(uint64_t)7) | pr;
+  }
+  uint64_t wunit = unit;
+  g1_xyzz* outp = partials + unit * 64;
 #pragma unroll 1
-  for (uint32_t t = 0; t < total; t++) {
-    if (g.fair) issue_fair_tick_low(g.fair);
-    fp30 cx, cy;
-    f30_load_entry(cx, cy, s.nx.v, s.ny.v, xyzz30_entry_neg(acc, s.nneg));
-    f30_pin(cx);
-    f30_pin(cy);
-    const bool cneg = s.nneg, cdbl = s.ndbl;
-    const uint32_t cidx = s.nidx;
-    if (t + 1u < total) {
-      comb_gather(s);
-      if (t + 2u < total) comb_next_mask(s);
-    }
-    if (cdbl && !acc.inf) {
-      g1_xyzz30 tmp = acc;
-      xyzz30_dbl(tmp);
-      acc = tmp;
-    }
-    bool done = false;
-    if (!acc.inf) done = xyzz30_madd_fast(acc, cx, cy);
-    if (!done) {
-      g1_xyzz30 tmp = acc;
-      fp_t rx, ry;
-      load_affine96(rx, ry, tgrp, cidx);
-      fp30 sx, sy;
-      f30_load_entry(sx, sy, rx.v, ry.v, xyzz30_entry_neg(tmp, cneg));
-      xyzz30_madd_complete(tmp, sx, sy);
-      acc = tmp;
-    }
-  }
-  g1_xyzz out;
-  xyzz30_to_xyzz(out, acc);
-  partials[unit * 64 + lane] = out;
+  for (;;) {
+    uint32_t ln = (uint32_t)lane;
+    asm volatile("" : "+v"(ln));
+    const uint32_t l = ln % lpb;
+    const uint64_t blob = (lpb == 64u) ? wunit / splits : wunit * (64u / lpb) + ln / lpb;
+    const uint32_t grp = l / lpg;
+    const uint32_t owner = split * lpg + l % lpg;
+    const uint32_t b0 = owner * bpo;
+    const uint64_t* mrow = masks + blob * (64u * 256u);
+    const uint32_t kbase = grp * g.H;
+    CombLane s;
+    s.mrow = mrow;
+    s.tgrp = table + (uint64_t)grp * g.epg * 6u;
+    s.nb = nb;
+    s.bpo = bpo;
+    s.b0 = b0;
+    s.kbase = kbase;
+    s.H = g.H;
+    s.ep64 = g.ep64;
+    s.wide = SHAPE == COMB_SHAPE_WIDE ? true : (SHAPE == COMB_SHAPE_NARROW ? false : comb_shape_is_wide(g, splits, lpb));
+    const uint32_t q0 = b0 / nb;
+    s.q0e = q0 * g.ep64;
+    s.mlane = mrow + kbase * 64u + q0;
+    s.mb0 = s.mb1 = s.mb2 = s.mb3 = 0;
+    s.nneg = s.ndbl = false;
+    s.nidx = 0;
+    comb_walk_at(s.w, g.H, nb, bpo, first);
+    comb_lane_at(s.lw, nb, b0, s.w);
+    s.lp1 = s.lw;
+    comb_next_mask<true>(s);
+    comb_gather(s);
+    if (cnt > 1u) comb_next_mask(s);
+
+#pragma unroll 1
+    for (uint32_t t = 0; t < cnt; t++) {
+      if (g.fair) issue_fair_tick_low(g.fair);
+      fp30 cx, cy;
+      f30_load_entry(cx, cy, s.nx.v, s.ny.v, xyzz30_entry_neg(acc, s.nneg));
+      f30_pin(cx);
+      f30_pin(cy);
+      const bool cneg = s.nneg, cdbl = s.ndbl;
+      const uint32_t cidx = s.nidx;
+      if (t + 1u < cnt) {
+        comb_gather(s);
+        if (t + 2u < cnt) comb_next_mask(s);
+      }
+      if (cdbl && !acc.inf) {
+        g1_xyzz30 tmp = acc;
+        xyzz30_dbl(tmp);
+        acc = tmp;
+      }
+      bool done = false;
+      if (!acc.inf) done = xyzz30_madd_fast(acc, cx, cy);
+      if (!done) {
+        g1_xyzz30 tmp = acc;
+        fp_t rx, ry;
+        load_affine96(rx, ry, s.tgrp, cidx);
+        fp30 sx, sy;
+        f30_load_entry(sx, sy, rx.v, ry.v, xyzz30_entry_neg(tmp, cneg));
+        xyzz30_madd_complete(tmp, sx, sy);
+        acc = tmp;
+      }
+    }
+    g1_xyzz out;
+    xyzz30_to_xyzz(out, acc);
+    outp[lane] = out;
+    if (d2 == 0u) break;
+    wunit = unit2;
+    first = total - d2;
+    cnt = d2;
+    d2 = 0;
+    xyzz30_set_inf(acc);
+    outp = partials2 + unit2 * 64;
+  }
+  if (rec != nullptr && lane == 0) {
+    atomicMax(&rec[COMB_REC_END + ((uint32_t)unit & 7u)], (unsigned long long)wall_clock64());
+    atomicAdd(&rec[COMB_REC_UNITS], 1ull);
+  }
   if (TIMED) {
     if (wave_times && lane == 0) {
       uint32_t hwid, xcc;
diff --git a/kateth_amd/csrc/msm_reduce_kernels.cuh b/kateth_amd/csrc/msm_reduce_kernels.cuh
--- a/kateth_amd/csrc/msm_reduce_kernels.cuh
+++ b/kateth_amd/csrc/msm_reduce_kernels.cuh
@@ -1,4 +1,5 @@
 #pragma once
+#include "comb_geom.hpp"
 #include "msm_fixed.cuh"
 
 namespace kzg {
@@ -36,10 +37,22 @@
 }
 
 static __global__ __launch_bounds__(64) void k_msm_reduce_half4(const g1_xyzz* __restrict__ partials, uint64_t units, g1_xyzz* __restrict__ unit_sums,
-                                                                uint64_t n_out) {
+                                                                uint64_t n_out, const g1_xyzz* __restrict__ partials2, CombBalance bal,
+                                                                unsigned long long* __restrict__ rec, volatile unsigned long long* msg,
+                                                                unsigned long long seq) {
   __shared__ g1_xyzz28 lds[32];
   issue_priority_latency();
   const int lane = threadIdx.x;
+  if (rec != nullptr && blockIdx.x == 0) {
+    if (lane == 0) msg[0] = seq;
+    __threadfence_system();
+    if (lane < (int)COMB_REC_WORDS) {
+      msg[1 + lane] = rec[lane];
+      rec[lane] = lane == (int)COMB_REC_START ? ~0ull : 0ull;
+    }
+    __threadfence_system();
+    if (lane == 0) msg[1 + COMB_REC_WORDS] = seq;
+  }
   const int q = lane >> 4, j = lane & 15;
   const uint64_t u = (uint64_t)blockIdx.x * 2 + (uint32_t)(q >> 1);
   const uint64_t slot = u * 2 + (uint32_t)(q & 1);
@@ -48,11 +61,18 @@
   xyzz28_set_inf(acc);
   if (live) {
     const g1_xyzz* row = partials + u * 64 + (uint32_t)(q & 1) * 32u;
-    const g1_xyzz a = row[j], b = row[j + 16];
-    g1_xyzz28 other;
+    const g1_xyzz* row2 = partials2 + u * 64 + (uint32_t)(q & 1) * 32u;
+    const bool giver = !comb_balance_empty(bal) && u < comb_balance_units(n_out) && comb_balance_shed(bal, (uint32_t)u & 7u) != 0u;
+    const int terms = giver ? 4 : 2;
+    const g1_xyzz a = row[j];
     xyzz28_from_xyzz(acc, a);
-    xyzz28_from_xyzz(other, b);
-    xyzz28_add_complete_inl<true>(acc, other);
+#pragma unroll 1
+    for (int k = 1; k < terms; k++) {
+      const g1_xyzz b = ((k & 2) ? row2 : row)[j + 16 * (k & 1)];
+      g1_xyzz28 other;
+      xyzz28_from_xyzz(other, b);
+      xyzz28_add_complete_inl<true>(acc, other);
+    }
   }
 #pragma unroll 1
   for (int step = 1; step < 16; step <<= 1) {
diff --git a/kateth_amd/kzg.py b/kateth_amd/kzg.py
--- a/kateth_amd/kzg.py
+++ b/kateth_amd/kzg.py
@@ -130,6 +130,7 @@
     "kzg_ctx_msm_kernel_name": (ctypes.c_char_p, [ctypes.c_void_p]),
     "kzg_ctx_plane_groups": (ctypes.c_int32, [ctypes.c_void_p]),
     "kzg_ctx_table_bytes": (ctypes.c_uint64, [ctypes.c_void_p]),
+    "kzg_ctx_comb_balance": (ctypes.c_int32, [ctypes.c_void_p, _u64p]),
     "kzg_blob_to_commitment_batch": (ctypes.c_int32, [ctypes.c_void_p, _u8p, ctypes.c_uint64, _u8p, _i32p]),
     "kzg_blob_to_commitment_batch_dev": (ctypes.c_int32, [ctypes.c_void_p, ctypes.c_void_p, ctypes.c_uint64, ctypes.c_void_p, ctypes.c_void_p, ctypes.c_void_p]),
     "kzg_blob_to_commitment_batch_affine": (ctypes.c_int32, [ctypes.c_void_p, _u8p, ctypes.c_uint64, _u8p, _i32p]),
@@ -504,6 +505,16 @@
     def workspace_bytes(self):
         return [int(self._lib.kzg_ctx_workspace_bytes(self._h, k)) for k in range(3)]
 
+    def comb_balance(self) -> dict:
+        w = (ctypes.c_uint64 * 44)()
+        self._check(self._lib.kzg_ctx_comb_balance(self._h, w), "kzg_ctx_comb_balance")
+        w = [int(x) for x in w]
+        rec = None
+        if w[16]:
+            rec = {"seq": w[16], "start": w[17], "end": w[18:26], "end_us": [(e - w[17]) / 100.0 for e in w[18:26]], "units": w[27],
+                   "ran": {"partner": w[28:36], "shed": w[36:44]}}
+        return {"partner": w[0:8], "shed": w[8:16], "record": rec}
+
     def _check(self, rc: int, what: str):
         if rc < 0:
             raise EngineError("%s failed (%d): %s" % (what, rc, self._lib.kzg_last_error().decode()))
```

After: 155,200 blobs/s (median of 6 runs). 1.6% higher.
